# AcrylicShrimp/omok-ai

Hardware: AMD Instinct MI355X
Metric: self-play games/sec (15x15, 800 sims/move); MCTS nodes/sec (higher is better)
Workload: dtype f16x3 split MFMA, fp32 acc; fc0 corrections mixed f16/fp6; 1 GPU; 4096 concurrent 15x15 games per GPU, 800 sims/move, K=16, two trees per game; games_per_gpu=4096, board=15, sims_per_move=800, batch_k=16, warmup_step=whole episode, parallelism=games sharded x1, no hot-path collective

## Files before the change

bindings/omok_mi355x.rs:

```rust
#![allow(non_camel_case_types, dead_code)]

use std::ffi::{CStr, CString};
use std::os::raw::{c_char, c_int, c_void};
use std::ptr;

#[repr(C)]
#[derive(Clone, Copy, Debug)]
pub struct OmokConfig {
    pub board_size: i32,
    pub games: i32,
    pub max_nodes: i32,
    pub max_tables: i32,
    pub max_batch_k: i32,
    pub device: i32,
    pub net_mode: i32,
    pub max_tree_waves: i32,
    pub seed: u64,
    pub game_offset: i64,
}

#[repr(C)]
pub struct OmokEngine {
    _private: [u8; 0],
}
// ... 129 lines not shown
        pub fn omok_mirror_apply(e: *mut OmokEngine) -> c_int;
        pub fn omok_train_begin(e: *mut OmokEngine, max_batch: i32) -> c_int;
        pub fn omok_train_end(e: *mut OmokEngine) -> c_int;
        pub fn omok_train_step(e: *mut OmokEngine, records_dev: *const c_void, n_records: i64, indices: *const i64, batch: i32, losses: *mut f32) -> c_int;
        pub fn omok_train_losses(e: *mut OmokEngine, records_dev: *const c_void, n_records: i64, indices: *const i64, batch: i32, losses: *mut f32) -> c_int;
        pub fn omok_train_batch_indices(e: *mut OmokEngine, n_records: i64, batch: i32, key: u64, step: i32, out: *mut i64) -> c_int;
        pub fn omok_train_run(e: *mut OmokEngine, records_dev: *const c_void, n_records: i64, update_count: i32, batch_size: i32, key: u64, losses: *mut f32) -> c_int;
        pub fn omok_train_gradient_count(e: *const OmokEngine) -> i64;
        pub fn omok_train_backward(e: *mut OmokEngine, records_dev: *const c_void, n_records: i64, indices: *const i64, batch: i32, grad_dst_dev: *mut c_void) -> c_int;
        pub fn omok_train_apply(e: *mut OmokEngine, grads_dev: *const c_void, ranks: i32, losses: *mut f32) -> c_int;
        pub fn omok_debug_train_gradient(e: *mut OmokEngine, index: i32, out: *mut f32, count: i64) -> c_int;
        pub fn omok_net_read(e: *mut OmokEngine, index: i32, out: *mut f32, count: i64) -> c_int;
        pub fn omok_alive_count(e: *mut OmokEngine) -> c_int;
        pub fn omok_current_ply(e: *mut OmokEngine) -> c_int;
        pub fn omok_game_info(e: *mut OmokEngine, alive: *mut u8, status: *mut u8, plies: *mut i32) -> c_int;
        pub fn omok_tree_dump(e: *mut OmokEngine, game: i32, side: i32, ints: *mut i32, floats: *mut f32, cap_nodes: i32) -> c_int;
        pub fn omok_tree_root(e: *mut OmokEngine, game: i32, side: i32, root_n: *mut u32, root_w: *mut f32, n_nodes: *mut i32, n_tables: *mut i32) -> c_int;
        pub fn omok_root_stats(e: *mut OmokEngine, n: *mut u32, w: *mut f32) -> c_int;
        pub fn omok_root_children(e: *mut OmokEngine, game: i32, side: i32, actions: *mut i32, n: *mut u32, w: *mut f32, p: *mut f32, cap: i32) -> c_int;
        pub fn omok_replay_game(e: *mut OmokEngine, game: i32, boards: *mut u8, turns: *mut u8, pi: *mut f32, z: *mut f32, cap_plies: i32) -> c_int;
        pub fn omok_game_log_enable(e: *mut OmokEngine, enabled: i32) -> c_int;
        pub fn omok_game_log_read(e: *mut OmokEngine, first_game: i32, games: i32, start_boards: *mut u8, lengths: *mut i32, moves: *mut u16, root_n: *mut u32, root_w: *mut f32, child_n: *mut u32, child_w: *mut f32) -> c_int;
        pub fn omok_env_replay(e: *mut OmokEngine, start_boards: *const u8, moves: *const u16, lengths: *const i32, batch: i32, stride: i32, upto: i32, boards_out: *mut u8, status_out: *mut i32, played_out: *mut i32) -> c_int;
        pub fn omok_replay_pack_dev(e: *mut OmokEngine, dst_dev: *mut c_void, cap_records: i64) -> i64;
        pub fn omok_replay_record_bytes(e: *const OmokEngine) -> i32;
        pub fn omok_replay_augment_dev(e: *mut OmokEngine, dst_dev: *mut c_void, cap_records: i64) -> i64;
        pub fn omok_replay_augment_records_dev(e: *mut OmokEngine, records_dev: *const c_void, n_records: i64, game_offsets: *const i64, game_lengths: *const i32, games: i32, dst_dev: *mut c_void, cap_records: i64) -> i64;
        pub fn omok_replay_augmented_game(e: *mut OmokEngine, game: i32, boards: *mut u8, turns: *mut u8, pi: *mut f32, z: *mut f32, cap_records: i32) -> c_int;
        pub fn omok_operand_row_bytes(e: *const OmokEngine) -> i64;
        pub fn omok_debug_operand_rows(e: *mut OmokEngine, first_row: i32, rows: i32, out: *mut c_void) -> c_int;
        pub fn omok_debug_set_base_cache(e: *mut OmokEngine, enabled: i32) -> c_int;
        pub fn omok_debug_set_children_kernel(e: *mut OmokEngine, which: i32) -> c_int;
        pub fn omok_debug_set_window_rects(e: *mut OmokEngine, enabled: i32) -> c_int;
        pub fn omok_debug_last_plan(e: *mut OmokEngine, out: *mut i32, cap: i32) -> c_int;
        pub fn omok_get_stats(e: *mut OmokEngine, stats: *mut f64) -> c_int;
        pub fn omok_reset_stats(e: *mut OmokEngine) -> c_int;
        pub fn omok_set_profiling(e: *mut OmokEngine, enabled: i32) -> c_int;
    }
}


#[repr(u8)]
#[derive(Clone, Copy, Debug, PartialEq, Eq)]
pub enum GameStatus {
    InProgress = 0,
    Draw = 1,
    BlackWin = 2,
    WhiteWin = 3,
}

impl GameStatus {
    pub fn from_raw(v: i32) -> Option<GameStatus> {
        match v {
            0 => Some(GameStatus::InProgress),
            1 => Some(GameStatus::Draw),
            2 => Some(GameStatus::BlackWin),
            3 => Some(GameStatus::WhiteWin),
            _ => None,
        }
    }
}

#[derive(Debug)]
pub struct OmokError {
    pub code: i32,
    pub message: String,
// ... 142 lines not shown
```

include/omok_mi355x.h:

```cpp
#ifndef OMOK_MI355X_H
#define OMOK_MI355X_H
#include <stdint.h>

#ifdef __cplusplus
extern "C" {
#endif

#define OMOK_OK 0
#define OMOK_ERR_INVALID (-1)
#define OMOK_ERR_HIP (-2)
#define OMOK_ERR_STATE (-3)
#define OMOK_ERR_OVERFLOW (-4)
#define OMOK_ERR_ILLEGAL (-5)

#define OMOK_MODE_PLAYER 0
#define OMOK_MODE_OPPONENT 1

#define OMOK_NET_F16X3 0
#define OMOK_NET_F32 1
#define OMOK_NET_F16X3_ROWS 2

#define OMOK_NET_F16X3_FP6 3
#define OMOK_NET_F16X3_F16 4
#define OMOK_NET_F16X3_MIXED 5
// ... 108 lines not shown
int omok_debug_train_gradient(omok_engine* e, int32_t index, float* out, int64_t count);
int omok_net_read(omok_engine* e, int32_t index, float* out, int64_t count);

int omok_alive_count(omok_engine* e);
int omok_current_ply(omok_engine* e);
int omok_game_info(omok_engine* e, uint8_t* alive, uint8_t* status, int32_t* plies);
int omok_tree_dump(omok_engine* e, int32_t game, int32_t side, int32_t* ints, float* floats, int32_t cap_nodes);
int omok_tree_root(omok_engine* e, int32_t game, int32_t side, uint32_t* root_n, float* root_w,
                   int32_t* n_nodes, int32_t* n_tables);
int omok_root_stats(omok_engine* e, uint32_t* n, float* w);
int omok_root_children(omok_engine* e, int32_t game, int32_t side, int32_t* actions, uint32_t* n, float* w, float* p, int32_t cap);
int omok_replay_game(omok_engine* e, int32_t game, uint8_t* boards, uint8_t* turns, float* pi, float* z,
                     int32_t cap_plies);
#define OMOK_MOVE_CELL 255
#define OMOK_MOVE_EXTERNAL 256
int omok_game_log_enable(omok_engine* e, int32_t enabled);
int omok_game_log_read(omok_engine* e, int32_t first_game, int32_t games, uint8_t* start_boards, int32_t* lengths, uint16_t* moves,
                       uint32_t* root_n, float* root_w, uint32_t* child_n, float* child_w);
int omok_env_replay(omok_engine* e, const uint8_t* start_boards, const uint16_t* moves, const int32_t* lengths, int32_t batch,
                    int32_t stride, int32_t upto, uint8_t* boards_out, int32_t* status_out, int32_t* played_out);
int64_t omok_replay_pack_dev(omok_engine* e, void* dst_dev, int64_t cap_records);
int32_t omok_replay_record_bytes(const omok_engine* e);
int64_t omok_replay_augment_dev(omok_engine* e, void* dst_dev, int64_t cap_records);
int64_t omok_replay_augment_records_dev(omok_engine* e, const void* records_dev, int64_t n_records, const int64_t* game_offsets,
                                        const int32_t* game_lengths, int32_t games, void* dst_dev, int64_t cap_records);
int omok_replay_augmented_game(omok_engine* e, int32_t game, uint8_t* boards, uint8_t* turns, float* pi, float* z,
                               int32_t cap_records);

int64_t omok_operand_row_bytes(const omok_engine* e);
int omok_debug_operand_rows(omok_engine* e, int32_t first_row, int32_t rows, void* out);
int omok_debug_set_base_cache(omok_engine* e, int32_t enabled);
int omok_debug_set_children_kernel(omok_engine* e, int32_t which);
int omok_debug_set_window_rects(omok_engine* e, int32_t enabled);
#define OMOK_PLAN_INTS 16
int omok_debug_last_plan(omok_engine* e, int32_t* out, int32_t cap);

#define OMOK_STAT_SIMS 0
#define OMOK_STAT_EVALS 1
#define OMOK_STAT_PLY_GAMES 2
#define OMOK_STAT_FINISHED 3
#define OMOK_STAT_MS_TREE 4
#define OMOK_STAT_MS_TRUNK 5
#define OMOK_STAT_MS_FC0 6
#define OMOK_STAT_MS_TAIL 7
#define OMOK_STAT_MS_PLY 8
#define OMOK_STAT_FC0_LAUNCHES 9
#define OMOK_STAT_FC0_ROWS 10
#define OMOK_STAT_TREE_BYTES 11
#define OMOK_STAT_ROUND_LAUNCHES 12
#define OMOK_STAT_MS_ROUND 13
#define OMOK_STAT_PEAK_NODES 14
#define OMOK_STAT_PEAK_TABLES 15
#define OMOK_STAT_FC0_FORMAT 16
#define OMOK_STAT_PROBE_ROWS 17
#define OMOK_STAT_PROBE_DP_FP6 18
#define OMOK_STAT_PROBE_DV_FP6 19
#define OMOK_STAT_PROBE_DP_F16 20
#define OMOK_STAT_PROBE_DV_F16 21
#define OMOK_STAT_PROBE_LIMIT 22
#define OMOK_STAT_PROBE_LOGIT_MAX 23
#define OMOK_STAT_CHILDREN2_LAUNCHES 24
#define OMOK_STAT_CHILDREN1_LAUNCHES 25
#define OMOK_STAT_PROBE_DLOGIT_FP6 26
#define OMOK_STAT_PROBE_DLOGIT_F16 27
#define OMOK_STAT_PROBE_ROUND_ROWS 28
#define OMOK_STAT_PROBE_ROUND_FP6 29
// ... 25 lines not shown
```

omok-ai_amd/api.py:

```python
import ctypes as C

import os

import numpy as np

from . import binding as B
from . import weights as W

EMPTY, BLACK, WHITE = 0, 1, 2
TURN_BLACK, TURN_WHITE = 0, 1
IN_PROGRESS, DRAW, BLACK_WIN, WHITE_WIN = 0, 1, 2, 3


class Engine:

    def __init__(self, board_size=15, games=1, max_nodes=2048, max_tables=1024, max_batch_k=16, device=0,
                 net_mode=B.NET_F16X3, seed=0, game_offset=0, max_tree_waves=0):
        self.n, self.hw, self.games = board_size, board_size * board_size, games
        self.max_nodes = max_nodes
        self.max_batch_k = max_batch_k
        cfg = B.Config(board_size, games, max_nodes, max_tables, max_batch_k, device, net_mode, max_tree_waves, seed, game_offset)
        h = C.c_void_p()
        rc = B.lib().omok_create(C.byref(cfg), C.byref(h))
        if rc != 0:
# ... 185 lines not shown
        played = np.zeros(batch, dtype=np.int32)
        self._chk(B.lib().omok_env_replay(self.h, None if start is None else B.u8ptr(start), moves.ctypes.data_as(C.POINTER(C.c_uint16)),
                                          B.iptr(lengths), batch, moves.shape[1], int(upto), B.u8ptr(boards), B.iptr(status), B.iptr(played)))
        return boards, status, played

    def replay_augment_records(self, records_ptr, n_records, offsets, lengths, dst_ptr, cap_records):
        offsets = np.ascontiguousarray(offsets, dtype=np.int64).reshape(-1)
        lengths = np.ascontiguousarray(lengths, dtype=np.int32).reshape(-1)
        if len(offsets) != len(lengths):
            raise ValueError(f"{len(offsets)} offsets for {len(lengths)} lengths")
        n = B.lib().omok_replay_augment_records_dev(self.h, C.c_void_p(records_ptr), int(n_records), offsets.ctypes.data_as(C.POINTER(C.c_int64)),
                                                    B.iptr(lengths), len(lengths), C.c_void_p(dst_ptr), int(cap_records))
        if n < 0:
            raise B.OmokError(int(n), B.lib().omok_last_error(self.h).decode())
        return int(n)

    def encode_nn_input(self, boards, turns, mode=B.MODE_PLAYER):
        boards = np.ascontiguousarray(boards, dtype=np.uint8).reshape(-1, self.hw)
        turns = np.ascontiguousarray(turns, dtype=np.uint8).reshape(-1)
        out = np.zeros((boards.shape[0], 3 * self.hw), dtype=np.float32)
        self._chk(B.lib().omok_encode_nn_input(self.h, B.u8ptr(boards), B.u8ptr(turns), boards.shape[0], mode, B.fptr(out)))
        return out.reshape(-1, self.n, self.n, 3)

    def operand_rows(self, first_row, rows):
        nb = int(B.lib().omok_operand_row_bytes(self.h))
        if nb < 0:
            raise B.OmokError(nb, "no operand rows in this net mode")
        out = np.empty((rows, nb), dtype=np.uint8)
        self._chk(B.lib().omok_debug_operand_rows(self.h, first_row, rows, out.ctypes.data_as(C.c_void_p)))
        return out

    def set_base_cache(self, on=True):
        self._chk(B.lib().omok_debug_set_base_cache(self.h, int(bool(on))))

    def set_window_rects(self, on=True):
        self._chk(B.lib().omok_debug_set_window_rects(self.h, int(bool(on))))

    def set_children_kernel(self, which=2):
        self._chk(B.lib().omok_debug_set_children_kernel(self.h, int(which)))

    def last_plan(self):
        out = np.zeros(len(B.PLAN_NAMES), dtype=np.int32)
        n = self._chk(B.lib().omok_debug_last_plan(self.h, B.iptr(out), out.size))
        assert n == out.size
        d = dict(zip(B.PLAN_NAMES, (int(x) for x in out)))
        d["path"] = B.PLAN_PATHS[d["path"]]
        return d

    def set_profiling(self, on=True):
        self._chk(B.lib().omok_set_profiling(self.h, int(on)))

    def stats(self):
        s = (C.c_double * len(B.STAT_NAMES))()
        self._chk(B.lib().omok_get_stats(self.h, s))
        return dict(zip(B.STAT_NAMES, list(s)))

    def reset_stats(self):
        self._chk(B.lib().omok_reset_stats(self.h))


class Environment:

    def __init__(self, engine):
        self.eng = engine
        self._board = np.zeros((1, engine.hw), dtype=np.uint8)
        self._turn = np.zeros(1, dtype=np.uint8)
# ... 320 lines not shown
```

omok-ai_amd/binding.py:

```python
import ctypes as C
import os
import subprocess

import numpy as np

_HERE = os.path.dirname(os.path.abspath(__file__))
LIB_PATH = os.environ.get("OMOK_MI355X_LIB") or os.path.join(_HERE, "libomok_mi355x.so")

OK = 0
NET_F16X3, NET_F32, NET_F16X3_ROWS, NET_F16X3_FP6, NET_F16X3_F16, NET_F16X3_MIXED = 0, 1, 2, 3, 4, 5
FC0_FORMATS = {-1: "f32", 0: "fp6", 1: "f16", 2: "mixed"}
MODE_PLAYER, MODE_OPPONENT = 0, 1
OPP_RANDOM, OPP_NAIVE = 0, 1
PLAN_NAMES = ["path", "rows", "nsplit", "tsplit", "runs", "singles", "run_rows", "full_runs", "tiles", "t_split", "ways", "fways",
              "fc0_format", "n_cu", "nsup", "reserved"]
PLAN_PATHS = {-1: "none", 0: "plain", 1: "copy", 2: "difference", 3: "f32"}
STAT_NAMES = ["sims", "evals", "ply_games", "finished", "ms_tree", "ms_trunk", "ms_fc0", "ms_tail", "ms_ply",
              "fc0_launches", "fc0_rows", "tree_bytes", "round_launches", "ms_round", "peak_nodes", "peak_tables",
              "fc0_format", "probe_rows", "probe_dp_fp6", "probe_dv_fp6", "probe_dp_f16", "probe_dv_f16", "probe_limit", "probe_logit_max",
              "children2_launches", "children1_launches", "probe_dlogit_fp6", "probe_dlogit_f16", "probe_round_rows",
              "probe_round_dp_fp6", "probe_round_dv_fp6", "probe_round_dlogit_fp6", "probe_round_dp_mixed", "probe_round_dv_mixed", "probe_round_dlogit_mixed",
              "probe_round_dp_f16", "probe_round_dv_f16", "probe_round_dlogit_f16", "probe_logit_limit", "probe_outside",
              "work_diff_runs", "work_diff_singles", "work_diff_children", "work_copy_runs", "work_copy_singles", "work_copy_children", "work_diff_full_runs",
              "work_win_pixels", "work_win_tiles", "work_full_tiles", "ms_train_apply"]

SYMBOLS = [
    "omok_create", "omok_destroy", "omok_last_error", "omok_net_num_tensors", "omok_net_tensor_size", "omok_net_load",
    "omok_net_commit", "omok_net_load_file", "omok_net_save_file", "omok_net2_load", "omok_net2_commit", "omok_net2_load_file", "omok_net2_info", "omok_match_reset", "omok_evaluate_pv", "omok_evaluate_logits", "omok_env_play", "omok_env_place_stone", "omok_encode_nn_input", "omok_selfplay_reset", "omok_set_episode", "omok_execute", "omok_execute_shared", "omok_execute_shared_recorded",
    "omok_compute_policy", "omok_play_actions", "omok_set_actions", "omok_root_children",
    "omok_env_scripted_actions", "omok_opponent_actions", "omok_versus_run",
    "omok_env_check_positions", "omok_selfplay_reset_from", "omok_root_stats",
    "omok_match_reset_from", "omok_env_random_positions",
    "omok_sample_actions", "omok_advance", "omok_selfplay_run", "omok_selfplay_run_slots", "omok_round_generate", "omok_round_inputs",
    "omok_round_eval", "omok_round_outputs", "omok_round_logits", "omok_round_inject", "omok_round_scatter", "omok_mirror_generate",
    "omok_mirror_inputs", "omok_mirror_eval", "omok_mirror_outputs", "omok_mirror_inject", "omok_mirror_apply",
    "omok_alive_count", "omok_current_ply", "omok_game_info", "omok_tree_dump", "omok_tree_root", "omok_replay_game",
    "omok_operand_row_bytes", "omok_debug_operand_rows", "omok_debug_set_base_cache", "omok_debug_set_children_kernel", "omok_debug_set_window_rects", "omok_debug_last_plan",
    "omok_replay_pack_dev", "omok_replay_record_bytes", "omok_replay_augment_dev", "omok_replay_augmented_game", "omok_get_stats", "omok_reset_stats", "omok_set_profiling",
    "omok_train_begin", "omok_train_end", "omok_train_step", "omok_train_losses", "omok_train_batch_indices", "omok_train_run",
    "omok_train_gradient_count", "omok_train_backward", "omok_train_apply",
    "omok_debug_train_gradient", "omok_net_read",
    "omok_game_log_enable", "omok_game_log_read", "omok_env_replay",
    "omok_replay_augment_records_dev",
    "omok_selfplay_run_slots_logged", "omok_game_log_entry_bytes",
]


class Config(C.Structure):
    _fields_ = [("board_size", C.c_int32), ("games", C.c_int32), ("max_nodes", C.c_int32), ("max_tables", C.c_int32),
                ("max_batch_k", C.c_int32), ("device", C.c_int32), ("net_mode", C.c_int32), ("max_tree_waves", C.c_int32),
                ("seed", C.c_uint64), ("game_offset", C.c_int64)]


class OmokError(RuntimeError):
    def __init__(self, code, msg):
        super().__init__(f"omok error {code}: {msg}")
        self.code = code


def build():
    subprocess.check_call(["make", "-s", "-C", os.path.join(_HERE, "csrc")])


_lib = None


def lib():
    global _lib
    if _lib is not None:
        return _lib
    if not os.path.exists(LIB_PATH):
        raise OmokError(-2, f"{LIB_PATH} is missing: build it with __graft_entry__.build() (hipcc --offload-arch=gfx950); "
                            "there is no CPU fallback")
    L = C.CDLL(LIB_PATH)
    fp, ip = C.POINTER(C.c_float), C.POINTER(C.c_int32)
    u8p = C.POINTER(C.c_uint8)
    H = C.c_void_p
    L.omok_create.argtypes = [C.POINTER(Config), C.POINTER(H)]
    L.omok_destroy.argtypes = [H]
    L.omok_destroy.restype = None
    L.omok_last_error.argtypes = [H]
    L.omok_last_error.restype = C.c_char_p
    L.omok_net_tensor_size.argtypes = [H, C.c_int]
    L.omok_net_tensor_size.restype = C.c_int64
    L.omok_net_load.argtypes = [H, C.c_int, fp, C.c_int64]
    L.omok_net_commit.argtypes = [H]
    L.omok_net_load_file.argtypes = [H, C.c_char_p]
    L.omok_net_save_file.argtypes = [H, C.c_char_p]
    L.omok_net2_load.argtypes = [H, C.c_int, fp, C.c_int64]
    L.omok_net2_commit.argtypes = [H]
    L.omok_net2_load_file.argtypes = [H, C.c_char_p]
    L.omok_net2_info.argtypes = [H, ip, ip, C.POINTER(C.c_double)]
    L.omok_match_reset.argtypes = [H, C.c_int32]
    L.omok_evaluate_pv.argtypes = [H, fp, C.c_int32, fp, fp]
    L.omok_evaluate_logits.argtypes = [H, fp, C.c_int32, fp, fp]
    L.omok_env_play.argtypes = [H, ip, C.c_int32, C.c_int32, ip, u8p, u8p, C.POINTER(C.c_uint16)]
    L.omok_encode_nn_input.argtypes = [H, u8p, u8p, C.c_int32, C.c_int32, fp]
    L.omok_selfplay_reset.argtypes = [H]
    L.omok_execute_shared_recorded.argtypes = [H, C.c_int32, C.c_int32, C.c_float, C.c_float, C.c_int32, u8p, u8p, ip, fp, fp, C.c_int32, ip, ip]
    L.omok_operand_row_bytes.argtypes = [H]
    L.omok_operand_row_bytes.restype = C.c_int64
    L.omok_debug_operand_rows.argtypes = [H, C.c_int32, C.c_int32, C.c_void_p]
    L.omok_debug_set_base_cache.argtypes = [H, C.c_int32]
    L.omok_debug_set_children_kernel.argtypes = [H, C.c_int32]
    L.omok_debug_set_window_rects.argtypes = [H, C.c_int32]
    L.omok_debug_last_plan.argtypes = [H, ip, C.c_int32]
    L.omok_set_episode.argtypes = [H, C.c_uint64]
    L.omok_env_place_stone.argtypes = [H, u8p, u8p, C.POINTER(C.c_uint16), ip, C.c_int32, ip]
    L.omok_compute_policy.argtypes = [H, fp, u8p]
    L.omok_play_actions.argtypes = [H, ip]
    L.omok_set_actions.argtypes = [H, ip]
    L.omok_env_scripted_actions.argtypes = [H, C.c_int32, u8p, u8p, C.c_int32, ip]
    L.omok_opponent_actions.argtypes = [H, C.c_int32, ip]
    L.omok_versus_run.argtypes = [H, C.c_int32, C.c_int32, C.c_int32, C.c_int32, C.c_float, C.c_float, C.c_int32, ip, C.POINTER(C.c_double)]
    L.omok_env_check_positions.argtypes = [H, u8p, C.c_int32, ip, ip]
    L.omok_selfplay_reset_from.argtypes = [H, u8p]
    L.omok_match_reset_from.argtypes = [H, C.c_int32, u8p]
    L.omok_env_random_positions.argtypes = [H, C.c_uint64, C.c_int64, C.c_int32, C.c_int32, u8p, u8p]
    L.omok_root_stats.argtypes = [H, C.POINTER(C.c_uint32), fp]
    L.omok_root_children.argtypes = [H, C.c_int32, C.c_int32, ip, C.POINTER(C.c_uint32), fp, fp, C.c_int32]
    L.omok_execute.argtypes = [H, C.c_int32, C.c_int32, C.c_float, C.c_float]
    L.omok_execute_shared.argtypes = [H, C.c_int32, C.c_int32, C.c_float, C.c_float, C.c_int32]
    L.omok_sample_actions.argtypes = [H, C.c_float, C.c_int32, ip]
    L.omok_advance.argtypes = [H]
    L.omok_selfplay_run.argtypes = [H, C.c_int32, C.c_int32, C.c_float, C.c_float, C.c_float, C.c_int32, C.c_int32,
                                    C.POINTER(C.c_double)]
    L.omok_selfplay_run_slots.argtypes = [H, C.c_int32, C.c_int32, C.c_int32, C.c_float, C.c_float, C.c_float, C.c_int32, C.c_void_p, C.c_int64,
                                          C.POINTER(C.c_int64), ip, ip, C.POINTER(C.c_int64), C.POINTER(C.c_double)]
    L.omok_selfplay_run_slots_logged.argtypes = [H, C.c_int32, C.c_int32, C.c_int32, C.c_float, C.c_float, C.c_float, C.c_int32, C.c_void_p, C.c_int64,
                                                 C.c_void_p, C.POINTER(C.c_int64), ip, ip, C.POINTER(C.c_int64), C.POINTER(C.c_double)]
    L.omok_game_log_entry_bytes.argtypes = []
    L.omok_game_log_entry_bytes.restype = C.c_int32
    L.omok_round_generate.argtypes = [H, C.c_int32, C.c_int32, C.c_float, C.c_float, ip]
    L.omok_round_inputs.argtypes = [H, fp]
    L.omok_round_eval.argtypes = [H]
    L.omok_round_outputs.argtypes = [H, fp, fp]
    L.omok_round_logits.argtypes = [H, fp, fp]
    L.omok_round_inject.argtypes = [H, fp, fp]
# ... 56 lines not shown
```

omok-ai_amd/csrc/common.h:

```cpp
#pragma once
#include <hip/hip_runtime.h>
#include <stdint.h>

namespace omok {

constexpr uint16_t NONE16 = 0xFFFFu;
constexpr uint8_t NONE8 = 0xFFu;
constexpr int KMAX = 64;
constexpr float F32_EPS = 1.1920928955078125e-7f;

enum { ST_IN_PROGRESS = 0, ST_DRAW = 1, ST_BLACK_WIN = 2, ST_WHITE_WIN = 3 };
enum { RNG_EXPAND = 1, RNG_NOISE = 2, RNG_SAMPLE = 3, RNG_OPPONENT = 4, RNG_TRAIN_BATCH = 5 };

template <int N>
struct Geo {
    static constexpr int HW = N * N;
    static constexpr int ROWP = (HW + 63) / 64 * 64;
    static constexpr int NW = (HW + 63) / 64;
    static constexpr int IT = ROWP / 64;
};

struct __attribute__((aligned(16))) NodeHdr {
    uint16_t parent;
    uint16_t table;
// ... 35 lines not shown
struct Store {
    NodeHdr* hdr;
    uint64_t* board;
    float* policy;
    uint32_t* tcn;
    float* tcw;
    uint16_t* tcidx;
    uint8_t* tcorder;
    uint16_t* towner;
    TreeState* ts;
    uint16_t* req_node;
    GameState* gs;
    uint32_t* req_ref;
    uint32_t* req_aux;
    int32_t* d_count;
    uint64_t* rp_board;
    uint8_t* rp_turn;
    float* rp_pi;
    float* rp_z;
    unsigned long long* d_bytes;
    int cap_nodes, cap_tables, games;
    int stride_nodes, stride_tables;
};

struct RoundArgs {
    int side, round, K, ply;
    float epsilon, alpha;
    uint64_t seed;
    int64_t game_offset;
    const float* scatter_v;
    int32_t* req_cnt;
    int32_t* zero_ptr;
    int zero_n;
};

void launch_reset(int n, const Store& S, const float* root_policy_dev , hipStream_t st);
void launch_reset_from(int n, const Store& S, const uint8_t* boards_dev, const float* p_dev, const float* p2_dev, int split, hipStream_t st);
void launch_random_positions(int n, uint64_t key, int64_t first_game, int stones, int batch, uint8_t* boards_dev, uint8_t* ok_dev, hipStream_t st);
void launch_position_check(int n, const uint8_t* boards_dev, int batch, int32_t* verdict_dev, int32_t* stones_dev, hipStream_t st);
struct GameLog {
    uint32_t* root_n;
    float* root_w;
    uint32_t* child_n;
    float* child_w;
    uint16_t* move;
    uint8_t* start_board;
};
void launch_log_move(int n, const Store& S, int side, int start_ply, const GameLog& L, hipStream_t st);
void launch_replay(int n, const uint8_t* start_dev, const int32_t* verdict_dev, const uint16_t* moves_dev, const int32_t* lengths_dev, int batch, int stride,
                   int upto, uint8_t* boards_out, int32_t* status_out, int32_t* played_out, hipStream_t st);
void launch_root_stats(const Store& S, int side, uint32_t* n_dev, float* w_dev, hipStream_t st);
struct SlotMeta { long long offset; int32_t len; int32_t status; };
void launch_harvest(int n, const Store& S, uint8_t* mask_dev , long long* slot_off_dev , long long* out_count_dev, SlotMeta* meta_dev,
                    uint8_t* dst_dev, long long cap_records, hipStream_t st);
constexpr int LOG_ENTRY_BYTES = 20;
void launch_harvest_log(int n, const Store& S, const GameLog& L, const uint8_t* mask_dev, const long long* slot_off_dev, uint8_t* log_dst_dev,
                        long long cap_records, hipStream_t st);
void launch_refill(int n, const Store& S, const float* root_policy_dev, int32_t* next_gid_dev, int total_games, int32_t* new_gid_dev , hipStream_t st);
void launch_round(int n, const Store& S, const RoundArgs& a, hipStream_t st);
void launch_fill(const Store& S, int side, int K, hipStream_t st);
void launch_scan(int n, const Store& S, int side, int K, hipStream_t st, unsigned long long* evals_dev = nullptr, int32_t* zero_ptr = nullptr, int zero_n = 0,
                 bool fill = true);
void launch_round_shared(int n, const Store& S, const RoundArgs& a, int rounds_total, int group, int waves, uint16_t* sh_req, uint32_t* sh_cnt,
                         hipStream_t st, uint8_t* rec_order = nullptr, uint32_t* rec_pos = nullptr);
void launch_scatter_shared(int n, const Store& S, int side, const float* p_dev, const float* v_dev, int max_count, int waves, const uint16_t* sh_req,
                           const uint32_t* sh_cnt, hipStream_t st, uint8_t* rec_order = nullptr, uint32_t* rec_pos = nullptr);
constexpr int MAX_TREE_WAVES = 16;
constexpr int MAX_GAMES = 32767;
constexpr int SCAN_GAMES_PER_THREAD = 32;
void launch_scatter(int n, const Store& S, int side, const float* p_dev, const float* v_dev, int max_count, hipStream_t st, bool backups = true);
void launch_backups(int n, const Store& S, int side, const float* v_dev, hipStream_t st);
void launch_softmax_scatter(int n, const Store& S, int side, const float* logits_dev, int lrow, float* v_dev, float* vpre_dev, int max_count,
                            hipStream_t st, bool backups = true);
void launch_sample(int n, const Store& S, int side, int ply, float temperature, int threshold, uint64_t seed,
                   int64_t game_offset, int32_t* actions_dev, hipStream_t st);
void launch_mirror_scan(int n, const Store& S, int side, hipStream_t st);
void launch_advance(int n, const Store& S, int side, const float* p_dev, hipStream_t st);
void launch_encode_requests(int n, const Store& S, float* out_dev , int max_b, hipStream_t st);
void launch_env_play(int n, const int32_t* moves_dev, int batch, int len, int32_t* status_dev, uint8_t* boards_dev,
                     uint8_t* turns_dev, uint16_t* legal_dev, hipStream_t st);
void launch_encode_boards(int n, const uint8_t* boards_dev, const uint8_t* turns_dev, int batch, int mode,
                          float* out_dev, hipStream_t st);
void launch_replay_pack(int n, const Store& S, const long long* offsets_dev, uint8_t* dst_dev, long long cap_records, hipStream_t st);
void launch_replay_offsets(int n, const Store& S, int per_transition, long long* offsets_dev , hipStream_t st);
void launch_set_actions(int n, const Store& S, int side, const int32_t* actions_dev, uint32_t* d_flags , hipStream_t st);
void launch_clear_actions(const Store& S, hipStream_t st);
void launch_opponent_move(int n, const Store& S, int side, int kind, uint64_t seed, int64_t game_offset, int32_t* actions_dev, hipStream_t st);
void launch_env_scripted(int n, const uint8_t* boards_dev, int kind, int batch, int32_t* forced_dev, hipStream_t st);
void launch_policy(int n, const Store& S, int side, float* pi_dev , uint8_t* has_dev , hipStream_t st);
void launch_env_place(int n, uint8_t* boards_dev, uint8_t* turns_dev, uint16_t* legal_dev, const int32_t* actions_dev, int batch,
                      int32_t* status_dev, hipStream_t st);
int set_advance_lds_attribute(int n, size_t bytes);
void launch_replay_augment(int n, const Store& S, const long long* offsets_dev, int game_first, int game_count, long long base_sub,
                           uint8_t* dst_dev, long long cap_records, hipStream_t st);
struct AugSpan { long long src, dst; };
void launch_replay_augment_records(int n, const uint8_t* src_dev, const long long* first_dev, const AugSpan* span_dev, int m, long long transitions,
                                   uint8_t* dst_dev, long long cap_records, hipStream_t st);
size_t advance_lds_bytes(int cap_nodes, int cap_tables);

void launch_match_split(const Store& S, int tree_side, int split, uint32_t* ref2, uint32_t* aux2, int32_t* cnt, unsigned long long* evals, int max_rows,
                        hipStream_t st);
void launch_match_join(const int32_t* cnt, const float* v2, float* v1, const float* p2, float* p1, int rowp, int max_rows, hipStream_t st);
void launch_match_roots(int n, const Store& S, const float* root_policy2, int split, hipStream_t st);

struct NetBuffers;
}
```

omok-ai_amd/csrc/engine.cpp:

```cpp
#include "../../include/omok_mi355x.h"
#include "common.h"
#include "net.h"
#include "train.h"

#include <algorithm>
#include <cstdarg>
#include <cstdio>
#include <cstring>
#include <string>
#include <vector>

using namespace omok;

hipEvent_t Prof::get() {
    if (n_pool > 0) return pool[--n_pool];
    hipEvent_t e;
    hipEventCreate(&e);
    return e;
}
void Prof::begin(int cat, hipStream_t st) {
    if (!enabled || !active) return;
    if (n_items == cap_items) {
        if (cap_items >= 8192) resolve();
        else {
// ... 27 lines not shown
    }
    n_items = 0;
}
void Prof::destroy() {
    resolve();
    for (int i = 0; i < n_pool; ++i) hipEventDestroy(pool[i]);
    free(pool);
    free(items);
    pool = nullptr; items = nullptr; n_pool = cap_pool = n_items = cap_items = 0;
}

struct omok_engine {
    omok_config cfg{};
    int n = 0, hw = 0, rowp = 0, nw = 0, T = 0;
    Store S{};
    Net net{};
    Prof prof{};
    hipStream_t st = nullptr;
    std::vector<void*> allocs;
    std::string err;
    int ply = 0;
    int start_ply = 0;
    bool reset_done = false;
    bool sampled = false;
    uint64_t episode = 0;
    uint64_t key = 0;
    int round_reqs = -1;
    int round_cap = 0;
    int mirror_reqs = -1;
    float* d_root_policy = nullptr;
    int32_t* d_actions = nullptr;
    uint32_t* d_error = nullptr;
    unsigned long long* d_evals = nullptr;
    int32_t* d_req_cnt = nullptr;
    uint16_t* d_sh_req = nullptr;
    uint32_t* d_sh_cnt = nullptr;
    uint32_t* d_flags = nullptr;
    float* d_pi = nullptr;
    uint8_t* d_has = nullptr;
    long long* d_aug_offsets = nullptr;
    uint8_t* d_aug_scratch = nullptr;
    Net* net2 = nullptr;
    bool match = false;
    int split = 0;
    int match_cnt[2] = {0, 0};
    uint32_t* d_mref = nullptr;
    uint32_t* d_maux = nullptr;
    int32_t* d_mcnt = nullptr;
    unsigned long long* d_mevals = nullptr;
    float* d_root_policy2 = nullptr;
    Train* train = nullptr;
    bool log_on = false;
    bool log_started = false;
    void* log_mem = nullptr;
    GameLog log{};
    double sims = 0, evals = 0, ply_games = 0, finished = 0;
    uint32_t peak_nodes = 0, peak_tables = 0;
    size_t bytes = 0;
};

static std::string g_create_error;

static int fail(omok_engine* e, int code, const char* fmt, ...) {
    char buf[512];
    va_list ap;
    va_start(ap, fmt);
// ... 155 lines not shown
    S.stride_nodes = cfg->max_nodes | 1;
    S.stride_tables = cfg->max_tables | 1;
    S.games = cfg->games;
    const size_t T = (size_t)e->T, cn = (size_t)S.stride_nodes, ct = (size_t)S.stride_tables, rp = (size_t)e->rowp;
    const size_t G = (size_t)cfg->games, HW = (size_t)e->hw;
    if (cfg->max_tree_waves < 0 || cfg->max_tree_waves > MAX_TREE_WAVES)
        { omok_destroy(e); return fail(nullptr, OMOK_ERR_INVALID, "max_tree_waves must be in [0, %d]", MAX_TREE_WAVES); }
    const size_t max_b = std::max(G, (size_t)cfg->max_tree_waves) * (size_t)cfg->max_batch_k;
    int rc = 0;
    rc |= dalloc(e, &S.hdr, T * cn);
    rc |= dalloc(e, &S.board, T * cn * 2 * e->nw);
    rc |= dalloc(e, &S.policy, T * cn * rp);
    rc |= dalloc(e, &S.tcn, T * ct * rp);
    rc |= dalloc(e, &S.tcw, T * ct * rp);
    rc |= dalloc(e, &S.tcidx, T * ct * rp);
    rc |= dalloc(e, &S.tcorder, T * ct * rp);
    rc |= dalloc(e, &S.towner, T * ct);
    rc |= dalloc(e, &S.ts, T);
    rc |= dalloc(e, &S.req_node, T * KMAX);
    rc |= dalloc(e, &S.gs, G);
    rc |= dalloc(e, &S.req_ref, max_b);
    rc |= dalloc(e, &S.req_aux, max_b);
    rc |= dalloc(e, &S.d_count, 4);
    rc |= dalloc(e, &S.rp_board, G * HW * 2 * e->nw);
    rc |= dalloc(e, &S.rp_turn, G * HW);
    rc |= dalloc(e, &S.rp_pi, G * HW * rp);
    rc |= dalloc(e, &S.rp_z, G * HW);
    rc |= dalloc(e, &S.d_bytes, 2);
    rc |= dalloc(e, &e->d_root_policy, rp);
    rc |= dalloc(e, &e->d_actions, G);
    rc |= dalloc(e, &e->d_error, 4);
    rc |= dalloc(e, &e->d_evals, 2);
    rc |= dalloc(e, &e->d_req_cnt, G);
    rc |= dalloc(e, &e->d_sh_req, (size_t)MAX_TREE_WAVES * KMAX);
    rc |= dalloc(e, &e->d_sh_cnt, 2 * (size_t)KMAX);
    rc |= dalloc(e, &e->d_flags, 4);
    rc |= dalloc(e, &e->d_pi, G * HW);
    rc |= dalloc(e, &e->d_has, G);
    rc |= dalloc(e, &e->d_aug_offsets, G + 1);
    if (rc) {
        g_create_error = e->err;
        omok_destroy(e);
        return OMOK_ERR_HIP;
    }
    hipMemsetAsync(S.d_count, 0, 16, e->st);
    hipMemsetAsync(S.d_bytes, 0, 16, e->st);
    hipMemsetAsync(e->d_error, 0, 16, e->st);
    hipMemsetAsync(e->d_evals, 0, 16, e->st);
    hipMemsetAsync(S.gs, 0, sizeof(GameState) * G, e->st);
    hipMemsetAsync(S.ts, 0, sizeof(TreeState) * T, e->st);
    if (set_advance_lds_attribute(e->n, advance_lds_bytes(cfg->max_nodes, cfg->max_tables)) != 0) {
        g_create_error = "hipFuncSetAttribute(k_advance, max dynamic LDS) failed";
        omok_destroy(e);
        return OMOK_ERR_HIP;
    }
    configure_net(e, e->net, (int)max_b);
    if (net_alloc(e->net) == 0) {
        g_create_error = "net buffer allocation failed (hipMalloc)";
        omok_destroy(e);
        return OMOK_ERR_HIP;
    }
    if (hipStreamSynchronize(e->st) != hipSuccess) {
        g_create_error = "stream sync failed after init";
        omok_destroy(e);
        return OMOK_ERR_HIP;
    }
    *out = e;
    return OMOK_OK;
}

extern "C" int omok_net_num_tensors(void) { return NET_TENSORS; }
extern "C" int64_t omok_net_tensor_size(const omok_engine* e, int index) { return e ? net_tensor_size(e->n, index) : -1; }

static int sync_and_check(omok_engine* e, const char* what);

static int net2_alloc(omok_engine* e) {
    if (e->net2) return 0;
    const size_t mb = (size_t)e->net.max_b;
    if (!e->d_mref && dalloc(e, &e->d_mref, mb)) return OMOK_ERR_HIP;
    if (!e->d_maux && dalloc(e, &e->d_maux, mb)) return OMOK_ERR_HIP;
    if (!e->d_mcnt && dalloc(e, &e->d_mcnt, 4)) return OMOK_ERR_HIP;
// ... 141 lines not shown
        if (hipMemcpy(buf.data(), e->net.w[i], sizeof(float) * len, hipMemcpyDeviceToHost) != hipSuccess) { fclose(f); return fail(e, OMOK_ERR_HIP, "weight read-back failed"); }
        ok = wr_u64(f, len) && fwrite(buf.data(), sizeof(float), len, f) == len;
    }
    ok = (fclose(f) == 0) && ok;
    return ok ? OMOK_OK : fail(e, OMOK_ERR_INVALID, "short write to %s", path);
}

static int need_net(omok_engine* e) {
    if (!e->net.committed) return fail(e, OMOK_ERR_STATE, "net not loaded/committed (omok_net_load x31 + omok_net_commit)");
    if (e->match && !e->net2->committed) return fail(e, OMOK_ERR_STATE, "match episode: net 2 was reloaded and not committed (omok_net2_commit)");
    return 0;
}

static Net& net_at(omok_engine* e, int idx) { return idx == 0 ? e->net : *e->net2; }
static void invalidate_nets(omok_engine* e) {
    net_invalidate_sibling_cache(e->net);
    if (e->net2) net_invalidate_sibling_cache(*e->net2);
}
static bool block_live(const omok_engine* e, int b) { return b == 0 ? e->split > 0 : e->split < e->cfg.games; }
static Store block_view(const omok_engine* e, int b) {
    Store V = e->S;
    if (b == 0) V.d_count = e->d_mcnt;
    else { V.req_ref = e->d_mref; V.req_aux = e->d_maux; V.d_count = e->d_mcnt + 1; }
    return V;
}
struct Block { Net* net; Store view; int rows, off, b; };
static int eval_blocks(omok_engine* e, int tree_side, int rows, bool pending, Block out[2]) {
    if (!e->match) { out[0] = Block{&e->net, e->S, rows, 0, 0}; return 1; }
    int n = 0;
    for (int b = 0; b < 2; ++b)
        if (block_live(e, b)) out[n++] = Block{&net_at(e, tree_side ^ b), block_view(e, b), pending ? e->match_cnt[b] : rows, b ? e->match_cnt[0] : 0, b};
    return n;
}
static void block_forward(omok_engine* e, const Block& B, int max_count, int sibling_side = -1, bool skip_softmax = false) {
    Net& X = *B.net;
    if (e->match) {
        X.grp_lo = B.b ? e->split : 0;
        X.grp_hi = B.b ? e->cfg.games : e->split;
        X.grp_sub = B.b ? e->d_mcnt : nullptr;
    }
    net_forward_requests(X, B.view, max_count, e->st, &e->prof, sibling_side, skip_softmax);
    if (e->match) {
        X.grp_hi = -1;
        X.grp_sub = nullptr;
    }
}
static void match_split(omok_engine* e, int tree_side, int max_rows) {
    launch_match_split(e->S, tree_side, e->split, e->d_mref, e->d_maux, e->d_mcnt, e->d_mevals, max_rows, e->st);
}
static void match_join(omok_engine* e, int tree_side, bool p, int max_rows) {
    if (!block_live(e, 1)) return;
    Net &A = net_at(e, tree_side), &B = net_at(e, tree_side ^ 1);
    launch_match_join(e->d_mcnt, B.v, A.v, p ? B.p : nullptr, p ? A.p : nullptr, e->rowp, max_rows, e->st);
}
static int match_counts(omok_engine* e) {
    HIPCHK(e, hipMemcpyAsync(e->match_cnt, e->d_mcnt, sizeof(e->match_cnt), hipMemcpyDeviceToHost, e->st));
    return sync_and_check(e, "match counts") ? OMOK_ERR_HIP : 0;
}
static int no_match(omok_engine* e, const char* what) {
    if (e->match) return fail(e, OMOK_ERR_STATE, "%s is not available in a match episode (omok_match_reset): start self-play with omok_selfplay_reset", what);
    return 0;
}

static int check_async(omok_engine* e, const char* what) {
    hipError_t r = hipGetLastError();
    if (r != hipSuccess) return fail(e, OMOK_ERR_HIP, "%s: launch failed: %s", what, hipGetErrorString(r));
    return 0;
}

static int sync_and_check(omok_engine* e, const char* what) {
    hipError_t r = hipStreamSynchronize(e->st);
    if (r != hipSuccess) return fail(e, OMOK_ERR_HIP, "%s: %s", what, hipGetErrorString(r));
    return check_async(e, what);
}
// ... 386 lines not shown

extern "C" int omok_match_reset_from(omok_engine* e, int32_t split, const uint8_t* boards) {
    if (!e || !boards) return OMOK_ERR_INVALID;
    if (int rc = check_reset(e, true, split)) return rc;
    ENTER(e);
    return reset_from_positions(e, boards, true, split);
}

extern "C" int omok_env_random_positions(omok_engine* e, uint64_t key, int64_t first_game, int32_t stones, int32_t batch, uint8_t* boards_out,
                                         uint8_t* ok_out) {
    if (!e || !boards_out || !ok_out) return OMOK_ERR_INVALID;
    if (stones < 0 || stones >= e->hw) return fail(e, OMOK_ERR_INVALID, "stones %d outside [0, %d)", stones, e->hw);
    if (batch < 1) return fail(e, OMOK_ERR_INVALID, "batch %d < 1", batch);
    ENTER(e);
    const size_t B = (size_t)batch;
    Scratch sc;
    uint8_t* d_out = sc.get<uint8_t>(B * e->hw + B);
    if (!d_out) return fail(e, OMOK_ERR_HIP, "env_random_positions: device allocation failed");
    e->prof.begin(PC_PLY, e->st);
    launch_random_positions(e->n, key, first_game, stones, batch, d_out, d_out + B * e->hw, e->st);
    e->prof.end(e->st);
    hipMemcpyAsync(boards_out, d_out, B * e->hw, hipMemcpyDeviceToHost, e->st);
    hipMemcpyAsync(ok_out, d_out + B * e->hw, B, hipMemcpyDeviceToHost, e->st);
    return sync_and_check(e, "env_random_positions") ? OMOK_ERR_HIP : OMOK_OK;
}

static int need_reset(omok_engine* e) {
    if (!e->reset_done) return fail(e, OMOK_ERR_STATE, "omok_selfplay_reset has not been called");
    return 0;
}

static Net& backup_net(omok_engine* e, int side) { return e->match ? net_at(e, side) : e->net; }

static void forward_and_scatter(omok_engine* e, const Block& B, int side, int rows_cap, bool backups_inline) {
    Net& X = *B.net;
    const bool fused = net_logits_cover_batch(X, rows_cap);
    block_forward(e, B, rows_cap, side, fused);
    e->prof.begin(PC_TREE_OTHER, e->st);
    if (fused) {
        int lrow = 0;
        const float* lg = net_logits(X, &lrow);
        launch_softmax_scatter(e->n, B.view, side, lg, lrow, X.v, X.vpre, rows_cap, e->st, backups_inline);
    } else launch_scatter(e->n, B.view, side, X.p, X.v, rows_cap, e->st, backups_inline);
    e->prof.end(e->st);
}

static void enqueue_round(omok_engine* e, int round, int K, float eps, float alpha, bool eval_and_scatter, int alive, bool defer_backups = false,
                          bool pending_backups = false) {
    const int side = e->ply & 1;
    const int max_req = std::min(alive * K, e->net.max_b);
    const bool sib_round = !e->match && eval_and_scatter && net_round_takes_sibling_path(e->net, max_req);
    RoundArgs a{side, round, K, e->ply, eps, alpha, e->key, e->cfg.game_offset, pending_backups ? backup_net(e, side).v : nullptr,
                sib_round ? e->d_req_cnt : nullptr, sib_round ? e->net.d_gcnt : nullptr, sib_round ? NET_GCNT_INTS : 0};
    e->prof.round_begin();
    e->prof.begin(PC_ROUND, e->st);
    launch_round(e->n, e->S, a, e->st);
    e->prof.end(e->st);
    e->prof.begin(PC_TREE_OTHER, e->st);
    if (!sib_round) launch_scan(e->n, e->S, side, K, e->st, e->d_evals);
    if (e->match) match_split(e, side, max_req);
    else {
        e->net.gcnt_zeroed = e->net.fill_in_group = sib_round;
        e->net.scan_cnt = sib_round ? e->d_req_cnt : nullptr;
        e->net.scan_evals = e->d_evals;
        e->net.fill_side = side;
        e->net.fill_k = K;
    }
    e->prof.end(e->st);
    if (eval_and_scatter) {
        Block blk[2];
        const int nb = eval_blocks(e, side, alive * K, false, blk);
        for (int i = 0; i < nb; ++i) forward_and_scatter(e, blk[i], side, alive * K, !e->match && !defer_backups);
        if (e->match) {
            e->prof.begin(PC_TREE_OTHER, e->st);
            match_join(e, side, false, max_req);
            if (!defer_backups) launch_backups(e->n, e->S, side, net_at(e, side).v, e->st);
            e->prof.end(e->st);
        }
    }
    e->prof.round_end();
}

static int enqueue_execute(omok_engine* e, int count, int K, float eps, float alpha, int alive) {
    int processed = 0, round = 0;
    while (processed < count) {
        enqueue_round(e, round, K, eps, alpha, true, alive, true, round > 0);
        processed += K;
        round += 1;
    }
    if (round > 0) {
        e->prof.begin(PC_TREE_OTHER, e->st);
        launch_backups(e->n, e->S, e->ply & 1, backup_net(e, e->ply & 1).v, e->st);
        e->prof.end(e->st);
    }
    return round;
}

static int check_exec_args(omok_engine* e, int count, int K, float eps, float alpha) {
    if (count < 1) return fail(e, OMOK_ERR_INVALID, "count must be >= 1");
    if (K < 1 || K > e->cfg.max_batch_k) return fail(e, OMOK_ERR_INVALID, "batch_size %d outside [1, max_batch_k=%d]", K, e->cfg.max_batch_k);
    if (!(alpha > 0.0f && alpha <= (float)OMOK_ALPHA_MAX)) return fail(e, OMOK_ERR_INVALID, "alpha must be in (0, %d]", OMOK_ALPHA_MAX);
    if (!(eps >= 0.0f && eps <= 1.0f)) return fail(e, OMOK_ERR_INVALID, "epsilon must be in [0,1]");
    return 0;
}

static int check_temperature(omok_engine* e, float temperature) {
    if (!(temperature > 0.0f && 1.0f / temperature <= (float)OMOK_TEMPERATURE_INV_MAX))
        return fail(e, OMOK_ERR_INVALID, "temperature must be >= 1 / %d", OMOK_TEMPERATURE_INV_MAX);
    return 0;
}

static int check_search(omok_engine* e, int count, int K, float eps, float alpha, float temperature = 1.0f) {
    if (need_net(e) || need_reset(e)) return OMOK_ERR_STATE;
    if (check_exec_args(e, count, K, eps, alpha)) return OMOK_ERR_INVALID;
    return check_temperature(e, temperature);
}

extern "C" int omok_execute(omok_engine* e, int32_t count, int32_t batch_size, float epsilon, float alpha) {
    if (!e) return OMOK_ERR_INVALID;
    if (int rc = check_search(e, count, batch_size, epsilon, alpha)) return rc;
    HIPCHK(e, hipSetDevice(e->cfg.device));
    uint32_t bits = 0, alive = 0;
    if (read_status(e, &bits, &alive)) return OMOK_ERR_HIP;
    const int rounds = enqueue_execute(e, count, batch_size, epsilon, alpha, (int)alive);
    e->sims += (double)rounds * batch_size * alive;
    if (read_status(e, &bits, &alive)) return OMOK_ERR_HIP;
    return tree_error(e, bits);
}

struct SharedRecording {
    uint8_t *sim_order, *backup_order;
    int32_t* group_counts;
    float *p, *v;
    int32_t cap_requests, *n_groups, *n_requests;
};
static int execute_shared(omok_engine* e, const char* who, int count, int K, float epsilon, float alpha, int waves, const SharedRecording* rec) {
    if (int rc = check_search(e, count, K, epsilon, alpha)) return rc;
    if (no_match(e, who)) return OMOK_ERR_STATE;
    if (e->cfg.games != 1) return fail(e, OMOK_ERR_INVALID, "%s searches ONE tree: create the engine with games = 1 (got %d)", who, e->cfg.games);
    if (waves < 1 || waves > MAX_TREE_WAVES || waves * K > e->net.max_b)
        return fail(e, OMOK_ERR_INVALID, "waves must be in [1, %d] and waves * batch_size <= %d (the net batch, sized by max(games, max_tree_waves = %d) * max_batch_k)",
                    MAX_TREE_WAVES, e->net.max_b, e->cfg.max_tree_waves);
    ENTER(e);
    const size_t per = (size_t)waves * K;
    Scratch sc;
    uint8_t* d_rec = rec ? sc.get<uint8_t>(2 * per) : nullptr;
    uint32_t* d_pos = rec ? sc.get<uint32_t>(2) : nullptr;
    if (sc.failed) return fail(e, OMOK_ERR_HIP, "recorded mode: device allocation failed");
    std::vector<float> prow(rec ? per * e->rowp : 0);
    uint32_t bits = 0, alive = 0;
    if (read_status(e, &bits, &alive)) return OMOK_ERR_HIP;
    const int side = e->ply & 1;
    RoundArgs a{side, 0, 0, e->ply, epsilon, alpha, e->key, e->cfg.game_offset};
    e->prof.begin(PC_ROUND, e->st);
    launch_round(e->n, e->S, a, e->st);
    e->prof.end(e->st);
    int exec_count = count / K;
    if (exec_count * K != count) exec_count += 1;
    a.K = K;
    int group = 0, total_req = 0;
    for (; group * waves < exec_count; ++group) {
        if (rec) {
            hipMemsetAsync(d_rec, 0xFF, 2 * per, e->st);
            hipMemsetAsync(d_pos, 0, 8, e->st);
        }
        e->prof.begin(PC_ROUND, e->st);
        launch_round_shared(e->n, e->S, a, exec_count, group, waves, e->d_sh_req, e->d_sh_cnt, e->st, d_rec, d_pos);
        k_add_evals<<<1, 64, 0, e->st>>>(e->S.d_count, e->d_evals);
        e->prof.end(e->st);
        int32_t cnt = 0;
        if (rec) {
            if (hipMemcpyAsync(&cnt, e->S.d_count, 4, hipMemcpyDeviceToHost, e->st) != hipSuccess || sync_and_check(e, "execute_shared_recorded")) return OMOK_ERR_HIP;
            if (total_req + cnt > rec->cap_requests) return fail(e, OMOK_ERR_INVALID, "recorded mode: more than cap_requests = %d requests", rec->cap_requests);
        }
        if (!rec || cnt > 0) net_forward_requests(e->net, e->S, waves * K, e->st, &e->prof);
        if (cnt > 0) {
            hipMemcpyAsync(prow.data(), e->net.p, sizeof(float) * (size_t)cnt * e->rowp, hipMemcpyDeviceToHost, e->st);
            hipMemcpyAsync(rec->v + total_req, e->net.v, sizeof(float) * cnt, hipMemcpyDeviceToHost, e->st);
        }
        e->prof.begin(PC_TREE_OTHER, e->st);
        launch_scatter_shared(e->n, e->S, side, e->net.p, e->net.v, waves * K, waves, e->d_sh_req, e->d_sh_cnt, e->st, rec ? d_rec + per : nullptr, rec ? d_pos + 1 : nullptr);
        e->prof.end(e->st);
        if (!rec) continue;
        uint32_t pos[2] = {0, 0};
        hipMemcpyAsync(rec->sim_order + (size_t)group * per, d_rec, per, hipMemcpyDeviceToHost, e->st);
        hipMemcpyAsync(rec->backup_order + (size_t)group * per, d_rec + per, per, hipMemcpyDeviceToHost, e->st);
// ... 26 lines not shown
    const SharedRecording rec{sim_order, backup_order, group_counts, p, v, cap_requests, n_groups, n_requests};
    return execute_shared(e, "omok_execute_shared_recorded", count, batch_size, epsilon, alpha, waves, &rec);
}

static void enqueue_sample(omok_engine* e, float temperature, int threshold) {
    e->prof.begin(PC_PLY, e->st);
    launch_sample(e->n, e->S, e->ply & 1, e->ply, temperature, threshold, e->key, e->cfg.game_offset, e->d_actions, e->st);
    e->prof.end(e->st);
}

static void enqueue_opponent_move(omok_engine* e, int kind) {
    e->prof.begin(PC_PLY, e->st);
    launch_opponent_move(e->n, e->S, e->ply & 1, kind, e->key, e->cfg.game_offset, e->d_actions, e->st);
    e->prof.end(e->st);
}

extern "C" int omok_sample_actions(omok_engine* e, float temperature, int32_t threshold, int32_t* actions) {
    if (!e) return OMOK_ERR_INVALID;
    if (need_reset(e)) return OMOK_ERR_STATE;
    if (check_temperature(e, temperature)) return OMOK_ERR_INVALID;
    HIPCHK(e, hipSetDevice(e->cfg.device));
    enqueue_sample(e, temperature, threshold);
    if (actions) HIPCHK(e, hipMemcpyAsync(actions, e->d_actions, sizeof(int32_t) * e->cfg.games, hipMemcpyDeviceToHost, e->st));
    uint32_t bits = 0;
    if (read_status(e, &bits, nullptr)) return OMOK_ERR_HIP;
    e->sampled = true;
    return tree_error(e, bits);
}

static void enqueue_log_move(omok_engine* e, int side) {
    if (e->log_on && e->log_started) launch_log_move(e->n, e->S, side, e->start_ply, e->log, e->st);
}

static void enqueue_advance(omok_engine* e, int max_rows) {
    const int side = e->ply & 1;
    if (e->match) match_join(e, 1 - side, true, max_rows);
    enqueue_log_move(e, side);
    launch_advance(e->n, e->S, side, backup_net(e, 1 - side).p, e->st);
    invalidate_nets(e);
}

static void enqueue_mirror_and_advance(omok_engine* e, int alive) {
    const int side = e->ply & 1;
    e->prof.begin(PC_PLY, e->st);
    launch_mirror_scan(e->n, e->S, side, e->st);
    k_add_evals<<<1, 64, 0, e->st>>>(e->S.d_count, e->d_evals);
    if (e->match) match_split(e, 1 - side, alive);
    e->prof.end(e->st);
    Block blk[2];
    const int nb = eval_blocks(e, 1 - side, alive, false, blk);
    for (int i = 0; i < nb; ++i) block_forward(e, blk[i], alive);
    e->prof.begin(PC_PLY, e->st);
    enqueue_advance(e, alive);
    e->prof.end(e->st);
}

struct Search { int count, K; float epsilon, alpha, temperature; int threshold; };

static void play_ply(omok_engine* e, const Search& s, int alive, int scripted = -1) {
    if (scripted >= 0) enqueue_opponent_move(e, scripted);
    else {
        const int rounds = enqueue_execute(e, s.count, s.K, s.epsilon, s.alpha, alive);
        enqueue_sample(e, s.temperature, s.threshold);
        e->sims += (double)rounds * s.K * alive;
    }
    enqueue_mirror_and_advance(e, alive);
}

static int end_ply(omok_engine* e, uint32_t* alive, bool count_finished = true) {
    uint32_t bits = 0, after = 0;
    if (read_status(e, &bits, &after)) return OMOK_ERR_HIP;
    e->ply_games += *alive;
    if (count_finished) e->finished += (double)*alive - (double)after;
    e->ply += 1;
    e->sampled = false;
    *alive = after;
    return tree_error(e, bits);
}

extern "C" int omok_advance(omok_engine* e) {
    if (!e) return OMOK_ERR_INVALID;
    if (need_net(e) || need_reset(e)) return OMOK_ERR_STATE;
    if (!e->sampled) return fail(e, OMOK_ERR_STATE, "omok_sample_actions must precede omok_advance");
    HIPCHK(e, hipSetDevice(e->cfg.device));
    uint32_t bits = 0, alive = 0;
    if (read_status(e, &bits, &alive)) return OMOK_ERR_HIP;
    enqueue_mirror_and_advance(e, (int)alive);
    return end_ply(e, &alive);
}

extern "C" int omok_selfplay_run(omok_engine* e, int32_t count, int32_t batch_size, float epsilon, float alpha,
                                 float temperature, int32_t threshold, int32_t max_plies, double* stats) {
    if (!e) return OMOK_ERR_INVALID;
    if (int rc = check_search(e, count, batch_size, epsilon, alpha, temperature)) return rc;
    HIPCHK(e, hipSetDevice(e->cfg.device));
    const Search s{count, batch_size, epsilon, alpha, temperature, threshold};
    uint32_t bits = 0, alive = 0;
    if (read_status(e, &bits, &alive)) return OMOK_ERR_HIP;
    for (int plies = 0; alive > 0 && (max_plies <= 0 || plies < max_plies); ++plies) {
// ... 189 lines not shown
    if (e->ply != e->start_ply)
        return fail(e, OMOK_ERR_STATE, "omok_versus_run starts at a fresh reset: %d move(s) were played since (the episode is at ply %d)", e->ply - e->start_ply, e->ply);
    HIPCHK(e, hipSetDevice(e->cfg.device));
    const Search s{count, batch_size, epsilon, alpha, 1.0f, 0};
    uint32_t bits = 0, alive = 0;
    if (read_status(e, &bits, &alive)) return OMOK_ERR_HIP;
    for (int plies = 0; alive > 0 && (max_plies <= 0 || plies < max_plies); ++plies) {
        play_ply(e, s, (int)alive, (e->ply & 1) == opponent_side ? kind : -1);
        if (int rc = end_ply(e, &alive)) return rc;
    }
    e->sampled = false;
    if (results) {
        std::vector<GameState> gs((size_t)e->cfg.games);
        HIPCHK(e, hipMemcpyAsync(gs.data(), e->S.gs, sizeof(GameState) * gs.size(), hipMemcpyDeviceToHost, e->st));
        if (sync_and_check(e, "versus_run")) return OMOK_ERR_HIP;
        results[0] = results[1] = results[2] = 0;
        for (const GameState& g : gs) {
            if (g.alive) continue;
            if (g.status == ST_BLACK_WIN) results[0] += 1;
            else if (g.status == ST_WHITE_WIN) results[1] += 1;
            else if (g.status == ST_DRAW) results[2] += 1;
        }
    }
    if (stats) return omok_get_stats(e, stats);
    return OMOK_OK;
}

extern "C" int omok_root_children(omok_engine* e, int32_t game, int32_t side, int32_t* actions, uint32_t* n, float* w, float* p, int32_t cap) {
    if (!e || game < 0 || game >= e->cfg.games || (side != 0 && side != 1) || cap < 0) return OMOK_ERR_INVALID;
    ENTER(e);
    const size_t t = (size_t)side * e->cfg.games + game, rp = (size_t)e->rowp, nw2 = 2 * (size_t)e->nw;
    const size_t tn = t * (size_t)e->S.stride_nodes, tt = t * (size_t)e->S.stride_tables;
    NodeHdr h0;
    HIPCHK(e, hipMemcpyAsync(&h0, e->S.hdr + tn, sizeof(h0), hipMemcpyDeviceToHost, e->st));
    if (sync_and_check(e, "root_children")) return OMOK_ERR_HIP;
    if (h0.table == NONE16 || h0.nch == 0) return 0;
    std::vector<uint32_t> cn(rp);
    std::vector<float> cw(rp), pol(rp);
    std::vector<uint8_t> co(rp);
    std::vector<uint64_t> bb(nw2);
    const size_t row = (tt + h0.table) * rp;
    hipMemcpyAsync(cn.data(), e->S.tcn + row, 4 * rp, hipMemcpyDeviceToHost, e->st);
    hipMemcpyAsync(cw.data(), e->S.tcw + row, 4 * rp, hipMemcpyDeviceToHost, e->st);
    hipMemcpyAsync(co.data(), e->S.tcorder + row, rp, hipMemcpyDeviceToHost, e->st);
    hipMemcpyAsync(pol.data(), e->S.policy + tn * rp, 4 * rp, hipMemcpyDeviceToHost, e->st);
    hipMemcpyAsync(bb.data(), e->S.board + tn * nw2, 8 * nw2, hipMemcpyDeviceToHost, e->st);
    if (sync_and_check(e, "root_children")) return OMOK_ERR_HIP;
    for (int a = 0; a < e->hw; ++a) {
        const int rank = co[a];
        if (rank == NONE8 || rank >= cap) continue;
        if (actions) actions[rank] = a;
        if (n) n[rank] = cn[a];
        if (w) w[rank] = cw[a];
        if (p) {
            const bool occ = ((bb[a / 64] | bb[e->nw + a / 64]) >> (a % 64)) & 1ULL;
            p[rank] = h0.has_policy ? pol[a] : ((occ || h0.legal == 0) ? 0.0f : 1.0f / (float)h0.legal);
        }
    }
    return h0.nch;
}

extern "C" int omok_env_place_stone(omok_engine* e, uint8_t* boards, uint8_t* turns, uint16_t* legal, const int32_t* actions,
                                    int32_t batch, int32_t* status_out) {
    if (!e || !boards || !turns || !legal || !actions || !status_out || batch < 1) return OMOK_ERR_INVALID;
    ENTER(e);
    const size_t B = (size_t)batch;
// ... 307 lines not shown
extern "C" int omok_tree_root(omok_engine* e, int32_t game, int32_t side, uint32_t* root_n, float* root_w, int32_t* n_nodes, int32_t* n_tables) {
    if (!e || game < 0 || game >= e->cfg.games || (side != 0 && side != 1)) return OMOK_ERR_INVALID;
    ENTER(e);
    TreeState ts;
    HIPCHK(e, hipMemcpyAsync(&ts, e->S.ts + (size_t)side * e->cfg.games + game, sizeof(ts), hipMemcpyDeviceToHost, e->st));
    if (sync_and_check(e, "tree_root")) return OMOK_ERR_HIP;
    if (root_n) *root_n = ts.root_n;
    if (root_w) *root_w = ts.root_w;
    if (n_nodes) *n_nodes = (int32_t)ts.n_nodes;
    if (n_tables) *n_tables = (int32_t)ts.n_tables;
    return OMOK_OK;
}

extern "C" int omok_root_stats(omok_engine* e, uint32_t* n, float* w) {
    if (!e || !n || !w) return OMOK_ERR_INVALID;
    if (need_reset(e)) return OMOK_ERR_STATE;
    ENTER(e);
    const size_t G = (size_t)e->cfg.games;
    uint32_t* d_n = (uint32_t*)e->d_pi;
    float* d_w = e->d_pi + G;
    launch_root_stats(e->S, e->ply & 1, d_n, d_w, e->st);
    std::vector<uint32_t> host(2 * G);
    HIPCHK(e, hipMemcpyAsync(host.data(), e->d_pi, 8 * G, hipMemcpyDeviceToHost, e->st));
    if (sync_and_check(e, "root_stats")) return OMOK_ERR_HIP;
    memcpy(n, host.data(), 4 * G);
    memcpy(w, host.data() + G, 4 * G);
    return OMOK_OK;
}

extern "C" int omok_tree_dump(omok_engine* e, int32_t game, int32_t side, int32_t* ints, float* floats, int32_t cap_nodes) {
    if (!e || !ints || !floats || game < 0 || game >= e->cfg.games || (side != 0 && side != 1)) return OMOK_ERR_INVALID;
    ENTER(e);
    const size_t t = (size_t)side * e->cfg.games + game;
    TreeState ts;
    HIPCHK(e, hipMemcpyAsync(&ts, e->S.ts + t, sizeof(ts), hipMemcpyDeviceToHost, e->st));
    if (sync_and_check(e, "tree_dump")) return OMOK_ERR_HIP;
    const int nn = (int)ts.n_nodes, nt = (int)ts.n_tables;
    if (nn > cap_nodes) return -nn;
    const size_t rp = (size_t)e->rowp, nw2 = 2 * (size_t)e->nw;
    std::vector<NodeHdr> hdr((size_t)nn);
    std::vector<uint64_t> board((size_t)nn * nw2);
    std::vector<float> pol((size_t)nn * rp), cw((size_t)nt * rp);
    std::vector<uint32_t> cn((size_t)nt * rp);
    std::vector<uint8_t> co((size_t)nt * rp);
    const size_t tn = t * (size_t)e->S.stride_nodes, tt = t * (size_t)e->S.stride_tables;
    hipMemcpyAsync(hdr.data(), e->S.hdr + tn, sizeof(NodeHdr) * nn, hipMemcpyDeviceToHost, e->st);
    hipMemcpyAsync(board.data(), e->S.board + tn * nw2, 8 * nw2 * nn, hipMemcpyDeviceToHost, e->st);
    hipMemcpyAsync(pol.data(), e->S.policy + tn * rp, 4 * rp * nn, hipMemcpyDeviceToHost, e->st);
    if (nt) {
        hipMemcpyAsync(cn.data(), e->S.tcn + tt * rp, 4 * rp * nt, hipMemcpyDeviceToHost, e->st);
        hipMemcpyAsync(cw.data(), e->S.tcw + tt * rp, 4 * rp * nt, hipMemcpyDeviceToHost, e->st);
        hipMemcpyAsync(co.data(), e->S.tcorder + tt * rp, rp * nt, hipMemcpyDeviceToHost, e->st);
    }
    if (sync_and_check(e, "tree_dump")) return OMOK_ERR_HIP;
    const int hw = e->hw;
    for (int i = 0; i < nn; ++i) {
        const NodeHdr& h = hdr[i];
        int32_t* o = ints + (size_t)i * 8;
        float* f = floats + (size_t)i * (1 + hw);
        uint32_t n = ts.root_n;
        float w = ts.root_w;
        int order = -1;
        if (i != 0) {
            const size_t slot = (size_t)hdr[h.parent].table * rp + h.action;
            n = cn[slot]; w = cw[slot]; order = co[slot];
        }
// ... 117 lines not shown
    long long off[2] = {0, 0};
    launch_replay_offsets(e->n, e->S, 6, e->d_aug_offsets, e->st);
    HIPCHK(e, hipMemcpyAsync(off, e->d_aug_offsets + game, 16, hipMemcpyDeviceToHost, e->st));
    if (sync_and_check(e, "replay_augmented_game")) return OMOK_ERR_HIP;
    const int total = (int)(off[1] - off[0]);
    const int n = total < cap_records ? total : cap_records;
    if (n <= 0) return total;
    launch_replay_augment(e->n, e->S, e->d_aug_offsets, game, 1, off[0], e->d_aug_scratch, (long long)max_rec, e->st);
    std::vector<uint8_t> host((size_t)total * rec);
    HIPCHK(e, hipMemcpyAsync(host.data(), e->d_aug_scratch, host.size(), hipMemcpyDeviceToHost, e->st));
    if (sync_and_check(e, "replay_augmented_game")) return OMOK_ERR_HIP;
    for (int i = 0; i < n; ++i) {
        const uint8_t* r = host.data() + (size_t)i * rec;
        if (boards) memcpy(boards + (size_t)i * hw, r, hw);
        if (turns) turns[i] = r[hw];
        if (pi) memcpy(pi + (size_t)i * hw, r + brd, 4 * hw);
        if (z) memcpy(z + i, r + brd + 4 * hw, 4);
    }
    return total;
}

extern "C" int64_t omok_operand_row_bytes(const omok_engine* e) { return e && e->net.mode != OMOK_NET_F32 ? (int64_t)e->net.row_u4 * 16 : OMOK_ERR_INVALID; }
extern "C" int omok_debug_operand_rows(omok_engine* e, int32_t first_row, int32_t rows, void* out) {
    if (!e || !out || first_row < 0 || rows < 0 || first_row + rows > e->net.max_b || e->net.mode == OMOK_NET_F32) return OMOK_ERR_INVALID;
    ENTER(e);
    HIPCHK(e, hipMemcpyAsync(out, (const char*)e->net.a_fc0 + (size_t)first_row * e->net.row_u4 * 16, (size_t)rows * e->net.row_u4 * 16, hipMemcpyDeviceToHost, e->st));
    return sync_and_check(e, "debug_operand_rows") ? OMOK_ERR_HIP : OMOK_OK;
}

extern "C" int omok_debug_set_base_cache(omok_engine* e, int32_t enabled) {
    if (!e) return OMOK_ERR_INVALID;
    e->net.base_cache = enabled != 0;
    net_invalidate_sibling_cache(e->net);
    return OMOK_OK;
}

extern "C" int omok_debug_set_window_rects(omok_engine* e, int32_t enabled) {
    if (!e) return OMOK_ERR_INVALID;
    e->net.win_rects = enabled != 0;
    return OMOK_OK;
}

extern "C" int omok_debug_set_children_kernel(omok_engine* e, int32_t which) {
    if (!e) return OMOK_ERR_INVALID;
    if (which != 1 && which != 2) return fail(e, OMOK_ERR_INVALID, "children kernel %d (1 = k_sib_children, 2 = k_sib_children2)", which);
    if (which == 1 && e->net.mode != OMOK_NET_F32 && e->net.diff_fp6)
        return fail(e, OMOK_ERR_STATE, "omok_debug_set_children_kernel(1): the engine runs the mixed operand format, whose difference path exists in k_sib_children2 only "
                                       "(create the engine with OMOK_NET_F16X3_FP6 or _F16 to compare the two kernels)");
    e->net.sib_v2 = which == 2;
    net_invalidate_sibling_cache(e->net);
    return OMOK_OK;
}

extern "C" int omok_debug_last_plan(omok_engine* e, int32_t* out, int32_t cap) {
    if (!e || !out || cap < 0) return OMOK_ERR_INVALID;
    ENTER(e);
    const Net& net = e->net;
    int32_t plan[OMOK_PLAN_INTS] = {};
    plan[0] = net.plan_path; plan[1] = net.plan_rows; plan[2] = net.plan_nsplit; plan[3] = net.plan_tsplit;
    plan[12] = net.mode == OMOK_NET_F32 ? -1 : net.diff_fp6 ? FC0_MIXED : net.fc0_fmt;
    plan[13] = net.n_cu;
    plan[14] = 2 * net.hw;
    if (sync_and_check(e, "debug_last_plan")) return OMOK_ERR_HIP;
    if ((net.plan_path == 1 || net.plan_path == 2) && net.d_gcnt) {
        int32_t c[NET_GCNT_HEAD_INTS];
        HIPCHK(e, hipMemcpy(c, net.d_gcnt, sizeof(c), hipMemcpyDeviceToHost));
// ... 86 lines not shown
```

omok-ai_amd/csrc/net.h:

```cpp
#pragma once
#include "common.h"
#include "../../include/omok_mi355x.h"

namespace omok {

constexpr int NET_TENSORS = 31;
constexpr int NC = 128;
constexpr int NM = 32;
constexpr int NF = 512;
enum { FC0_AUTO = -1, FC0_FP6 = 0, FC0_F16 = 1, FC0_MIXED = 2 };
constexpr float NET_PROBE_LIMIT = 3e-4f;
constexpr float NET_PROBE_LOGIT_LIMIT = 5e-4f;
constexpr float NET_PROBE_CONTRACT = 1e-3f;
constexpr int NET_PROBE_ROWS = 2048;

struct Net {
    int n = 0, hw = 0, rowp = 0, mode = 0;
    int cfg_mode = 0;
    bool siblings = true;
    int device = 0;
    int max_b = 0;
    bool committed = false;
    bool loaded[NET_TENSORS] = {};
    int64_t wsize[NET_TENSORS] = {};
// ... 73 lines not shown
        case 23: return NC * hw * NF;
        case 24: return NF;
        case 25: return (int64_t)NF * NF;
        case 26: return NF;
        case 27: return NF;
        case 28: return 1;
        case 29: return NF * hw;
        case 30: return hw;
    }
    return -1;
}

bool net_logits_cover_batch(const Net& net, int max_count);
bool net_round_takes_sibling_path(const Net& net, int max_count);
enum {
    NET_GCNT_RUNS = 0,
    NET_GCNT_SINGLES = 1,
    NET_GCNT_ROWS_IN_RUNS = 2,
    NET_GCNT_FULL_ROWS = 3,
    NET_GCNT_WIN_TILES = 4,
    NET_GCNT_SPLIT_TILE0 = 5,
    NET_GCNT_WIN_WAYS = 6,
    NET_GCNT_TILE_ORDER = 7,
    NET_GCNT_BINS = 8,
    NET_GCNT_FULL_EVALS = 96,
    NET_GCNT_UNCACHEABLE = 97,
    NET_GCNT_FULL_WAYS = 98,
    NET_GCNT_FULL_STRIDE = 99,
    NET_GCNT_HEAD_INTS = 100
};
constexpr int NET_GCNT_P0 = 8 + 81 + 7 + 16;
constexpr int NET_GCNT_INTS = NET_GCNT_P0 + 225;
constexpr int NET_WORK_DIFF = 0, NET_WORK_COPY = 3, NET_WORK_DIFF_FULL = 6, NET_WORK_WIN_PIXELS = 7, NET_WORK_WIN_TILES = 8, NET_WORK_FULL_TILES = 9, NET_WORK_COUNT = 16;
void net_forward_requests(Net& net, const Store& S, int max_count, hipStream_t st, struct Prof* prof, int sibling_side = -1, bool skip_softmax = false);
void net_forward_inputs(Net& net, const Store& S, int count, hipStream_t st, struct Prof* prof);
inline void net_invalidate_sibling_cache(Net& net) { net.sib_cache_valid = false; }
int net_commit(Net& net, const Store& S, hipStream_t st);
void net_set_fc0_format(Net& net, int fmt);
const float* net_logits(const Net& net, int* row_stride);
size_t net_alloc(Net& net);
void net_free(Net& net);

enum { PC_ROUND = 0, PC_TREE_OTHER, PC_TRUNK, PC_FC0, PC_TAIL, PC_PLY, PC_TRAIN_APPLY, PC_COUNT };
constexpr int PC_COUNT_MAX = 8;
struct Prof {
    bool enabled = false;
    int every = 1;
    long long rounds_seen = 0, rounds_timed = 0;
    bool active = true;
    bool in_round = false;
    double ms_s[PC_COUNT_MAX] = {};
    long long launches_s[PC_COUNT_MAX] = {};
    void round_begin() { in_round = true; active = every <= 1 || rounds_seen % every == 0; ++rounds_seen; if (active) ++rounds_timed; }
    void round_end() { in_round = false; active = true; }
    double scale() const { return rounds_timed > 0 ? (double)rounds_seen / (double)rounds_timed : 1.0; }
    double total_ms(int cat) const { return ms[cat] + ms_s[cat] * scale(); }
    double total_launches(int cat) const { return (double)launches[cat] + (double)launches_s[cat] * scale(); }
    struct Item { int cat; bool sampled; hipEvent_t a, b; };
    Item* items = nullptr;
    int n_items = 0, cap_items = 0;
    hipEvent_t* pool = nullptr;
    int n_pool = 0, cap_pool = 0;
    double ms[PC_COUNT] = {};
    long long launches[PC_COUNT] = {};
    hipEvent_t get();
    void begin(int cat, hipStream_t st);
    void end(hipStream_t st);
// ... 6 lines not shown
```

omok-ai_amd/csrc/net_kernels.hip:

```cpp
#include "net.h"

#include <cmath>
#include <cstdlib>
#include <cstring>
#include <vector>

namespace omok {

typedef _Float16 half8 __attribute__((ext_vector_type(8)));
typedef float f32x16 __attribute__((ext_vector_type(16)));
typedef float f32x4 __attribute__((ext_vector_type(4)));

enum { EPI_SPLIT = 0, EPI_LOGITS = 1, EPI_PARTIAL = 2 };
constexpr int GT_BS = 128;

__host__ __device__ inline int kperm(int T, int s, int h, int j) { return 32 * T + 16 * s + 8 * (j >> 2) + 4 * h + (j & 3); }
__device__ inline float lrelu(float x) {
    const float y = 0.2f * x;
    float r;
    asm("v_max_f32 %0, %1, %2" : "=v"(r) : "v"(x), "v"(y));
    return r;
}

typedef _Float16 half2v __attribute__((ext_vector_type(2)));
// ... 2567 lines not shown
        asm volatile("" ::: "memory");
        const bool stage = t + NST - 1 < ksteps;
        if (stage) issue_begin();
        else if (XT != 0) tail_issue(NST - 2 - rem);
        const half8* L = (const half8*)(lds + slot * STAGE_U4);
        half8 bh[2], bl[2], ah[MTW], al[MTW];
#pragma unroll
        for (int c = 0; c < 2; ++c) {
            bh[c] = L[(WFR + (2 * ws + c) * 2 + 0) * 64 + lane];
            bl[c] = L[(WFR + (2 * ws + c) * 2 + 1) * 64 + lane];
        }
#pragma unroll
        for (int i = 0; i < MTW; ++i) {
            ah[i] = L[((wm * MTW + i) * 2 + 0) * 64 + lane];
            al[i] = L[((wm * MTW + i) * 2 + 1) * 64 + lane];
        }
#pragma unroll
        for (int term = 0; term < 3; ++term)
#pragma unroll
            for (int i = 0; i < MTW; ++i) {
#pragma unroll
                for (int c = 0; c < 2; ++c) acc[i][c] = MFMA16(term == 1 ? al[i] : ah[i], term == 2 ? bl[c] : bh[c], acc[i][c]);
                if (stage && term == 0) {
#pragma unroll
                    for (int q = i; q < LPW; q += MTW) issue_one(q, nslot);
                }
            }
        if (stage) kt += 1;
        slot = slot + 1 == NST ? 0 : slot + 1;
        nslot = nslot + 1 == NST ? 0 : nslot + 1;
    }
}

template <int MT, int EPI, int TAG, int NST>
__global__ __launch_bounds__(512) void k_gemm_t(const uint4* __restrict__ wp, const uint4* __restrict__ act, int ksteps,
                                                size_t act_row_u4, int k_full, int last_cnt, int lo_off,
                                                const float* __restrict__ bias, uint4* __restrict__ out_split,
                                                size_t out_row_u4, float* __restrict__ out_logits, const int32_t* __restrict__ d_count,
                                                int max_count) {
    constexpr int MTW = MT / 4;
    extern __shared__ __attribute__((aligned(16))) unsigned char smem[];
    uint4* lds = (uint4*)smem;
    int count = d_count[0];
    if (count > max_count) count = max_count;
    const int b0 = blockIdx.x * GT_BS;
    if (b0 >= count) return;
    const int tid = threadIdx.x, lane = tid & 63;
    const int wave = __builtin_amdgcn_readfirstlane(tid >> 6);
    const int wm = wave >> 1, ws = wave & 1;
    const int h = lane >> 5;
    const int kbeg = EPI == EPI_PARTIAL ? (int)blockIdx.y * ksteps : 0;
    f32x16 acc[MTW][2];
    gemm_t_mainloop<MT, NST, 0>(lds, wp, act, ksteps, kbeg, act_row_u4, k_full, last_cnt, lo_off, b0, wave, lane, acc, [](int) {});

#pragma unroll
    for (int c = 0; c < 2; ++c) {
        const int sample = b0 + 32 * (2 * ws + c) + (lane & 31);
        if (sample >= count) continue;
#pragma unroll
        for (int i = 0; i < MTW; ++i) {
            const int mt = wm * MTW + i;
            float y[16];
#pragma unroll
            for (int g = 0; g < 4; ++g) {
                const f32x4 bv = *(const f32x4*)(bias + 32 * mt + 8 * g + 4 * h);
#pragma unroll
                for (int q = 0; q < 4; ++q) y[4 * g + q] = acc[i][c][4 * g + q] + bv[q];
            }
            if (EPI == EPI_PARTIAL) {
#pragma unroll
                for (int g = 0; g < 4; ++g) {
                    f32x4 o;
#pragma unroll
                    for (int q = 0; q < 4; ++q) o[q] = acc[i][c][4 * g + q];
                    *(f32x4*)(out_logits + ((size_t)blockIdx.y * out_row_u4 + sample) * (MT * 32) + 32 * mt + 8 * g + 4 * h) = o;
                }
            } else if (EPI == EPI_SPLIT) {
#pragma unroll
                for (int s = 0; s < 2; ++s) {
                    float v[8];
#pragma unroll
                    for (int j = 0; j < 8; ++j) v[j] = lrelu(y[8 * s + j]);
                    half8 hi, lo;
                    split8(v, hi, lo);
                    uint4* row = out_split + (size_t)sample * out_row_u4 + (size_t)(2 * mt + s) * 4;
                    row[h] = *(const uint4*)&hi;
                    row[2 + h] = *(const uint4*)&lo;
                }
            } else {
#pragma unroll
                for (int g = 0; g < 4; ++g) {
                    f32x4 o;
#pragma unroll
                    for (int q = 0; q < 4; ++q) o[q] = y[4 * g + q];
                    *(f32x4*)(out_logits + (size_t)sample * (MT * 32) + 32 * mt + 8 * g + 4 * h) = o;
                }
            }
        }
    }
}

template <int MTH>
__global__ __launch_bounds__(512) void k_tail_fused(const uint4* __restrict__ wp_fc1, const uint4* __restrict__ act, const float* __restrict__ bias_fc1,
                                                    const uint4* __restrict__ wp_heads, const float* __restrict__ bias_heads, float* __restrict__ out_logits,
                                                    const int32_t* __restrict__ d_count, int max_count) {
    constexpr int MTW = MTH / 4;
    constexpr int WFR = MTH * 2;
    constexpr int LPW = WFR / 8;
    constexpr int FC1_STAGE_U4 = 40 * 64;
    constexpr int H0_U4 = 2 * FC1_STAGE_U4, HST_U4 = WFR * 64;
    constexpr int CHUNK_U4 = 96 * 64;
    static_assert(WFR % 8 == 0 && 2 * HST_U4 <= FC1_STAGE_U4 && H0_U4 + HST_U4 <= CHUNK_U4, "heads ring inside the freed fc1 slots");
    extern __shared__ __attribute__((aligned(16))) unsigned char smem[];
    uint4* lds = (uint4*)smem;
    int count = d_count[0];
    if (count > max_count) count = max_count;
    const int b0 = blockIdx.x * GT_BS;
    if (b0 >= count) return;
    const int tid = threadIdx.x, lane = tid & 63;
    const int wave = __builtin_amdgcn_readfirstlane(tid >> 6);
    const int wm = wave >> 1, ws = wave & 1;
    const int h = lane >> 5;

    const uint4* hsrc = wp_heads + (size_t)wave * 64 + lane;
    auto hslot = [&](int slot) { return lds + (slot == 0 ? H0_U4 : (slot - 1) * HST_U4); };
    auto hissue_one = [&](int ks, int slot, int i) { dma16(hsrc + (size_t)ks * (WFR * 64) + i * 8 * 64, hslot(slot) + (wave + 8 * i) * 64); };
    auto hissue = [&](int ks, int slot) {
#pragma unroll
        for (int i = 0; i < LPW; ++i) hissue_one(ks, slot, i);
    };

    uint4 fr[4][2][2][2];
    {
        f32x16 acc[4][2];
        gemm_t_mainloop<16, 3, LPW>(lds, wp_fc1, act, 32, 0, 128, 32, 1, 2, b0, wave, lane, acc, [&](int j) { hissue(j, j); });
#pragma unroll
        for (int i = 0; i < 4; ++i) {
            const int mt = wm * 4 + i;
// ... 58 lines not shown
            const half8* L = (const half8*)hslot(slot);
            const half8* C = (const half8*)chunk + (size_t)(kk * 8) * 64 + lane;
            half8 bh[2], bl[2], ah[MTW], al[MTW];
#pragma unroll
            for (int c = 0; c < 2; ++c) {
                bh[c] = C[((2 * ws + c) * 2 + 0) * 64];
                bl[c] = C[((2 * ws + c) * 2 + 1) * 64];
            }
#pragma unroll
            for (int i = 0; i < MTW; ++i) {
                ah[i] = L[((wm * MTW + i) * 2 + 0) * 64 + lane];
                al[i] = L[((wm * MTW + i) * 2 + 1) * 64 + lane];
            }
#pragma unroll
            for (int term = 0; term < 3; ++term)
#pragma unroll
                for (int i = 0; i < MTW; ++i) {
#pragma unroll
                    for (int c = 0; c < 2; ++c) acc[i][c] = MFMA16(term == 1 ? al[i] : ah[i], term == 2 ? bl[c] : bh[c], acc[i][c]);
                    if (stage && term == 0) {
#pragma unroll
                        for (int q = i; q < LPW; q += MTW) hissue_one(ks + 2, nslot, q);
                    }
                }
            slot = slot + 1 == 3 ? 0 : slot + 1;
            nslot = nslot + 1 == 3 ? 0 : nslot + 1;
        }
    }

#pragma unroll
    for (int c = 0; c < 2; ++c) {
        const int sample = b0 + 32 * (2 * ws + c) + (lane & 31);
        if (sample >= count) continue;
#pragma unroll
        for (int i = 0; i < MTW; ++i) {
            const int mt = wm * MTW + i;
#pragma unroll
            for (int g = 0; g < 4; ++g) {
                const f32x4 bv = *(const f32x4*)(bias_heads + 32 * mt + 8 * g + 4 * h);
                f32x4 o;
#pragma unroll
                for (int q = 0; q < 4; ++q) o[q] = acc[i][c][4 * g + q] + bv[q];
                *(f32x4*)(out_logits + (size_t)sample * (MTH * 32) + 32 * mt + 8 * g + 4 * h) = o;
            }
        }
    }
}

constexpr int GW_DA = 3, GW_NB = 3;
constexpr int gemm_w_lds(int mt) { return (8 * GW_DA * (mt / 8) * 2 + GW_NB * 16) * 1024; }
template <int MT, int EPI>
__global__ __launch_bounds__(512) void k_gemm_w(const uint4* __restrict__ wp, const uint4* __restrict__ act, int ksteps, size_t act_row_u4,
                                                const float* __restrict__ bias, uint4* __restrict__ out_split, size_t out_row_u4,
                                                float* __restrict__ out_logits, const int32_t* __restrict__ d_count, int max_count) {
    static_assert(MT % 8 == 0 && EPI != EPI_PARTIAL, "k_gemm_w: whole-K launches of at least one m-tile per wave");
    constexpr int MTW = MT / 8;
    constexpr int AF = MTW * 2;
    constexpr int B_U4 = 128 * 8;
    extern __shared__ __attribute__((aligned(16))) unsigned char smem[];
    int count = d_count[0];
    if (count > max_count) count = max_count;
    const int b0 = blockIdx.x * GT_BS;
    if (b0 >= count) return;
    const int tid = threadIdx.x, lane = tid & 63;
    const int wave = __builtin_amdgcn_readfirstlane(tid >> 6);
    const int h = lane >> 5, sl = lane & 31;
    uint4* aring = (uint4*)smem + (size_t)wave * (GW_DA * AF * 64);
    uint4* ldsB = (uint4*)smem + (size_t)8 * GW_DA * AF * 64;
    const int nchunks = ksteps >> 1;
    const uint4* asrc = wp + (size_t)(wave * AF) * 64 + lane;
    const uint4* bsrc[2];
#pragma unroll
    for (int e = 0; e < 2; ++e) {
        const int s = 16 * wave + 8 * e + (lane >> 3);
        bsrc[e] = act + (size_t)(b0 + s) * act_row_u4 + (size_t)((lane & 7) ^ ((s >> 1) & 7));
    }
    auto issueA = [&](int kt, int slot) {
        kt = kt < ksteps ? kt : ksteps - 1;
#pragma unroll
        for (int i = 0; i < AF; ++i) dma16(asrc + (size_t)kt * (MT * 2 * 64) + i * 64, aring + (slot * AF + i) * 64);
    };
    auto issueA1 = [&](int kt, int slot, int i) {
        kt = kt < ksteps ? kt : ksteps - 1;
        dma16(asrc + (size_t)kt * (MT * 2 * 64) + i * 64, aring + (slot * AF + i) * 64);
    };
    auto issueB = [&](int ch, int buf) {
        ch = ch < nchunks ? ch : nchunks - 1;
// ... 31 lines not shown
            half8 ah[MTW], al[MTW], bh[4], bl[4];
#pragma unroll
            for (int i = 0; i < MTW; ++i) {
                ah[i] = __builtin_bit_cast(half8, LA[(2 * i) * 64]);
                al[i] = __builtin_bit_cast(half8, LA[(2 * i + 1) * 64]);
            }
#pragma unroll
            for (int ct = 0; ct < 4; ++ct) {
                bh[ct] = __builtin_bit_cast(half8, LB[ct * 256 + b_rd[kk][0]]);
                bl[ct] = __builtin_bit_cast(half8, LB[ct * 256 + b_rd[kk][1]]);
            }
            asm volatile("s_waitcnt lgkmcnt(0)" ::: "memory");
#pragma unroll
            for (int term = 0; term < 3; ++term)
#pragma unroll
                for (int i = 0; i < MTW; ++i) {
#pragma unroll
                    for (int ct = 0; ct < 4; ++ct) acc[i][ct] = MFMA16(term == 1 ? al[i] : ah[i], term == 2 ? bl[ct] : bh[ct], acc[i][ct]);
                    if (term == 0) {
                        issueA1(2 * c + kk + 3, sa, 2 * i);
                        issueA1(2 * c + kk + 3, sa, 2 * i + 1);
                    }
                }
            sa = sa + 1 == GW_DA ? 0 : sa + 1;
        }
        bb = bb + 1 == GW_NB ? 0 : bb + 1;
    }
    asm volatile("s_waitcnt vmcnt(0)" ::: "memory");

#pragma unroll
    for (int ct = 0; ct < 4; ++ct) {
        const int sample = b0 + 32 * ct + sl;
        if (sample >= count) continue;
#pragma unroll
        for (int i = 0; i < MTW; ++i) {
            const int mt = wave * MTW + i;
            float y[16];
#pragma unroll
            for (int g = 0; g < 4; ++g) {
                const f32x4 bv = *(const f32x4*)(bias + 32 * mt + 8 * g + 4 * h);
#pragma unroll
                for (int q = 0; q < 4; ++q) y[4 * g + q] = acc[i][ct][4 * g + q] + bv[q];
            }
            if (EPI == EPI_SPLIT) {
#pragma unroll
                for (int s = 0; s < 2; ++s) {
                    float v[8];
#pragma unroll
                    for (int j = 0; j < 8; ++j) v[j] = lrelu(y[8 * s + j]);
                    half8 hi, lo;
                    split8(v, hi, lo);
                    uint4* row = out_split + (size_t)sample * out_row_u4 + (size_t)(2 * mt + s) * 4;
                    row[h] = *(const uint4*)&hi;
                    row[2 + h] = *(const uint4*)&lo;
                }
            } else {
#pragma unroll
                for (int g = 0; g < 4; ++g) {
                    f32x4 o;
#pragma unroll
                    for (int q = 0; q < 4; ++q) o[q] = y[4 * g + q];
                    *(f32x4*)(out_logits + (size_t)sample * (MT * 32) + 32 * mt + 8 * g + 4 * h) = o;
                }
            }
        }
    }
}

__global__ __launch_bounds__(256) void k_splitk_finish(const float* __restrict__ part, int nsplit, size_t cap_rows,
                                                       const float* __restrict__ bias, uint4* __restrict__ out_split, size_t out_row_u4,
                                                       const int32_t* __restrict__ d_count, int max_count) {
    int count = d_count[0];
    if (count > max_count) count = max_count;
    const size_t i = (size_t)blockIdx.x * blockDim.x + threadIdx.x;
    const size_t sample = i >> 6;
    if (sample >= (size_t)count) return;
    const int piece = (int)(i & 63), mt = piece >> 2, s = (piece >> 1) & 1, h = piece & 1;
    const int n0 = 32 * mt + 16 * s + 4 * h;
    float v[8];
#pragma unroll
    for (int j = 0; j < 8; ++j) v[j] = 0.0f;
    for (int sp = 0; sp < nsplit; ++sp) {
        const float* p = part + ((size_t)sp * cap_rows + sample) * NF + n0;
        const f32x4 a = *(const f32x4*)p, b = *(const f32x4*)(p + 8);
#pragma unroll
        for (int j = 0; j < 4; ++j) { v[j] += a[j]; v[4 + j] += b[j]; }
    }
    const f32x4 ba = *(const f32x4*)(bias + n0), bb = *(const f32x4*)(bias + n0 + 8);
#pragma unroll
    for (int j = 0; j < 4; ++j) { v[j] = lrelu(v[j] + ba[j]); v[4 + j] = lrelu(v[4 + j] + bb[j]); }
    half8 hi, lo;
    split8(v, hi, lo);
    uint4* row = out_split + sample * out_row_u4 + (size_t)(2 * mt + s) * 4;
    row[h] = *(const uint4*)&hi;
    row[2 + h] = *(const uint4*)&lo;
}

__global__ __launch_bounds__(256) void k_splitk_logits(const float* __restrict__ part, int nsplit, size_t cap_rows, int width, const float* __restrict__ bias,
                                                       float* __restrict__ logits, const int32_t* __restrict__ d_count, int max_count) {
    int count = d_count[0];
    if (count > max_count) count = max_count;
    const size_t per_row = (size_t)width / 4, total = (size_t)count * per_row;
    for (size_t i = (size_t)blockIdx.x * blockDim.x + threadIdx.x; i < total; i += (size_t)gridDim.x * blockDim.x) {
        const size_t row = i / per_row, col = (i % per_row) * 4;
        f32x4 a = *(const f32x4*)(part + row * width + col);
        for (int sp = 1; sp < nsplit; ++sp) {
            const f32x4 b = *(const f32x4*)(part + ((size_t)sp * cap_rows + row) * width + col);
#pragma unroll
            for (int j = 0; j < 4; ++j) a[j] += b[j];
        }
        const f32x4 bv = *(const f32x4*)(bias + col);
#pragma unroll
        for (int j = 0; j < 4; ++j) a[j] += bv[j];
        *(f32x4*)(logits + row * width + col) = a;
    }
}

__global__ __launch_bounds__(64) void k_softmax(const float* __restrict__ logits, int lrow, int hw, int rowp, float* __restrict__ p,
                                                float* __restrict__ v, float* __restrict__ vpre, const int32_t* __restrict__ d_count, int max_count) {
    int count = d_count[0];
    if (count > max_count) count = max_count;
    const int lane = threadIdx.x;
    for (int s = blockIdx.x; s < count; s += gridDim.x) {
        const float* l = logits + (size_t)s * lrow;
        float mx = -INFINITY;
        for (int a = lane; a < hw; a += 64) mx = fmaxf(mx, l[a]);
        for (int o = 32; o > 0; o >>= 1) mx = fmaxf(mx, __shfl_xor(mx, o, 64));
        float sum = 0.0f, e[4] = {0.0f, 0.0f, 0.0f, 0.0f};
#pragma unroll
        for (int i = 0; i < 4; ++i) {
            const int a = lane + 64 * i;
            if (a < hw) { e[i] = expf(l[a] - mx); sum += e[i]; }
        }
        for (int o = 32; o > 0; o >>= 1) sum += __shfl_xor(sum, o, 64);
#pragma unroll
        for (int i = 0; i < 4; ++i) {
            const int a = lane + 64 * i;
            if (a < rowp) p[(size_t)s * rowp + a] = a < hw ? e[i] / sum : 0.0f;
        }
        if (lane == 0) { v[s] = tanhf(l[hw]); vpre[s] = l[hw]; }
    }
}

static inline void split_h(float x, _Float16& hi, _Float16& lo) {
    hi = (_Float16)x;
    lo = (_Float16)(x - (float)hi);
}
// ... 340 lines not shown
    hipStreamSynchronize(st);
    return 0;
}

template <int N, bool FROM_F32, bool BASE = false, bool DELTA = false, bool F16LO = false>
static void launch_trunk(Net& net, const Store& S, int max_count, hipStream_t st, const int32_t* row_list = nullptr, const int32_t* d_nrows = nullptr,
                         const int32_t* d_out_base = nullptr, const int32_t* d_nrows2 = nullptr, bool v2 = false, const BinPrefixArgs* role = nullptr) {
    using TG = TrunkGeo<N>;
    static bool attr_done[64] = {};
    auto kern = k_trunk<N, FROM_F32, BASE, DELTA, F16LO>;
    if (!attr_done[net.device & 63]) {
        hipFuncSetAttribute((const void*)kern, hipFuncAttributeMaxDynamicSharedMemorySize, TG::LDS_BYTES);
        attr_done[net.device & 63] = true;
    }
    const int wgs = (max_count + TG::SPW - 1) / TG::SPW;
    constexpr int ROLE_WGS = (BASE && DELTA) ? 1 : 0;
    const int grid = (wgs < 256 - ROLE_WGS ? wgs : 256 - ROLE_WGS) + ROLE_WGS;
    kern<<<grid, TG::WG_THREADS, TG::LDS_BYTES, st>>>(S.req_ref, S.req_aux, S.board, S.hdr, S.d_count, S.stride_nodes, net.in_f32, (const uint4*)net.wt_trunk, net.wt_first,
                                                       (uint4*)net.a_fc0, net.row_u4, max_count, row_list, d_nrows,
                                                       (BASE && DELTA) ? (const uint2*)net.d_comp : (const uint2*)net.d_groups, net.sib_h, d_out_base, (uint4*)net.a_base,
                                                       d_nrows2, v2 ? (uint4*)net.sib_h : nullptr, role ? *role : BinPrefixArgs{});
}

template <int N, bool FROM_F32, bool BASE = false, bool DELTA = false>
static void launch_trunk_fmt(Net& net, const Store& S, int max_count, hipStream_t st, const int32_t* row_list = nullptr, const int32_t* d_nrows = nullptr,
                             const int32_t* d_out_base = nullptr, const int32_t* d_nrows2 = nullptr, bool v2 = false, const BinPrefixArgs* role = nullptr) {
    if (net.fc0_fmt == FC0_F16) launch_trunk<N, FROM_F32, BASE, DELTA, true>(net, S, max_count, st, row_list, d_nrows, d_out_base, d_nrows2, v2, role);
    else launch_trunk<N, FROM_F32, BASE, DELTA, false>(net, S, max_count, st, row_list, d_nrows, d_out_base, d_nrows2, v2, role);
}

template <int MT, int EPI, int TAG, int NST = 3>
static void launch_gemm(const void* wp, const void* act, int ksteps, size_t act_row_u4, int k_full, int last_cnt, int lo_off,
                        const float* bias, void* out_split, size_t out_row_u4, float* out_logits, const Store& S, int max_count,
                        hipStream_t st, int device, int nsplit = 1) {
    constexpr int LDS = (MT * 2 + 8) * 1024 * NST;
    static bool attr_done[64] = {};
    auto kern = k_gemm_t<MT, EPI, TAG, NST>;
    if (!attr_done[device & 63]) {
        hipFuncSetAttribute((const void*)kern, hipFuncAttributeMaxDynamicSharedMemorySize, LDS);
        attr_done[device & 63] = true;
    }
    const dim3 grid((max_count + GT_BS - 1) / GT_BS, nsplit);
    kern<<<grid, 512, LDS, st>>>((const uint4*)wp, (const uint4*)act, ksteps, act_row_u4, k_full, last_cnt, lo_off, bias, (uint4*)out_split,
                                  out_row_u4, out_logits, S.d_count, max_count);
}

template <int MTH>
static void launch_tail_fused(const void* wp_fc1, const void* act, const float* bias_fc1, const void* wp_heads, const float* bias_heads, float* out_logits, const Store& S,
                              int max_count, hipStream_t st, int device) {
    constexpr int LDS = 160 * 1024;
    static bool attr_done[64] = {};
    auto kern = k_tail_fused<MTH>;
    if (!attr_done[device & 63]) {
        hipFuncSetAttribute((const void*)kern, hipFuncAttributeMaxDynamicSharedMemorySize, LDS);
        attr_done[device & 63] = true;
    }
    kern<<<dim3((max_count + GT_BS - 1) / GT_BS), 512, LDS, st>>>((const uint4*)wp_fc1, (const uint4*)act, bias_fc1, (const uint4*)wp_heads, bias_heads, out_logits, S.d_count,
                                                                 max_count);
}

template <int MT, int EPI>
static void launch_gemm_w(const void* wp, const void* act, int ksteps, size_t act_row_u4, const float* bias, void* out_split, size_t out_row_u4, float* out_logits,
                          const Store& S, int max_count, hipStream_t st, int device) {
    constexpr int LDS = gemm_w_lds(MT);
    static_assert(LDS <= 160 * 1024, "k_gemm_w LDS");
    static bool attr_done[64] = {};
    auto kern = k_gemm_w<MT, EPI>;
    if (!attr_done[device & 63]) {
        hipFuncSetAttribute((const void*)kern, hipFuncAttributeMaxDynamicSharedMemorySize, LDS);
        attr_done[device & 63] = true;
    }
    kern<<<dim3((max_count + GT_BS - 1) / GT_BS), 512, LDS, st>>>((const uint4*)wp, (const uint4*)act, ksteps, act_row_u4, bias, (uint4*)out_split, out_row_u4, out_logits,
                                                                 S.d_count, max_count);
}

constexpr int SIB_MAX_WWAYS = 14;
constexpr int SIB_MAX_FWAYS = 64;
__global__ void k_zero_ints(int32_t* __restrict__ p, int n) {
    for (int i = threadIdx.x; i < n; i += blockDim.x) p[i] = 0;
}
typedef void (*sib_kernel_t)(const uint64_t*, const uint4*, const float*, uint4*, size_t, const uint4*, const int32_t*, const float*, const uint32_t*, const int32_t*,
                             uint4*, uint2*, unsigned long long*);
static sib_kernel_t sib_kernel(bool delta, bool x16, int n) {
    if (n == 9) return delta ? (x16 ? k_sib_children<true, true, 9> : k_sib_children<true, false, 9>)
                             : (x16 ? k_sib_children<false, true, 9> : k_sib_children<false, false, 9>);
    return delta ? (x16 ? k_sib_children<true, true, 15> : k_sib_children<true, false, 15>)
                 : (x16 ? k_sib_children<false, true, 15> : k_sib_children<false, false, 15>);
}
typedef void (*sib2_kernel_t)(const uint64_t*, const uint4*, const float*, uint4*, size_t, const uint4*, const int32_t*, const uint4*, const uint32_t*, const int32_t*,
                              uint4*, uint2*, unsigned long long*, const uint4*);
static sib2_kernel_t sib2_kernel(bool x16, int n, bool mixed = false) {
    if (mixed) return n == 9 ? k_sib_children2<true, 9, false, false> : k_sib_children2<true, 15, false, false>;
    if (n == 9) return x16 ? k_sib_children2<true, 9> : k_sib_children2<false, 9>;
    return x16 ? k_sib_children2<true, 15> : k_sib_children2<false, 15>;
}
static void launch_trunk_siblings(Net& net, const Store& S, int side, int max_count, hipStream_t st, bool delta) {
    constexpr int LDS = TR_WBYTES + 4 * SIB_CGRID_BYTES + TR_SIDE_FLOATS * 4;
    static_assert(LDS + 32 <= 160 * 1024, "k_sib_children LDS (+ the static pair-barrier flags)");
    static bool attr_done[64] = {};
    if (!attr_done[net.device & 63]) {
        for (int d = 0; d < 2; ++d)
            for (int x = 0; x < 2; ++x)
                for (int n : {9, 15}) hipFuncSetAttribute((const void*)sib_kernel(d != 0, x != 0, n), hipFuncAttributeMaxDynamicSharedMemorySize, LDS);
        for (int x = 0; x < 3; ++x)
            for (int n : {9, 15}) hipFuncSetAttribute((const void*)sib2_kernel(x != 0, n, x == 2), hipFuncAttributeMaxDynamicSharedMemorySize, V2_LDS);
        attr_done[net.device & 63] = true;
// ... 148 lines not shown
    if (!net.fill_in_group) return;
    static bool said = false;
    if (!said) {
        said = true;
        fprintf(stderr, "omok_mi355x: internal inconsistency (recovered): the round's request-list fill was handed to the sibling path, but the forward (%s) does not take it; "
                        "the list is written here instead\n", where);
    }
    if (net.scan_cnt) launch_scan(net.n, S, net.fill_side, net.fill_k, st, net.scan_evals, nullptr, 0, true);
    else launch_fill(S, net.fill_side, net.fill_k, st);
    net.fill_in_group = net.gcnt_zeroed = false;
    net.scan_cnt = nullptr;
}
static int fc0_dense_nsplit(int rows, int nsup, int n_cu, size_t part_rows) {
    const int tiles128 = (rows + GT_BS - 1) / GT_BS;
    int nsplit = 1;
    double best = 1e30;
    constexpr int dmax = 64;
    for (int d = 1; d <= dmax; ++d) {
        const int per = (nsup + d - 1) / d;
        if ((d - 1) * per >= nsup) continue;
        if (d > 1 && (size_t)d * (size_t)(tiles128 * GT_BS) > part_rows) continue;
        const double waves = (double)(((size_t)tiles128 * d + n_cu - 1) / n_cu);
        const double cost = waves * (per + 4) * (d > 1 ? 1.04 : 1.0);
        if (cost < best - 1e-9) { best = cost; nsplit = d; }
    }
    return nsplit;
}
static int tail_tsplit(int rows, int n_cu, size_t part_rows) {
    const int tiles_t = (rows + GT_BS - 1) / GT_BS;
    int tsplit = 1;
    while (tsplit < 8 && tiles_t * tsplit * 2 <= n_cu && (size_t)(tsplit * 2) * (size_t)(tiles_t * GT_BS) <= part_rows) tsplit *= 2;
    return tsplit;
}
static void forward_f16x3(Net& net, const Store& S, int max_count, bool from_f32, hipStream_t st, Prof* prof, int sib_side = -1, bool skip_softmax = false) {
    const int hw = net.hw;
    const int use_sib = sib_env();
    const bool sib = sibling_path(net, from_f32, sib_side);
    if (!sib) recover_handed_over_fill(net, S, st, "forward_f16x3 on plain rows");
    const bool delta = sib && use_sib >= 2 && max_count >= sib_delta_min_rows(net);
    if (prof) prof->begin(PC_TRUNK, st);
    if (sib) launch_trunk_siblings(net, S, sib_side, max_count, st, delta);
    else if (net.n == 9) { if (from_f32) launch_trunk_fmt<9, true>(net, S, max_count, st); else launch_trunk_fmt<9, false>(net, S, max_count, st); }
    else {
        if (from_f32) launch_trunk_fmt<15, true>(net, S, max_count, st);
        else launch_trunk_fmt<15, false>(net, S, max_count, st);
    }
    if (prof) { prof->end(st); prof->begin(PC_FC0, st); }
    const float* bias_fc0 = net.wt_first + TR_SIDE_FLOATS;
    const float* bias_fc1 = bias_fc0 + NF;
    const float* bias_heads = bias_fc1 + NF;
    uint4* h0 = (uint4*)net.h0;
    const size_t mb = ((size_t)net.max_b + GT_BS - 1) / GT_BS * GT_BS;
    uint4* h1 = h0 + mb * 128;
    net.plan_path = sib ? (delta ? 2 : 1) : 0;
    net.plan_rows = max_count;
    net.plan_nsplit = 0;
    if (delta) launch_fc0_delta(net, max_count, bias_fc0, h0, st);
    else {
        const int nsup = hw * 2, tiles128 = (max_count + GT_BS - 1) / GT_BS;
        const int nsplit = net.plan_nsplit = fc0_dense_nsplit(max_count, nsup, net.n_cu, net.part_rows);
        if (nsplit == 1) launch_fc0<EPI_SPLIT, false>(net, net.fc0_fmt, tiles128, st, net.a_fc0, nsup, net.row_u4, bias_fc0, h0, 128, nullptr, S.d_count, max_count);
        else {
            const size_t cap_rows = (size_t)tiles128 * GT_BS;
            launch_fc0<EPI_PARTIAL, false>(net, net.fc0_fmt, (tiles128 * nsplit + 7) / 8 * 8, st, net.a_fc0, (nsup + nsplit - 1) / nsplit, net.row_u4, bias_fc0, nullptr, cap_rows,
                                           net.part, S.d_count, max_count);
            k_splitk_finish<<<(unsigned)(((size_t)max_count * 64 + 255) / 256), 256, 0, st>>>(net.part, nsplit, cap_rows, bias_fc0, h0, 128, S.d_count, max_count);
        }
    }
    if (prof) { prof->end(st); prof->begin(PC_TAIL, st); }
    const int MT = heads_mt(hw);
    const int tiles_t = (max_count + GT_BS - 1) / GT_BS;
    const int tsplit = net.plan_tsplit = tail_tsplit(max_count, net.n_cu, net.part_rows);
    const size_t cap_t = (size_t)tiles_t * GT_BS;
    const size_t fin_threads = (size_t)max_count * 64;
    if (tsplit == 1) {
        const char* gw_env = getenv("OMOK_GEMM_W");
        const bool gw = gw_env && gw_env[0] == '1';
        if (!gw) {
            if (MT == 8) launch_tail_fused<8>(net.wt_fc1, h0, bias_fc1, net.wt_heads, bias_heads, net.s0, S, max_count, st, net.device);
            else launch_tail_fused<4>(net.wt_fc1, h0, bias_fc1, net.wt_heads, bias_heads, net.s0, S, max_count, st, net.device);
        } else {
            launch_gemm_w<16, EPI_SPLIT>(net.wt_fc1, h0, 32, 128, bias_fc1, h1, 128, nullptr, S, max_count, st, net.device);
            if (MT == 8) launch_gemm_w<8, EPI_LOGITS>(net.wt_heads, h1, 32, 128, bias_heads, nullptr, 0, net.s0, S, max_count, st, net.device);
            else launch_gemm<4, EPI_LOGITS, 2>(net.wt_heads, h1, 32, 128, 32, 1, 2, bias_heads, nullptr, 0, net.s0, S, max_count, st, net.device);
        }
    } else {
        launch_gemm<16, EPI_PARTIAL, 1>(net.wt_fc1, h0, 32 / tsplit, 128, 32, 1, 2, bias_fc1, nullptr, cap_t, net.part, S, max_count, st, net.device, tsplit);
        k_splitk_finish<<<(unsigned)((fin_threads + 255) / 256), 256, 0, st>>>(net.part, tsplit, cap_t, bias_fc1, h1, 128, S.d_count, max_count);
        if (MT == 8) launch_gemm<8, EPI_PARTIAL, 2>(net.wt_heads, h1, 32 / tsplit, 128, 32, 1, 2, bias_heads, nullptr, cap_t, net.part, S, max_count, st, net.device, tsplit);
        else launch_gemm<4, EPI_PARTIAL, 2>(net.wt_heads, h1, 32 / tsplit, 128, 32, 1, 2, bias_heads, nullptr, cap_t, net.part, S, max_count, st, net.device, tsplit);
        const unsigned lg = (unsigned)(((size_t)max_count * (MT * 8) + 255) / 256);
        k_splitk_logits<<<lg < 2048 ? lg : 2048, 256, 0, st>>>(net.part, tsplit, cap_t, MT * 32, bias_heads, net.s0, S.d_count, max_count);
    }
    const int sg = max_count < 32768 ? max_count : 32768;
    if (!skip_softmax) k_softmax<<<sg, 64, 0, st>>>(net.s0, MT * 32, hw, net.rowp, net.p, net.v, net.vpre, S.d_count, max_count);
    if (prof) prof->end(st);
}

__device__ inline uint32_t probe_mix(uint32_t x) { x ^= x >> 16; x *= 0x7feb352dU; x ^= x >> 15; x *= 0x846ca68bU; x ^= x >> 16; return x; }
__global__ void k_probe_inputs(float* __restrict__ in, int hw, int rows, int row0) {
    const int i = blockIdx.x * blockDim.x + threadIdx.x;
    if (i >= rows * hw) return;
    const int r = i / hw, a = i % hw, gr = row0 + r;
    const uint32_t hr = probe_mix(0x9E3779B9u * (uint32_t)(gr + 1));
    const uint32_t kind = (uint32_t)gr % 5u;
    const uint32_t dens = kind < 2 ? (hr >> 8) % 40u : kind < 4 ? (hr >> 8) % 600u : (hr >> 8) % 1024u;
    const uint32_t hc = probe_mix(hr ^ (0x85EBCA6Bu * (uint32_t)(a + 1)));
    const bool occ = (hc & 1023u) < dens, black = (hc >> 10) & 1u;
    const int turn = (int)(hr & 1u);
    const bool mine = black == (turn == 0);
    float* o = in + (size_t)r * 3 * hw;
    o[2 * a] = occ && mine ? 1.0f : 0.0f;
    o[2 * a + 1] = occ && !mine ? 1.0f : 0.0f;
    o[2 * hw + a] = turn == 0 ? 1.0f : 0.0f;
}

__global__ __launch_bounds__(64) void k_probe_store(Store S, int n, int pk) {
    const int t = blockIdx.x, lane = threadIdx.x, hw = n * n, nw = (hw + 63) / 64;
    const uint32_t hr = probe_mix(0x9E3779B9u * (uint32_t)(t + 7919));
    const uint32_t kind = (uint32_t)t % 5u;
    const uint32_t dens = kind < 2 ? (hr >> 8) % 40u : (hr >> 8) % 500u;
    const int turn = (int)(hr & 1u);
    uint64_t bw[4] = {0, 0, 0, 0}, ww[4] = {0, 0, 0, 0};
    int stones = 0;
    for (int j = 0; j < nw; ++j) {
// ... 179 lines not shown
    auto contract = [](const ProbeErr& e) { return e.dp <= NET_PROBE_CONTRACT && e.dv <= NET_PROBE_CONTRACT && e.dl <= NET_PROBE_CONTRACT; };
    const ProbeErr& cp = plain[chosen == FC0_FP6 ? 0 : 1];
    const ProbeErr& cr = rounds[chosen == FC0_FP6 ? 0 : chosen == FC0_MIXED ? 1 : 2];
    net.probe_outside = (inside(cp) && (!have_rounds || inside(cr))) ? 0 : (contract(cp) && (!have_rounds || contract(cr))) ? 1 : 2;
    if (net.probe_outside) {
        static bool said[3] = {};
        if (!said[net.probe_outside]) {
            said[net.probe_outside] = true;
            fprintf(stderr, "omok_mi355x: net_commit: the %s operand format measures |dp| %.2e |dv| %.2e |dlogit| %.2e on plain rows%s against the fp32 kernels (max |logit| %.0f): %s\n",
                    chosen == FC0_FP6 ? "fp6" : chosen == FC0_MIXED ? "mixed" : "f16", cp.dp, cp.dv, cp.dl, have_rounds ? " (+ a sibling round)" : "", lmax,
                    net.probe_outside == 1 ? "outside the probe's margin (3e-4 / 5e-4), inside the 1e-3 contract -- committed (OMOK_STAT_PROBE_OUTSIDE = 1)"
                                           : "OUTSIDE the 1e-3 contract with the most precise split-operand format -- this net is evaluated with the fp32 kernels (slow; OMOK_STAT_PROBE_OUTSIDE = 2)");
        }
    }
    net.probe[0] = (float)R;
    net.probe[1] = plain[0].dp; net.probe[2] = plain[0].dv;
    net.probe[3] = plain[1].dp; net.probe[4] = plain[1].dv;
    net.probe[5] = lmax;
    net.probe[6] = 1.0f;
    net.probe[7] = plain[0].dl; net.probe[8] = plain[1].dl;
    net.probe[9] = (float)checked;
    for (int k = 0; k < 3; ++k) { net.probe[10 + 3 * k] = rounds[k].dp; net.probe[11 + 3 * k] = rounds[k].dv; net.probe[12 + 3 * k] = rounds[k].dl; }
    static const bool verbose = getenv("OMOK_PROBE_LOG") && atoi(getenv("OMOK_PROBE_LOG"));
    if (verbose)
        fprintf(stderr, "[net probe] N=%d plain rows %d: fp6 |dp| %.2e |dv| %.2e |dlogit| %.2e, f16 %.2e %.2e %.2e (max |logit| %.1f); sibling round of %d rows (%d checked): "
                        "fp6 %.2e %.2e %.2e, mixed %.2e %.2e %.2e, f16 %.2e %.2e %.2e -> %s\n", net.n, R, plain[0].dp, plain[0].dv, plain[0].dl, plain[1].dp, plain[1].dv, plain[1].dl,
                lmax, round_rows, checked, rounds[0].dp, rounds[0].dv, rounds[0].dl, rounds[1].dp, rounds[1].dv, rounds[1].dl, rounds[2].dp, rounds[2].dv, rounds[2].dl,
                chosen == FC0_FP6 ? "fp6" : chosen == FC0_MIXED ? "mixed" : "f16");
    return 0;
}

bool net_logits_cover_batch(const Net& net, int max_count) { return net.mode != OMOK_NET_F32 && max_count <= net.max_b; }

void net_forward_requests(Net& net, const Store& S, int max_count, hipStream_t st, Prof* prof, int sibling_side, bool skip_softmax) {
    if (max_count <= 0) return;
    if (max_count > net.max_b) max_count = net.max_b;
    if (net.mode == OMOK_NET_F32) {
        recover_handed_over_fill(net, S, st, "fp32 kernels");
        launch_encode_requests(net.n, S, net.in_f32, max_count, st);
        forward_f32(net, S, max_count, st, prof);
        net.plan_path = 3; net.plan_rows = max_count; net.plan_nsplit = net.plan_tsplit = 0;
    } else {
        forward_f16x3(net, S, max_count, false, st, prof, sibling_side, skip_softmax);
    }
}

void net_forward_inputs(Net& net, const Store& S, int count, hipStream_t st, Prof* prof) {
    if (count <= 0) return;
    if (net.mode == OMOK_NET_F32) {
        forward_f32(net, S, count, st, prof);
        net.plan_path = 3; net.plan_rows = count; net.plan_nsplit = net.plan_tsplit = 0;
    } else forward_f16x3(net, S, count, true, st, prof);
}

}
```

omok-ai_amd/csrc/tree_kernels.hip:

```cpp
#include "common.h"
#include <type_traits>

namespace omok {

#define LANE ((int)(threadIdx.x & 63))

struct U4 { uint32_t x, y, z, w; };

__device__ inline U4 philox(uint64_t seed, uint32_t c0, uint32_t c1, uint32_t c2, uint32_t c3) {
    uint32_t k0 = (uint32_t)seed, k1 = (uint32_t)(seed >> 32);
#pragma unroll
    for (int r = 0; r < 10; ++r) {
        const uint32_t h0 = __umulhi(0xD2511F53u, c0), l0 = 0xD2511F53u * c0;
        const uint32_t h1 = __umulhi(0xCD9E8D57u, c2), l1 = 0xCD9E8D57u * c2;
        const uint32_t n0 = h1 ^ c1 ^ k0, n2 = h0 ^ c3 ^ k1;
        c0 = n0; c1 = l1; c2 = n2; c3 = l0;
        k0 += 0x9E3779B9u;
        k1 += 0xBB67AE85u;
    }
    return U4{c0, c1, c2, c3};
}

__device__ inline double det_log(double x) {
    const unsigned long long b = (unsigned long long)__double_as_longlong(x);
// ... 303 lines not shown
    }
    const int idx = (int)R.n_nodes++;
    if (lane == 0) {
        const size_t slot = (size_t)tab * G::ROWP + action;
        T.corder[slot] = (uint8_t)hp.nch;
        T.cidx[slot] = (uint16_t)idx;
        T.cn[slot] = 0u;
        T.cw[slot] = 0.0f;
        T.hdr[parent].nch = (uint16_t)(hp.nch + 1);
        NodeHdr c;
        c.parent = (uint16_t)parent;
        c.table = NONE16;
        c.legal = (uint16_t)(hp.legal - 1);
        c.nch = 0;
        c.action = (uint8_t)action;
        c.status = (uint8_t)status;
        c.turn = (uint8_t)turn;
        c.has_policy = (uint8_t)has_policy;
        c.pad = 0;
        T.hdr[idx] = c;
    }
    if (lane < 2 * G::NW) {
        uint64_t w = bb[0];
#pragma unroll
        for (int i = 1; i < 2 * G::NW; ++i) w = lane == i ? bb[i] : w;
        T.board[(size_t)idx * (2 * G::NW) + lane] = w;
    }
    R.bytes += 24 + 8 * 2 * G::NW;
    hp.table = (uint16_t)tab;
    hp.nch = (uint16_t)(hp.nch + 1);
    return idx;
}

template <int N>
__device__ void apply_noise(const Tree<N>& T, const RoundArgs& A, uint32_t tree_global, float* s_row) {
    using G = Geo<N>;
    const int lane = LANE;
    NodeHdr h0 = T.hdr[0];
    uint64_t bb[2 * G::NW];
#pragma unroll
    for (int i = 0; i < 2 * G::NW; ++i) bb[i] = T.board[i];
#pragma unroll
    for (int j = 0; j < G::IT; ++j) {
        const int a = j * 64 + lane;
        s_row[a] = a < G::HW ? gamma_draw(A.alpha, A.seed, (uint32_t)a, (uint32_t)A.ply, tree_global) : 0.0f;
    }
    __syncthreads();
    const float total = seq_sum(s_row, G::HW);
    __syncthreads();
    const bool ok = total > 0.0f;
    const float inv = ok ? __fdiv_rn(1.0f, total) : 0.0f;
    const float ph = h0.legal ? __fdiv_rn(1.0f, (float)h0.legal) : 0.0f;
#pragma unroll
    for (int j = 0; j < G::IT; ++j) {
        const int a = j * 64 + lane;
        float m = 0.0f;
        if (a < G::HW) {
            const float noise = ok ? s_row[a] * inv : __fdiv_rn(1.0f, (float)G::HW);
            const bool empty = !(((bb[j] | bb[G::NW + j]) >> lane) & 1ULL);
            const float p = h0.has_policy ? T.pol[a] : (empty ? ph : 0.0f);
            m = (1.0f - A.epsilon) * p + A.epsilon * noise;
        }
        s_row[a] = m;
    }
    __syncthreads();
    const float sum = seq_sum(s_row, G::HW);
    const float sum_inv = __fdiv_rn(1.0f, sum);
#pragma unroll
    for (int j = 0; j < G::IT; ++j) {
        const int a = j * 64 + lane;
        T.pol[a] = a < G::HW ? s_row[a] * sum_inv : 0.0f;
    }
    if (lane == 0 && !h0.has_policy) T.hdr[0].has_policy = 1;
    __syncthreads();
}

constexpr int PR_LEVELS = 3;
struct PathRec {
    int tab[PR_LEVELS], act[PR_LEVELS];
    uint32_t n[PR_LEVELS];
    float w[PR_LEVELS];
    int depth;
};
__device__ inline int uni(int v) { return __builtin_amdgcn_readfirstlane(v); }
__device__ inline NodeHdr uni(const NodeHdr& h) {
    uint4 q = __builtin_bit_cast(uint4, h);
    q.x = (uint32_t)uni((int)q.x); q.y = (uint32_t)uni((int)q.y); q.z = (uint32_t)uni((int)q.z); q.w = (uint32_t)uni((int)q.w);
    return __builtin_bit_cast(NodeHdr, q);
}

template <int N, bool REC>
__device__ inline void select_leaf_impl(const Tree<N>& T, NodeHdr& h, int& node, uint32_t& node_n, unsigned long long& path_bytes, PathRec& rec) {
    using G = Geo<N>;
    constexpr int ROWP = G::ROWP;
    const int lane = LANE;
    int lev = 0;
    while (h.nch == h.legal && h.nch != 0) {
        const uint32_t pn = node_n > 1u ? node_n : 1u;
        const float sq = __fsqrt_rn((float)pn);
        const size_t tb = (size_t)h.table * ROWP;
        const float ph = __fdiv_rn(1.0f, (float)h.legal);
        unsigned long long best = 0ULL;
        uint8_t ordv[G::IT];
        uint32_t nv[G::IT];
        uint16_t civ[G::IT];
        float wv[G::IT], pv[G::IT];
#pragma unroll
        for (int j = 0; j < G::IT; ++j) {
            const int a = j * 64 + lane;
            ordv[j] = T.corder[tb + a];
            nv[j] = T.cn[tb + a];
            wv[j] = T.cw[tb + a];
            pv[j] = h.has_policy ? T.pol[(size_t)node * ROWP + a] : ph;
            civ[j] = T.cidx[tb + a];
        }
#pragma unroll
        for (int j = 0; j < G::IT; ++j) {
            const int a = j * 64 + lane;
            const uint8_t ord = ordv[j];
            if (ord != NONE8) {
                const uint32_t n = nv[j];
                const float w = wv[j];
                const float p = pv[j];
                const float q = __fdiv_rn(w, (float)n + F32_EPS);
                const float bias = __fdiv_rn(sq, (float)(1u + n));
                const float score = q + (1.0f * p) * bias;
                const unsigned long long v = ((unsigned long long)total_key_biased(score) << 32) |
                                             ((unsigned long long)ord << 16) | (unsigned long long)a;
                best = v > best ? v : best;
            }
        }
        best = wave_max_u64(best);
        const int a_best = (int)(best & 0xFFFFu);
        path_bytes += 12ull * h.nch;
        {
            uint32_t n_sel = nv[0], c_sel = civ[0];
            float w_sel = wv[0];
#pragma unroll
            for (int j = 1; j < G::IT; ++j) {
                n_sel = (a_best >> 6) == j ? nv[j] : n_sel;
                c_sel = (a_best >> 6) == j ? (uint32_t)civ[j] : c_sel;
                w_sel = (a_best >> 6) == j ? wv[j] : w_sel;
            }
            node_n = (uint32_t)__shfl((int)n_sel, a_best & 63, 64);
            node = __shfl((int)c_sel, a_best & 63, 64);
            if (REC) {
                const float w_best = __shfl(w_sel, a_best & 63, 64);
#pragma unroll
                for (int l = 0; l < PR_LEVELS; ++l)
                    if (l == lev) {
                        rec.tab[l] = uni((int)h.table);
                        rec.act[l] = uni(a_best);
                        rec.n[l] = (uint32_t)uni((int)node_n);
                        rec.w[l] = __builtin_bit_cast(float, uni(__builtin_bit_cast(int, w_best)));
                    }
            }
        }
        h = T.hdr[node];
        lev += 1;
    }
    if (REC) rec.depth = lev;
}
template <int N>
__device__ inline void select_leaf(const Tree<N>& T, NodeHdr& h, int& node, uint32_t& node_n, unsigned long long& path_bytes) {
    PathRec none;
    select_leaf_impl<N, false>(T, h, node, node_n, path_bytes, none);
}

template <int N>
__device__ inline bool five_in_pair(const uint64_t* own, int a, int pr) {
    constexpr int NW = Geo<N>::NW;
    const int dx = pr == 1 ? 0 : -1, dy = pr == 0 ? 0 : (pr == 3 ? 1 : -1);
    const int x0 = a % N, y0 = a / N;
    int run_a = 0, run_b = 0;
    bool on_a = true, on_b = true;
#pragma unroll
    for (int k = 1; k <= 5; ++k) {
        const int xa = x0 + dx * k, ya = y0 + dy * k, xb = x0 - dx * k, yb = y0 - dy * k;
        const bool in_a = xa >= 0 && xa < N && ya >= 0 && ya < N, in_b = xb >= 0 && xb < N && yb >= 0 && yb < N;
        on_a = on_a && in_a && get_bit<NW>(own, in_a ? ya * N + xa : 0) != 0;
        on_b = on_b && in_b && get_bit<NW>(own, in_b ? yb * N + xb : 0) != 0;
        run_a += on_a ? 1 : 0;
        run_b += on_b ? 1 : 0;
    }
    return 1 + run_a + run_b == 5;
}
__device__ inline int nth_set_bit_lane(uint64_t w, int r) {
    uint64_t cur = w;
    int base = 0;
#pragma unroll
    for (int sh = 32; sh >= 1; sh >>= 1) {
        const uint64_t low = cur & ((1ULL << sh) - 1ULL);
        const int c = __popcll(low);
        const bool up = r >= c;
        r -= up ? c : 0;
        base += up ? sh : 0;
        cur = up ? (cur >> sh) : low;
    }
    return base;
}

template <int N>
__device__ void run_sim(const Store& S, const Tree<N>& T, Regs& R, LeafCache<N>& C, const RoundArgs& A, uint32_t sim_index,
                        uint32_t tree_global) {
    using G = Geo<N>;
    constexpr int ROWP = G::ROWP, NW = G::NW;
    const int lane = LANE;
    int node = 0;
    uint32_t node_n = R.root_n;
    unsigned long long path_bytes = 0;
    if (R.memo_node >= 0) {
        node = R.memo_node;
        node_n = R.memo_n;
        path_bytes = R.memo_bytes;
    } else C.node = -1;
    const bool cached = C.node == node;
    NodeHdr h;
    if (cached) h = C.h;
    else { fence_own_stores(R); h = T.hdr[node]; }
    if (h.nch == h.legal && h.nch != 0) { fence_own_stores(R); C.node = -1; }
    select_leaf<N>(T, h, node, node_n, path_bytes);
    R.bytes += path_bytes;
    R.memo_node = node;
    R.memo_n = node_n;
    R.memo_bytes = path_bytes;
    if (h.status != ST_IN_PROGRESS) {
        fence_own_stores(R);
        backup<N>(T, R, node, h.status >= ST_BLACK_WIN ? 1.0f : 0.0f);
        R.memo_node = -1;
        C.node = -1;
        __syncthreads();
        return;
    }
    uint64_t bb[2 * NW];
    unsigned long long cand[G::IT];
    int total = 0;
    if (C.node == node) {
#pragma unroll
        for (int i = 0; i < 2 * NW; ++i) bb[i] = C.bb[i];
#pragma unroll
        for (int j = 0; j < G::IT; ++j) { cand[j] = C.cand[j]; total += __popcll(cand[j]); }
    } else {
        fence_own_stores(R);
#pragma unroll
        for (int i = 0; i < 2 * NW; ++i) bb[i] = T.board[(size_t)node * (2 * NW) + i];
#pragma unroll
        for (int j = 0; j < G::IT; ++j) {
            const int a = j * 64 + lane;
            bool c = a < G::HW && !(((bb[j] | bb[NW + j]) >> lane) & 1ULL);
            if (c && h.table != NONE16) c = T.corder[(size_t)h.table * ROWP + a] == NONE8;
            cand[j] = __ballot(c);
            total += __popcll(cand[j]);
        }
        C.node = node;
// ... 5 lines not shown
    const U4 o = philox(A.seed, sim_index, (uint32_t)A.ply, tree_global, RNG_EXPAND);
    int r = (int)__umulhi(o.x, (uint32_t)total);
    int action = 0;
    bool found = false;
#pragma unroll
    for (int j = 0; j < G::IT; ++j) {
        const int c = __popcll(cand[j]);
        if (!found) {
            if (r < c) { action = j * 64 + nth_set_bit(cand[j], r); found = true; }
            else r -= c;
        }
    }
    const int status = place_and_status<N>(bb, h.turn, h.legal, action);
    const int child = add_child<N>(S, T, R, node, h, action, bb, status, 1 - h.turn, 0);
    if (child < 0) { C.node = -1; return; }
    R.dirty = true;
    C.h = h;
#pragma unroll
    for (int j = 0; j < G::IT; ++j) C.cand[j] = cand[j] & ~((action >> 6) == j ? (1ULL << (action & 63)) : 0ULL);
    if (status != ST_IN_PROGRESS) {
        fence_own_stores(R);
        backup<N>(T, R, child, status == ST_DRAW ? 0.0f : 1.0f);
        R.memo_node = -1;
        C.node = -1;
        __syncthreads();
    } else {
        if (lane == 0) T.req[R.n_req] = (uint16_t)child;
        R.n_req += 1u;
        R.bytes += 4 + (G::HW + 2);
    }
}

template <int N>
__device__ void run_sims(const Store& S, const Tree<N>& T, Regs& R, LeafCache<N>& C, const RoundArgs& A, uint32_t first_sim, int count, uint32_t tree_global) {
    using G = Geo<N>;
    constexpr int ROWP = G::ROWP, NW = G::NW;
    const int lane = LANE;
    int done = 0;
#ifdef KROUND_PROF
    unsigned long long (&kp)[8] = R.kp;
    unsigned long long& kp_last = R.kp_last;
#endif
    PathRec rec;
    rec.depth = -1;
    NodeHdr root_h;
    bool root_ok = false;
    while (done < count) {
        int node = 0;
        uint32_t node_n = R.root_n;
        unsigned long long path_bytes = 0;
        if (R.memo_node >= 0) {
            node = R.memo_node;
            node_n = R.memo_n;
            path_bytes = R.memo_bytes;
        } else C.node = -1;
        NodeHdr h;
        const bool from_root = R.memo_node < 0;
        if (C.node == node) h = C.h;
        else if (from_root && root_ok) h = root_h;
        else {
            fence_own_stores(R);
            h = T.hdr[node];
            if (from_root) { root_h = uni(h); root_ok = true; }
        }
        if (h.nch == h.legal && h.nch != 0) { fence_own_stores(R); C.node = -1; }
        if (from_root) select_leaf_impl<N, true>(T, h, node, node_n, path_bytes, rec);
        else {
            select_leaf<N>(T, h, node, node_n, path_bytes);
            rec.depth = -1;
        }
        KP(2);
        R.memo_node = node;
        R.memo_n = node_n;
        R.memo_bytes = path_bytes;
        if (h.status != ST_IN_PROGRESS) {
            R.bytes += path_bytes;
            if (rec.depth >= 0 && rec.depth <= PR_LEVELS) {
                float v = h.status >= ST_BLACK_WIN ? 1.0f : 0.0f;
#pragma unroll
                for (int l = PR_LEVELS - 1; l >= 0; --l)
                    if (l < rec.depth) {
                        if (lane == 0) {
                            const size_t slot = (size_t)rec.tab[l] * ROWP + rec.act[l];
                            T.cn[slot] = rec.n[l] + 1u;
                            T.cw[slot] = rec.w[l] + v;
                        }
                        v = -v;
                        R.bytes += 16;
                    }
                R.root_n += 1u;
                R.root_w += v;
                R.bytes += 16;
                R.dirty = true;
            } else {
                fence_own_stores(R);
                backup<N>(T, R, node, h.status >= ST_BLACK_WIN ? 1.0f : 0.0f);
                __syncthreads();
            }
            R.memo_node = -1;
            C.node = -1;
            done += 1;
            KP(3);
            continue;
// ... 141 lines not shown
        if (lane < n_new_req) T.req[R.n_req + lane] = (uint16_t)(idx0 + lane);
        R.n_req += (uint32_t)n_new_req;
        R.bytes += (sim_bytes + 24 + 8 * 2 * NW) * (unsigned long long)n_commit + (unsigned long long)(4 + (G::HW + 2)) * (unsigned long long)n_new_req;
        R.dirty = true;
        h.table = (uint16_t)tab;
        h.nch = (uint16_t)(h.nch + n_commit);
        if (node == 0) root_ok = false;
        if (term_status != ST_IN_PROGRESS) {
            fence_own_stores(R);
            backup<N>(T, R, idx0 + n_commit - 1, term_status == ST_DRAW ? 0.0f : 1.0f);
            R.memo_node = -1;
            C.node = -1;
            __syncthreads();
        } else {
            C.h = h;
#pragma unroll
            for (int j = 0; j < G::IT; ++j) C.cand[j] = cand[j];
        }
        KP(7);
        done += n_commit;
    }
}

#ifndef KROUND_BATCH
#define KROUND_BATCH 1
#endif
#ifndef KROUND_WPS
#define KROUND_WPS 4
#endif
template <int N>
__global__ __launch_bounds__(64, KROUND_WPS) void k_round(Store S, RoundArgs A) {
    using G = Geo<N>;
    __shared__ float s_row[G::ROWP];
    const int g = blockIdx.x;
    const int t = A.side * S.games + g;
    if (A.zero_ptr && g == 0)
        for (int i = LANE; i < A.zero_n; i += 64) A.zero_ptr[i] = 0;
    const Tree<N> T(S, t);
    const GameState gs0 = S.gs[g];
    const TreeState ts = *T.ts;
    if (!gs0.alive) {
        if (A.req_cnt && LANE == 0) A.req_cnt[g] = 0;
        return;
    }
    Regs R{ts.n_nodes, ts.n_tables, ts.root_n, 0u, ts.error, ts.root_w, 0ull};
#ifdef KROUND_PROF
    unsigned long long (&kp)[8] = R.kp;
    unsigned long long& kp_last = R.kp_last;
    kp_last = __builtin_readcyclecounter();
#endif
    if (A.scatter_v && ts.n_req > 0) {
        scatter_tree<N>(S, T, ts, R, A.scatter_v);
        R.dirty = true;
    }
    A.ply = gs0.plies;
    const uint32_t tree_global = (uint32_t)((A.game_offset + gs0.gid) * 2 + A.side);
    KP(0);
    if (A.round == 0) apply_noise<N>(T, A, tree_global, s_row);
    KP(1);
    LeafCache<N> C;
    if (KROUND_BATCH) run_sims<N>(S, T, R, C, A, (uint32_t)(A.round * A.K), A.K, tree_global);
    else for (int i = 0; i < A.K; ++i) run_sim<N>(S, T, R, C, A, (uint32_t)(A.round * A.K + i), tree_global);
    if (LANE == 0) {
        TreeState o = ts;
        o.n_nodes = R.n_nodes; o.n_tables = R.n_tables; o.root_n = R.root_n; o.root_w = R.root_w;
        o.error = R.error; o.n_req = R.n_req;
        *T.ts = o;
        if (A.req_cnt) A.req_cnt[g] = (int32_t)R.n_req;
        atomicAdd(S.d_bytes, R.bytes);
#ifdef KROUND_PROF
        const unsigned int L = (unsigned int)A.round & 63u;
        if (t < 8192)
            for (int i = 0; i < 8; ++i) g_kprof[L][t][i] = kp[i];
#endif
    }
}
#ifdef KROUND_PROF
extern "C" void omok_debug_kround_prof(unsigned long long* out ) {
    hipDeviceSynchronize();
    hipMemcpyFromSymbol(out, HIP_SYMBOL(g_kprof), sizeof(unsigned long long) * 64 * 8192 * 8);
    static unsigned long long zero[1] = {0};
    (void)zero;
}
#endif

__device__ inline void wave_fence() {
    __builtin_amdgcn_fence(__ATOMIC_SEQ_CST, "workgroup");
    __builtin_amdgcn_wave_barrier();
}
__device__ inline void tree_lock(int* lock) {
    if (LANE == 0)
        while (atomicCAS(lock, 0, 1) != 0) __builtin_amdgcn_s_sleep(2);
    wave_fence();
}
__device__ inline void tree_unlock(int* lock) {
    wave_fence();
    if (LANE == 0) atomicExch(lock, 0);
}

template <int N>
__device__ inline void backup_shared(const Tree<N>& T, int x, float v) {
    constexpr int ROWP = Geo<N>::ROWP;
// ... 358 lines not shown
                    const bool empty = a < hw && !((occ[i][jj] >> lane) & 1ULL);
                    if (a < hw) srow[i * hw + a] = empty ? p : 0.0f;
                }
            }
        }
        __syncthreads();
        if (lane < nreq) {
            float acc = 0.0f;
#pragma unroll 15
            for (int a = 0; a < hw; ++a) acc += srow[lane * hw + a];
            const bool renorm = F32_EPS <= acc;
            sinv[lane] = renorm ? __fdiv_rn(1.0f, acc) : 0.0f;
        }
        __syncthreads();
#pragma unroll
        for (int i = 0; i < SSP_BATCH; ++i) {
            if (i < nreq) {
                const float inv = sinv[i];
                const bool renorm = inv != 0.0f;
#pragma unroll
                for (int jj = 0; jj < G::IT; ++jj) {
                    const int a = jj * 64 + lane;
                    const float r = a < hw ? srow[i * hw + a] : 0.0f;
                    S.policy[tn[i] * ROWP + a] = renorm ? r * inv : r;
                }
                if (lane == 0) S.hdr[tn[i]].has_policy = 1;
            }
        }
        __syncthreads();
    }
}

template <int N>
__device__ inline void scatter_tree(const Store& S, const Tree<N>& T, const TreeState& ts, Regs& R, const float* __restrict__ V) {
    using G = Geo<N>;
    constexpr int ROWP = G::ROWP;
    const int lane = LANE, nreq = (int)ts.n_req;
    int x = 0, par = -1 - lane, act = 0;
    float val = 0.0f;
    if (lane < nreq) {
        x = (int)T.req[lane];
        const NodeHdr hx = T.hdr[x];
        par = (int)hx.parent;
        act = (int)hx.action;
        val = V[(size_t)ts.req_base + lane];
    }
    const int prev_par = __shfl_up(par, 1, 64);
    unsigned long long rem = __ballot(lane < nreq && (lane == 0 || par != prev_par));
    while (rem) {
        const int s0 = __ffsll((long long)rem) - 1;
        rem &= rem - 1ULL;
        const int s1 = rem ? __ffsll((long long)rem) - 1 : nreq;
        const int leaf = __shfl(par, s0, 64);
        int depth = 0;
        size_t my_slot = 0;
        uint32_t my_n = 0;
        float my_w = 0.0f;
        bool fits = true;
        {
            int y = leaf;
            while (y != 0) {
                const NodeHdr h = T.hdr[y];
                const size_t slot = (size_t)T.hdr[h.parent].table * ROWP + h.action;
                const uint32_t n = T.cn[slot];
                const float w = T.cw[slot];
                if (lane == depth) { my_slot = slot; my_n = n; my_w = w; }
                y = h.parent;
                depth += 1;
                if (depth >= 64) { fits = y == 0; break; }
            }
        }
        if (fits) {
            const size_t tab_leaf = (size_t)T.hdr[leaf].table * ROWP;
            if (lane >= s0 && lane < s1) {
                const size_t slot = tab_leaf + act;
                const uint32_t n = T.cn[slot] + 1u;
                const float w = T.cw[slot] + (-val);
                T.cn[slot] = n;
                T.cw[slot] = w;
            }
            float root_w = R.root_w;
            const float sgn_root = (depth & 1) ? -1.0f : 1.0f;
            for (int r = s0; r < s1; ++r) {
                const float v = __shfl(val, r, 64);
                if (lane < depth) { my_n += 1u; my_w += (lane & 1) ? -v : v; }
                root_w += sgn_root * v;
            }
            if (lane < depth) { T.cn[my_slot] = my_n; T.cw[my_slot] = my_w; }
            R.root_n += (uint32_t)(s1 - s0);
            R.root_w = root_w;
            R.bytes += (unsigned long long)(s1 - s0) * (16ull * (unsigned long long)(depth + 1) + 16ull + 8ull * G::HW + 4ull);
            if (rem) __syncthreads();
        } else {
            for (int r = s0; r < s1; ++r) {
                backup<N>(T, R, (int)T.req[r], -V[(size_t)ts.req_base + (uint32_t)r]);
                __syncthreads();
                R.bytes += 8ull * G::HW + 4;
            }
        }
    }
}

template <int N>
__global__ __launch_bounds__(64) void k_scatter(Store S, int side, const float* __restrict__ V) {
    const int g = blockIdx.x;
    if (!S.gs[g].alive) return;
    const int t = side * S.games + g;
    const Tree<N> T(S, t);
    const TreeState ts = *T.ts;
    if (ts.n_req == 0) return;
    Regs R{ts.n_nodes, ts.n_tables, ts.root_n, 0u, ts.error, ts.root_w, 0ull};
    scatter_tree<N>(S, T, ts, R, V);
    if (LANE == 0) {
        TreeState o = ts;
        o.root_n = R.root_n; o.root_w = R.root_w; o.n_req = 0;
        *T.ts = o;
        atomicAdd(S.d_bytes, R.bytes);
    }
}

template <int N>
__global__ __launch_bounds__(64) void k_reset(Store S, const float* __restrict__ root_policy) {
    using G = Geo<N>;
    const int t = blockIdx.x;
    const int lane = LANE;
    const Tree<N> T(S, t);
#pragma unroll
    for (int j = 0; j < G::IT; ++j) {
        const int a = j * 64 + lane;
        T.pol[a] = a < G::HW ? root_policy[a] : 0.0f;
    }
    if (lane < 2 * G::NW) T.board[lane] = 0ULL;
    if (lane == 0) {
        NodeHdr h;
        h.parent = NONE16; h.table = NONE16; h.legal = (uint16_t)G::HW; h.nch = 0;
        h.action = NONE8; h.status = ST_IN_PROGRESS; h.turn = 0; h.has_policy = 1; h.pad = 0;
        T.hdr[0] = h;
        TreeState s{1u, 0u, 0u, 0.0f, 0u, 0u, 0u, 0u};
        *T.ts = s;
        if (t < S.games) {
            GameState gs{};
            gs.alive = 1; gs.status = ST_IN_PROGRESS; gs.last_action = -1; gs.mirror_idx = -1; gs.gid = t;
            S.gs[t] = gs;
        }
    }
}

template <int N, bool MATCH>
__global__ __launch_bounds__(64) void k_reset_from(Store S, const uint8_t* __restrict__ boards, const float* __restrict__ P, const float* __restrict__ P2,
                                                   int split) {
// ... 693 lines not shown
    for (int k = 0; k < nt; ++k) {
        const int d = s_tmap[k];
        if (d == NONE16) continue;
        uint32_t vn[G::IT];
        float vw[G::IT];
        uint16_t vi[G::IT];
        uint8_t vo[G::IT];
#pragma unroll
        for (int j = 0; j < G::IT; ++j) {
            const size_t s = (size_t)k * ROWP + j * 64 + lane;
            vn[j] = T.cn[s]; vw[j] = T.cw[s]; vi[j] = T.cidx[s]; vo[j] = T.corder[s];
        }
        const uint16_t own = s_nmap[T.owner[k]];
        __syncthreads();
#pragma unroll
        for (int j = 0; j < G::IT; ++j) {
            const size_t s = (size_t)d * ROWP + j * 64 + lane;
            T.cn[s] = vn[j]; T.cw[s] = vw[j]; T.corder[s] = vo[j];
            T.cidx[s] = vo[j] != NONE8 ? s_nmap[vi[j]] : (uint16_t)0;
        }
        if (lane == 0) T.owner[d] = own;
        __syncthreads();
    }
    if (lane == 0) {
        TreeState o = ts;
        o.n_nodes = (uint32_t)new_nodes; o.n_tables = (uint32_t)new_tables; o.root_n = new_n; o.root_w = new_w;
        *T.ts = o;
    }
    __syncthreads();
    return 0;
}

template <int N>
__device__ void ensure_action_exists(const Store& S, const Tree<N>& T, int action, const float* __restrict__ p_row, float* s_row) {
    using G = Geo<N>;
    constexpr int ROWP = G::ROWP, NW = G::NW;
    const int lane = LANE;
    const NodeHdr h0 = T.hdr[0];
    uint64_t bb[2 * NW];
#pragma unroll
    for (int i = 0; i < 2 * NW; ++i) bb[i] = T.board[i];
    bool renorm;
    float inv;
    masked_policy_row<N>(bb, action, p_row, s_row, renorm, inv);
    const bool exists = h0.table != NONE16 && T.corder[(size_t)h0.table * ROWP + action] != NONE8;
    if (!exists) {
        const TreeState ts = *T.ts;
        Regs R{ts.n_nodes, ts.n_tables, ts.root_n, 0u, ts.error, ts.root_w, 0ull};
        if (!get_bit<NW>(bb, action) && !get_bit<NW>(bb + NW, action)) (void)place_and_status<N>(bb, h0.turn, h0.legal, action);
        NodeHdr h0m = h0;
        const int idx = add_child<N>(S, T, R, 0, h0m, action, bb, ST_IN_PROGRESS, 1 - h0.turn, 1);
        if (idx >= 0) {
#pragma unroll
            for (int j = 0; j < G::IT; ++j) {
                const int a = j * 64 + lane;
                const float x = s_row[a];
                T.pol[(size_t)idx * ROWP + a] = renorm ? x * inv : x;
            }
        }
        if (lane == 0) {
            TreeState o = ts;
            o.n_nodes = R.n_nodes; o.n_tables = R.n_tables; o.error = R.error;
            *T.ts = o;
        }
    }
    __syncthreads();
}

template <int N>
__global__ __launch_bounds__(64) void k_advance(Store S, int side, const float* __restrict__ P) {
    using G = Geo<N>;
    constexpr int ROWP = G::ROWP, NW = G::NW;
    extern __shared__ __attribute__((aligned(16))) unsigned char smem[];
    float* s_row = (float*)smem;
    uint16_t* s_nmap = (uint16_t*)(smem + ROWP * 4);
    uint16_t* s_tmap = s_nmap + S.cap_nodes;
    uint8_t* s_alive = (uint8_t*)(s_tmap + S.cap_tables);
    const int g = blockIdx.x;
    const int lane = LANE;
    const GameState gs = S.gs[g];
    if (!gs.alive || gs.last_action < 0) return;
    const int action = gs.last_action;
    const Tree<N> own(S, side * S.games + g);
    const Tree<N> opp(S, (1 - side) * S.games + g);
    if (gs.external) ensure_action_exists<N>(S, own, action, P + (size_t)gs.mirror_idx * ROWP, s_row);
    ensure_action_exists<N>(S, opp, action, P + (size_t)gs.mirror_idx * ROWP, s_row);
    int status;
    {
        const NodeHdr h0 = own.hdr[0];
        uint64_t bb[2 * NW];
#pragma unroll
        for (int i = 0; i < 2 * NW; ++i) bb[i] = own.board[i];
        status = place_and_status<N>(bb, h0.turn, h0.legal, action);
    }
    int err = 0;
    if (transition<N>(S, own, action, s_alive, s_nmap, s_tmap) != 0) err |= 16;
    if (transition<N>(S, opp, action, s_alive, s_nmap, s_tmap) != 0) err |= 32;
    if (lane == 0) {
        if (err) own.ts->error |= (uint32_t)err;
        GameState o = gs;
        if (!gs.external) {
            if (gs.rp_len < G::HW)
                S.rp_z[(size_t)g * G::HW + gs.rp_len] = (status == ST_BLACK_WIN || status == ST_WHITE_WIN) ? 1.0f : 0.0f;
            o.rp_len = gs.rp_len + 1;
        }
        o.external = 0;
        o.plies = gs.plies + 1;
        o.status = (uint8_t)status;
        o.alive = status == ST_IN_PROGRESS ? 1 : 0;
        o.last_action = -1;
        o.mirror_idx = -1;
        S.gs[g] = o;
    }
}

template <int N>
__device__ inline void load_request_board(const Store& S, uint32_t ref, uint32_t aux, uint64_t* bb, int& turn, int& mode) {
    constexpr int NW = Geo<N>::NW;
    const int t = (int)(ref >> 16), node = (int)(ref & 0xFFFFu);
// ... 379 lines not shown
                   uint8_t* boards_out, int32_t* status_out, int32_t* played_out, hipStream_t st) {
    DISPATCH_N(n, (k_replay<9><<<batch, 64, 0, st>>>(start, verdict, moves, lengths, stride, upto, boards_out, status_out, played_out)),
               (k_replay<15><<<batch, 64, 0, st>>>(start, verdict, moves, lengths, stride, upto, boards_out, status_out, played_out)));
}
void launch_root_stats(const Store& S, int side, uint32_t* n_dev, float* w_dev, hipStream_t st) {
    k_root_stats<<<(S.games + 255) / 256, 256, 0, st>>>(S, side, n_dev, w_dev);
}
void launch_round(int n, const Store& S, const RoundArgs& a, hipStream_t st) {
    DISPATCH_N(n, (k_round<9><<<S.games, 64, 0, st>>>(S, a)), (k_round<15><<<S.games, 64, 0, st>>>(S, a)));
}
void launch_round_shared(int n, const Store& S, const RoundArgs& a, int rounds_total, int group, int waves, uint16_t* sh_req, uint32_t* sh_cnt,
                         hipStream_t st, uint8_t* rec_order, uint32_t* rec_pos) {
    DISPATCH_N(n, (k_round_shared<9><<<1, waves * 64, 0, st>>>(S, a, rounds_total, group, sh_req, sh_cnt, rec_order, rec_pos)),
               (k_round_shared<15><<<1, waves * 64, 0, st>>>(S, a, rounds_total, group, sh_req, sh_cnt, rec_order, rec_pos)));
    k_scan_shared<<<1, 64, 0, st>>>(S, a.side, waves, sh_req, sh_cnt);
}
void launch_scatter_shared(int n, const Store& S, int side, const float* p, const float* v, int max_count, int waves, const uint16_t* sh_req,
                           const uint32_t* sh_cnt, hipStream_t st, uint8_t* rec_order, uint32_t* rec_pos) {
    const int grid = max_count > 0 ? max_count : 1;
    DISPATCH_N(n, (k_scatter_policy<9><<<grid, 64, 0, st>>>(S, p, max_count)), (k_scatter_policy<15><<<grid, 64, 0, st>>>(S, p, max_count)));
    DISPATCH_N(n, (k_scatter_shared<9><<<1, waves * 64, 0, st>>>(S, side, v, sh_req, sh_cnt, rec_order, rec_pos)),
               (k_scatter_shared<15><<<1, waves * 64, 0, st>>>(S, side, v, sh_req, sh_cnt, rec_order, rec_pos)));
}
void launch_fill(const Store& S, int side, int K, hipStream_t st) { k_fill<<<(S.games * K + 255) / 256, 256, 0, st>>>(S, side, K); }
void launch_scan(int n, const Store& S, int side, int K, hipStream_t st, unsigned long long* evals, int32_t* zero_ptr, int zero_n, bool fill) {
    k_scan<<<1, 1024, 0, st>>>(S, side, evals, zero_ptr, zero_ptr ? zero_n : 0);
    if (fill) launch_fill(S, side, K, st);
}
void launch_scatter(int n, const Store& S, int side, const float* p, const float* v, int max_count, hipStream_t st, bool backups) {
    const int grid = max_count < 8192 ? (max_count > 0 ? max_count : 1) : 8192;
    DISPATCH_N(n, (k_scatter_policy<9><<<grid, 64, 0, st>>>(S, p, max_count)), (k_scatter_policy<15><<<grid, 64, 0, st>>>(S, p, max_count)));
    if (backups) launch_backups(n, S, side, v, st);
}
void launch_backups(int n, const Store& S, int side, const float* v, hipStream_t st) {
    DISPATCH_N(n, (k_scatter<9><<<S.games, 64, 0, st>>>(S, side, v)), (k_scatter<15><<<S.games, 64, 0, st>>>(S, side, v)));
}
void launch_softmax_scatter(int n, const Store& S, int side, const float* logits, int lrow, float* v, float* vpre, int max_count, hipStream_t st,
                            bool backups) {
    const int nb = (max_count + SSP_BATCH - 1) / SSP_BATCH;
    const int grid = nb < 8192 ? (nb > 0 ? nb : 1) : 8192;
    DISPATCH_N(n, (k_softmax_scatter_policy<9><<<grid, 64, 0, st>>>(S, logits, lrow, v, vpre, max_count)),
               (k_softmax_scatter_policy<15><<<grid, 64, 0, st>>>(S, logits, lrow, v, vpre, max_count)));
    if (backups) launch_backups(n, S, side, v, st);
}
void launch_sample(int n, const Store& S, int side, int ply, float temperature, int threshold, uint64_t seed,
                   int64_t game_offset, int32_t* actions, hipStream_t st) {
    DISPATCH_N(n, (k_sample<9><<<S.games, 64, 0, st>>>(S, side, ply, temperature, threshold, seed, game_offset, actions)),
               (k_sample<15><<<S.games, 64, 0, st>>>(S, side, ply, temperature, threshold, seed, game_offset, actions)));
}
void launch_mirror_scan(int n, const Store& S, int side, hipStream_t st) { k_mirror_scan<<<1, 1024, 0, st>>>(S, side); }
void launch_advance(int n, const Store& S, int side, const float* p, hipStream_t st) {
    const size_t lds = advance_lds_bytes(S.cap_nodes, S.cap_tables);
    DISPATCH_N(n, (k_advance<9><<<S.games, 64, lds, st>>>(S, side, p)), (k_advance<15><<<S.games, 64, lds, st>>>(S, side, p)));
}
void launch_encode_requests(int n, const Store& S, float* out, int max_b, hipStream_t st) {
    if (max_b <= 0) return;
    DISPATCH_N(n, (k_encode_requests<9><<<max_b, 256, 0, st>>>(S, out, max_b)), (k_encode_requests<15><<<max_b, 256, 0, st>>>(S, out, max_b)));
}
void launch_env_play(int n, const int32_t* moves, int batch, int len, int32_t* status, uint8_t* boards, uint8_t* turns,
                     uint16_t* legal, hipStream_t st) {
    DISPATCH_N(n, (k_env_play<9><<<batch, 64, 0, st>>>(moves, len, status, boards, turns, legal)),
               (k_env_play<15><<<batch, 64, 0, st>>>(moves, len, status, boards, turns, legal)));
}
void launch_encode_boards(int n, const uint8_t* boards, const uint8_t* turns, int batch, int mode, float* out, hipStream_t st) {
    DISPATCH_N(n, (k_encode_boards<9><<<batch, 256, 0, st>>>(boards, turns, mode, out)),
               (k_encode_boards<15><<<batch, 256, 0, st>>>(boards, turns, mode, out)));
}
void launch_replay_offsets(int n, const Store& S, int per_transition, long long* offsets, hipStream_t st) {
    DISPATCH_N(n, (k_replay_offsets<9><<<1, 64, 0, st>>>(S, per_transition, offsets)), (k_replay_offsets<15><<<1, 64, 0, st>>>(S, per_transition, offsets)));
}
void launch_set_actions(int n, const Store& S, int side, const int32_t* actions, uint32_t* flags, hipStream_t st) {
    const int grid = (S.games + 255) / 256;
    DISPATCH_N(n, (k_set_actions<9><<<grid, 256, 0, st>>>(S, side, actions, flags)), (k_set_actions<15><<<grid, 256, 0, st>>>(S, side, actions, flags)));
}
void launch_clear_actions(const Store& S, hipStream_t st) { k_clear_actions<<<(S.games + 255) / 256, 256, 0, st>>>(S); }
void launch_opponent_move(int n, const Store& S, int side, int kind, uint64_t seed, int64_t game_offset, int32_t* actions, hipStream_t st) {
    DISPATCH_N(n, (k_opponent_move<9><<<S.games, 64, 0, st>>>(S, side, kind, seed, game_offset, actions)),
               (k_opponent_move<15><<<S.games, 64, 0, st>>>(S, side, kind, seed, game_offset, actions)));
}
void launch_env_scripted(int n, const uint8_t* boards, int kind, int batch, int32_t* forced, hipStream_t st) {
    DISPATCH_N(n, (k_env_scripted<9><<<batch, 64, 0, st>>>(boards, kind, forced)), (k_env_scripted<15><<<batch, 64, 0, st>>>(boards, kind, forced)));
}
void launch_policy(int n, const Store& S, int side, float* pi, uint8_t* has, hipStream_t st) {
    DISPATCH_N(n, (k_policy<9><<<S.games, 64, 0, st>>>(S, side, pi, has)), (k_policy<15><<<S.games, 64, 0, st>>>(S, side, pi, has)));
}
void launch_env_place(int n, uint8_t* boards, uint8_t* turns, uint16_t* legal, const int32_t* actions, int batch, int32_t* status, hipStream_t st) {
// ... 53 lines not shown
```

Baseline: 601.0 games/s.

## Defer policy softmax to node descent with raw logits written directly into tree

The policy GEMM epilogue writes raw logits straight into per-node policy rows, and value/tanh into the request buffers. Expanded nodes are marked POLICY_RAW, and the masked softmax is computed only when a node is first descended into or receives root noise. A materialise kernel normalises raw nodes before host-visible reads. This removes the separate softmax-scatter pass and the softmax work for leaves that are never revisited, at the cost of extra branching and lazy work inside the tree kernel.

```diff
diff --git a/bindings/omok_mi355x.rs b/bindings/omok_mi355x.rs
--- a/bindings/omok_mi355x.rs
+++ b/bindings/omok_mi355x.rs
@@ -185,6 +185,8 @@
         pub fn omok_debug_set_base_cache(e: *mut OmokEngine, enabled: i32) -> c_int;
         pub fn omok_debug_set_children_kernel(e: *mut OmokEngine, which: i32) -> c_int;
         pub fn omok_debug_set_window_rects(e: *mut OmokEngine, enabled: i32) -> c_int;
+        pub fn omok_debug_set_lazy_policy(e: *mut OmokEngine, enabled: i32) -> c_int;
+        pub fn omok_debug_lazy_policy_stats(e: *mut OmokEngine, out: *mut u64) -> c_int;
         pub fn omok_debug_last_plan(e: *mut OmokEngine, out: *mut i32, cap: i32) -> c_int;
         pub fn omok_get_stats(e: *mut OmokEngine, stats: *mut f64) -> c_int;
         pub fn omok_reset_stats(e: *mut OmokEngine) -> c_int;
diff --git a/include/omok_mi355x.h b/include/omok_mi355x.h
--- a/include/omok_mi355x.h
+++ b/include/omok_mi355x.h
@@ -164,6 +164,8 @@
 int omok_debug_set_base_cache(omok_engine* e, int32_t enabled);
 int omok_debug_set_children_kernel(omok_engine* e, int32_t which);
 int omok_debug_set_window_rects(omok_engine* e, int32_t enabled);
+int omok_debug_set_lazy_policy(omok_engine* e, int32_t enabled);
+int omok_debug_lazy_policy_stats(omok_engine* e, uint64_t* out);
 #define OMOK_PLAN_INTS 16
 int omok_debug_last_plan(omok_engine* e, int32_t* out, int32_t cap);
 
diff --git a/omok-ai_amd/api.py b/omok-ai_amd/api.py
--- a/omok-ai_amd/api.py
+++ b/omok-ai_amd/api.py
@@ -241,6 +241,14 @@
 
     def set_base_cache(self, on=True):
         self._chk(B.lib().omok_debug_set_base_cache(self.h, int(bool(on))))
+
+    def set_lazy_policy(self, on=True):
+        self._chk(B.lib().omok_debug_set_lazy_policy(self.h, int(bool(on))))
+
+    def lazy_policy_stats(self):
+        out = (C.c_uint64 * 2)()
+        self._chk(B.lib().omok_debug_lazy_policy_stats(self.h, out))
+        return {"noise": int(out[0]), "descent": int(out[1])}
 
     def set_window_rects(self, on=True):
         self._chk(B.lib().omok_debug_set_window_rects(self.h, int(bool(on))))
diff --git a/omok-ai_amd/binding.py b/omok-ai_amd/binding.py
--- a/omok-ai_amd/binding.py
+++ b/omok-ai_amd/binding.py
@@ -43,6 +43,7 @@
     "omok_game_log_enable", "omok_game_log_read", "omok_env_replay",
     "omok_replay_augment_records_dev",
     "omok_selfplay_run_slots_logged", "omok_game_log_entry_bytes",
+    "omok_debug_set_lazy_policy", "omok_debug_lazy_policy_stats",
 ]
 
 
@@ -104,6 +105,9 @@
     L.omok_debug_set_base_cache.argtypes = [H, C.c_int32]
     L.omok_debug_set_children_kernel.argtypes = [H, C.c_int32]
     L.omok_debug_set_window_rects.argtypes = [H, C.c_int32]
+    if hasattr(L, "omok_debug_set_lazy_policy"):
+        L.omok_debug_set_lazy_policy.argtypes = [H, C.c_int32]
+        L.omok_debug_lazy_policy_stats.argtypes = [H, C.POINTER(C.c_uint64)]
     L.omok_debug_last_plan.argtypes = [H, ip, C.c_int32]
     L.omok_set_episode.argtypes = [H, C.c_uint64]
     L.omok_env_place_stone.argtypes = [H, u8p, u8p, C.POINTER(C.c_uint16), ip, C.c_int32, ip]
diff --git a/omok-ai_amd/csrc/common.h b/omok-ai_amd/csrc/common.h
--- a/omok-ai_amd/csrc/common.h
+++ b/omok-ai_amd/csrc/common.h
@@ -91,6 +91,8 @@
     int32_t* req_cnt;
     int32_t* zero_ptr;
     int zero_n;
+    int lazy_rows;
+    uint32_t* lazy_stats;
 };
 
 void launch_reset(int n, const Store& S, const float* root_policy_dev , hipStream_t st);
@@ -128,13 +130,14 @@
 constexpr int MAX_GAMES = 32767;
 constexpr int SCAN_GAMES_PER_THREAD = 32;
 void launch_scatter(int n, const Store& S, int side, const float* p_dev, const float* v_dev, int max_count, hipStream_t st, bool backups = true);
-void launch_backups(int n, const Store& S, int side, const float* v_dev, hipStream_t st);
+void launch_backups(int n, const Store& S, int side, const float* v_dev, hipStream_t st, int raw_rows = 0);
+void launch_materialise(int n, const Store& S, int tree_first, int trees, hipStream_t st);
 void launch_softmax_scatter(int n, const Store& S, int side, const float* logits_dev, int lrow, float* v_dev, float* vpre_dev, int max_count,
                             hipStream_t st, bool backups = true);
 void launch_sample(int n, const Store& S, int side, int ply, float temperature, int threshold, uint64_t seed,
                    int64_t game_offset, int32_t* actions_dev, hipStream_t st);
 void launch_mirror_scan(int n, const Store& S, int side, hipStream_t st);
-void launch_advance(int n, const Store& S, int side, const float* p_dev, hipStream_t st);
+void launch_advance(int n, const Store& S, int side, const float* p_dev, hipStream_t st, bool raw = false);
 void launch_encode_requests(int n, const Store& S, float* out_dev , int max_b, hipStream_t st);
 void launch_env_play(int n, const int32_t* moves_dev, int batch, int len, int32_t* status_dev, uint8_t* boards_dev,
                      uint8_t* turns_dev, uint16_t* legal_dev, hipStream_t st);
diff --git a/omok-ai_amd/csrc/engine.cpp b/omok-ai_amd/csrc/engine.cpp
--- a/omok-ai_amd/csrc/engine.cpp
+++ b/omok-ai_amd/csrc/engine.cpp
@@ -83,6 +83,8 @@
     int32_t* d_actions = nullptr;
     uint32_t* d_error = nullptr;
     unsigned long long* d_evals = nullptr;
+    uint32_t* d_lazy = nullptr;
+    bool lazy_policy = true;
     int32_t* d_req_cnt = nullptr;
     uint16_t* d_sh_req = nullptr;
     uint32_t* d_sh_cnt = nullptr;
@@ -304,6 +306,7 @@
     rc |= dalloc(e, &e->d_error, 4);
     rc |= dalloc(e, &e->d_evals, 2);
     rc |= dalloc(e, &e->d_req_cnt, G);
+    rc |= dalloc(e, &e->d_lazy, 4);
     rc |= dalloc(e, &e->d_sh_req, (size_t)MAX_TREE_WAVES * KMAX);
     rc |= dalloc(e, &e->d_sh_cnt, 2 * (size_t)KMAX);
     rc |= dalloc(e, &e->d_flags, 4);
@@ -319,6 +322,7 @@
     hipMemsetAsync(S.d_bytes, 0, 16, e->st);
     hipMemsetAsync(e->d_error, 0, 16, e->st);
     hipMemsetAsync(e->d_evals, 0, 16, e->st);
+    hipMemsetAsync(e->d_lazy, 0, 16, e->st);
     hipMemsetAsync(S.gs, 0, sizeof(GameState) * G, e->st);
     hipMemsetAsync(S.ts, 0, sizeof(TreeState) * T, e->st);
     if (set_advance_lds_attribute(e->n, advance_lds_bytes(cfg->max_nodes, cfg->max_tables)) != 0) {
@@ -526,14 +530,14 @@
         if (block_live(e, b)) out[n++] = Block{&net_at(e, tree_side ^ b), block_view(e, b), pending ? e->match_cnt[b] : rows, b ? e->match_cnt[0] : 0, b};
     return n;
 }
-static void block_forward(omok_engine* e, const Block& B, int max_count, int sibling_side = -1, bool skip_softmax = false) {
+static void block_forward(omok_engine* e, const Block& B, int max_count, int sibling_side = -1, bool skip_softmax = false, bool rows_to_nodes = false) {
     Net& X = *B.net;
     if (e->match) {
         X.grp_lo = B.b ? e->split : 0;
         X.grp_hi = B.b ? e->cfg.games : e->split;
         X.grp_sub = B.b ? e->d_mcnt : nullptr;
     }
-    net_forward_requests(X, B.view, max_count, e->st, &e->prof, sibling_side, skip_softmax);
+    net_forward_requests(X, B.view, max_count, e->st, &e->prof, sibling_side, skip_softmax, rows_to_nodes);
     if (e->match) {
         X.grp_hi = -1;
         X.grp_sub = nullptr;
@@ -986,10 +990,16 @@
 
 static Net& backup_net(omok_engine* e, int side) { return e->match ? net_at(e, side) : e->net; }
 
-static void forward_and_scatter(omok_engine* e, const Block& B, int side, int rows_cap, bool backups_inline) {
+static int lazy_round_rows(const omok_engine* e, int rows_cap) {
+    if (!e->lazy_policy || e->match || !net_logits_cover_batch(e->net, rows_cap) || !net_rows_fit_policy(e->net)) return 0;
+    return rows_cap;
+}
+
+static void forward_and_scatter(omok_engine* e, const Block& B, int side, int rows_cap, bool backups_inline, bool lazy = false) {
     Net& X = *B.net;
     const bool fused = net_logits_cover_batch(X, rows_cap);
-    block_forward(e, B, rows_cap, side, fused);
+    block_forward(e, B, rows_cap, side, fused, lazy);
+    if (lazy) return;
     e->prof.begin(PC_TREE_OTHER, e->st);
     if (fused) {
         int lrow = 0;
@@ -1000,12 +1010,13 @@
 }
 
 static void enqueue_round(omok_engine* e, int round, int K, float eps, float alpha, bool eval_and_scatter, int alive, bool defer_backups = false,
-                          bool pending_backups = false) {
+                          bool pending_backups = false, bool lazy = false, int pending_raw_rows = 0) {
     const int side = e->ply & 1;
     const int max_req = std::min(alive * K, e->net.max_b);
     const bool sib_round = !e->match && eval_and_scatter && net_round_takes_sibling_path(e->net, max_req);
     RoundArgs a{side, round, K, e->ply, eps, alpha, e->key, e->cfg.game_offset, pending_backups ? backup_net(e, side).v : nullptr,
-                sib_round ? e->d_req_cnt : nullptr, sib_round ? e->net.d_gcnt : nullptr, sib_round ? NET_GCNT_INTS : 0};
+                sib_round ? e->d_req_cnt : nullptr, sib_round ? e->net.d_gcnt : nullptr, sib_round ? NET_GCNT_INTS : 0,
+                pending_backups ? pending_raw_rows : 0, e->d_lazy};
     e->prof.round_begin();
     e->prof.begin(PC_ROUND, e->st);
     launch_round(e->n, e->S, a, e->st);
@@ -1024,7 +1035,7 @@
     if (eval_and_scatter) {
         Block blk[2];
         const int nb = eval_blocks(e, side, alive * K, false, blk);
-        for (int i = 0; i < nb; ++i) forward_and_scatter(e, blk[i], side, alive * K, !e->match && !defer_backups);
+        for (int i = 0; i < nb; ++i) forward_and_scatter(e, blk[i], side, alive * K, !e->match && !defer_backups, lazy);
         if (e->match) {
             e->prof.begin(PC_TREE_OTHER, e->st);
             match_join(e, side, false, max_req);
@@ -1035,16 +1046,17 @@
     e->prof.round_end();
 }
 
-static int enqueue_execute(omok_engine* e, int count, int K, float eps, float alpha, int alive) {
+static int enqueue_execute(omok_engine* e, int count, int K, float eps, float alpha, int alive, bool run_loop = false) {
     int processed = 0, round = 0;
+    const int raw_rows = run_loop ? lazy_round_rows(e, alive * K) : 0;
     while (processed < count) {
-        enqueue_round(e, round, K, eps, alpha, true, alive, true, round > 0);
+        enqueue_round(e, round, K, eps, alpha, true, alive, true, round > 0, raw_rows > 0, raw_rows);
         processed += K;
         round += 1;
     }
     if (round > 0) {
         e->prof.begin(PC_TREE_OTHER, e->st);
-        launch_backups(e->n, e->S, e->ply & 1, backup_net(e, e->ply & 1).v, e->st);
+        launch_backups(e->n, e->S, e->ply & 1, backup_net(e, e->ply & 1).v, e->st, raw_rows);
         e->prof.end(e->st);
     }
     return round;
@@ -1106,6 +1118,7 @@
     if (read_status(e, &bits, &alive)) return OMOK_ERR_HIP;
     const int side = e->ply & 1;
     RoundArgs a{side, 0, 0, e->ply, epsilon, alpha, e->key, e->cfg.game_offset};
+    launch_materialise(e->n, e->S, side * e->cfg.games, 1, e->st);
     e->prof.begin(PC_ROUND, e->st);
     launch_round(e->n, e->S, a, e->st);
     e->prof.end(e->st);
@@ -1198,15 +1211,17 @@
     if (e->log_on && e->log_started) launch_log_move(e->n, e->S, side, e->start_ply, e->log, e->st);
 }
 
-static void enqueue_advance(omok_engine* e, int max_rows) {
+static void enqueue_advance(omok_engine* e, int max_rows, bool raw = false) {
     const int side = e->ply & 1;
     if (e->match) match_join(e, 1 - side, true, max_rows);
     enqueue_log_move(e, side);
-    launch_advance(e->n, e->S, side, backup_net(e, 1 - side).p, e->st);
+    int lrow = 0;
+    launch_advance(e->n, e->S, side, raw ? net_logits(e->net, &lrow) : backup_net(e, 1 - side).p, e->st, raw);
     invalidate_nets(e);
 }
 
-static void enqueue_mirror_and_advance(omok_engine* e, int alive) {
+static void enqueue_mirror_and_advance(omok_engine* e, int alive, bool run_loop = false) {
+    const bool raw = run_loop && lazy_round_rows(e, alive) > 0;
     const int side = e->ply & 1;
     e->prof.begin(PC_PLY, e->st);
     launch_mirror_scan(e->n, e->S, side, e->st);
@@ -1215,9 +1230,9 @@
     e->prof.end(e->st);
     Block blk[2];
     const int nb = eval_blocks(e, 1 - side, alive, false, blk);
-    for (int i = 0; i < nb; ++i) block_forward(e, blk[i], alive);
+    for (int i = 0; i < nb; ++i) block_forward(e, blk[i], alive, -1, raw);
     e->prof.begin(PC_PLY, e->st);
-    enqueue_advance(e, alive);
+    enqueue_advance(e, alive, raw);
     e->prof.end(e->st);
 }
 
@@ -1226,11 +1241,11 @@
 static void play_ply(omok_engine* e, const Search& s, int alive, int scripted = -1) {
     if (scripted >= 0) enqueue_opponent_move(e, scripted);
     else {
-        const int rounds = enqueue_execute(e, s.count, s.K, s.epsilon, s.alpha, alive);
+        const int rounds = enqueue_execute(e, s.count, s.K, s.epsilon, s.alpha, alive, true);
         enqueue_sample(e, s.temperature, s.threshold);
         e->sims += (double)rounds * s.K * alive;
     }
-    enqueue_mirror_and_advance(e, alive);
+    enqueue_mirror_and_advance(e, alive, true);
 }
 
 static int end_ply(omok_engine* e, uint32_t* alive, bool count_finished = true) {
@@ -1486,6 +1501,7 @@
     const size_t t = (size_t)side * e->cfg.games + game, rp = (size_t)e->rowp, nw2 = 2 * (size_t)e->nw;
     const size_t tn = t * (size_t)e->S.stride_nodes, tt = t * (size_t)e->S.stride_tables;
     NodeHdr h0;
+    launch_materialise(e->n, e->S, (int)t, 1, e->st);
     HIPCHK(e, hipMemcpyAsync(&h0, e->S.hdr + tn, sizeof(h0), hipMemcpyDeviceToHost, e->st));
     if (sync_and_check(e, "root_children")) return OMOK_ERR_HIP;
     if (h0.table == NONE16 || h0.nch == 0) return 0;
@@ -1859,6 +1875,7 @@
     if (!e || !ints || !floats || game < 0 || game >= e->cfg.games || (side != 0 && side != 1)) return OMOK_ERR_INVALID;
     ENTER(e);
     const size_t t = (size_t)side * e->cfg.games + game;
+    launch_materialise(e->n, e->S, (int)t, 1, e->st);
     TreeState ts;
     HIPCHK(e, hipMemcpyAsync(&ts, e->S.ts + t, sizeof(ts), hipMemcpyDeviceToHost, e->st));
     if (sync_and_check(e, "tree_dump")) return OMOK_ERR_HIP;
@@ -2042,6 +2059,22 @@
     if (!e) return OMOK_ERR_INVALID;
     e->net.base_cache = enabled != 0;
     net_invalidate_sibling_cache(e->net);
+    return OMOK_OK;
+}
+
+extern "C" int omok_debug_set_lazy_policy(omok_engine* e, int32_t enabled) {
+    if (!e) return OMOK_ERR_INVALID;
+    e->lazy_policy = enabled != 0;
+    return OMOK_OK;
+}
+extern "C" int omok_debug_lazy_policy_stats(omok_engine* e, uint64_t* out) {
+    if (!e || !out) return OMOK_ERR_INVALID;
+    ENTER(e);
+    uint32_t c[2] = {0, 0};
+    HIPCHK(e, hipMemcpyAsync(c, e->d_lazy, sizeof(c), hipMemcpyDeviceToHost, e->st));
+    if (sync_and_check(e, "lazy_policy_stats")) return OMOK_ERR_HIP;
+    out[0] = c[0];
+    out[1] = c[1];
     return OMOK_OK;
 }
 
diff --git a/omok-ai_amd/csrc/net.h b/omok-ai_amd/csrc/net.h
--- a/omok-ai_amd/csrc/net.h
+++ b/omok-ai_amd/csrc/net.h
@@ -129,7 +129,15 @@
 constexpr int NET_GCNT_P0 = 8 + 81 + 7 + 16;
 constexpr int NET_GCNT_INTS = NET_GCNT_P0 + 225;
 constexpr int NET_WORK_DIFF = 0, NET_WORK_COPY = 3, NET_WORK_DIFF_FULL = 6, NET_WORK_WIN_PIXELS = 7, NET_WORK_WIN_TILES = 8, NET_WORK_FULL_TILES = 9, NET_WORK_COUNT = 16;
-void net_forward_requests(Net& net, const Store& S, int max_count, hipStream_t st, struct Prof* prof, int sibling_side = -1, bool skip_softmax = false);
+void net_forward_requests(Net& net, const Store& S, int max_count, hipStream_t st, struct Prof* prof, int sibling_side = -1, bool skip_softmax = false,
+                          bool rows_to_nodes = false);
+bool net_rows_fit_policy(const Net& net);
+struct LogitsDst {
+    const uint32_t* req_ref;
+    float* policy;
+    float *v, *vpre;
+    int stride_nodes, hw;
+};
 void net_forward_inputs(Net& net, const Store& S, int count, hipStream_t st, struct Prof* prof);
 inline void net_invalidate_sibling_cache(Net& net) { net.sib_cache_valid = false; }
 int net_commit(Net& net, const Store& S, hipStream_t st);
diff --git a/omok-ai_amd/csrc/net_kernels.hip b/omok-ai_amd/csrc/net_kernels.hip
--- a/omok-ai_amd/csrc/net_kernels.hip
+++ b/omok-ai_amd/csrc/net_kernels.hip
@@ -2623,12 +2623,30 @@
     }
 }
 
+__device__ inline float* logits_row(const LogitsDst& D, float* out_logits, size_t sample, int width) {
+    if (!D.req_ref) return out_logits + sample * width;
+    const uint32_t ref = D.req_ref[sample];
+    return D.policy + ((size_t)(ref >> 16) * (size_t)D.stride_nodes + (size_t)(ref & 0xFFFFu)) * width;
+}
+__device__ inline void logits_value_pick(const LogitsDst& D, int col, const f32x4& o, float& x, bool& have) {
+    const int q = D.hw - col;
+    const bool mine = (unsigned)q < 4u;
+    x = mine ? (q == 0 ? o[0] : q == 1 ? o[1] : q == 2 ? o[2] : o[3]) : x;
+    have = have || mine;
+}
+__device__ inline void logits_value_store(const LogitsDst& D, size_t sample, float x, bool have) {
+    if (D.req_ref && have) {
+        D.vpre[sample] = x;
+        D.v[sample] = tanhf(x);
+    }
+}
+
 template <int MT, int EPI, int TAG, int NST>
 __global__ __launch_bounds__(512) void k_gemm_t(const uint4* __restrict__ wp, const uint4* __restrict__ act, int ksteps,
                                                 size_t act_row_u4, int k_full, int last_cnt, int lo_off,
                                                 const float* __restrict__ bias, uint4* __restrict__ out_split,
                                                 size_t out_row_u4, float* __restrict__ out_logits, const int32_t* __restrict__ d_count,
-                                                int max_count) {
+                                                int max_count, LogitsDst D) {
     constexpr int MTW = MT / 4;
     extern __shared__ __attribute__((aligned(16))) unsigned char smem[];
     uint4* lds = (uint4*)smem;
@@ -2648,6 +2666,9 @@
     for (int c = 0; c < 2; ++c) {
         const int sample = b0 + 32 * (2 * ws + c) + (lane & 31);
         if (sample >= count) continue;
+        float* lrow = EPI == EPI_LOGITS ? logits_row(D, out_logits, (size_t)sample, MT * 32) : nullptr;
+        float vx = 0.0f;
+        bool vhave = false;
 #pragma unroll
         for (int i = 0; i < MTW; ++i) {
             const int mt = wm * MTW + i;
@@ -2684,17 +2705,19 @@
                     f32x4 o;
 #pragma unroll
                     for (int q = 0; q < 4; ++q) o[q] = y[4 * g + q];
-                    *(f32x4*)(out_logits + (size_t)sample * (MT * 32) + 32 * mt + 8 * g + 4 * h) = o;
-                }
-            }
-        }
+                    *(f32x4*)(lrow + 32 * mt + 8 * g + 4 * h) = o;
+                    logits_value_pick(D, 32 * mt + 8 * g + 4 * h, o, vx, vhave);
+                }
+            }
+        }
+        if (EPI == EPI_LOGITS) logits_value_store(D, (size_t)sample, vx, vhave);
     }
 }
 
 template <int MTH>
 __global__ __launch_bounds__(512) void k_tail_fused(const uint4* __restrict__ wp_fc1, const uint4* __restrict__ act, const float* __restrict__ bias_fc1,
                                                     const uint4* __restrict__ wp_heads, const float* __restrict__ bias_heads, float* __restrict__ out_logits,
-                                                    const int32_t* __restrict__ d_count, int max_count) {
+                                                    const int32_t* __restrict__ d_count, int max_count, LogitsDst D) {
     constexpr int MTW = MTH / 4;
     constexpr int WFR = MTH * 2;
     constexpr int LPW = WFR / 8;
@@ -2819,6 +2842,9 @@
     for (int c = 0; c < 2; ++c) {
         const int sample = b0 + 32 * (2 * ws + c) + (lane & 31);
         if (sample >= count) continue;
+        float* lrow = logits_row(D, out_logits, (size_t)sample, MTH * 32);
+        float vx = 0.0f;
+        bool vhave = false;
 #pragma unroll
         for (int i = 0; i < MTW; ++i) {
             const int mt = wm * MTW + i;
@@ -2828,9 +2854,11 @@
                 f32x4 o;
 #pragma unroll
                 for (int q = 0; q < 4; ++q) o[q] = acc[i][c][4 * g + q] + bv[q];
-                *(f32x4*)(out_logits + (size_t)sample * (MTH * 32) + 32 * mt + 8 * g + 4 * h) = o;
-            }
-        }
+                *(f32x4*)(lrow + 32 * mt + 8 * g + 4 * h) = o;
+                logits_value_pick(D, 32 * mt + 8 * g + 4 * h, o, vx, vhave);
+            }
+        }
+        logits_value_store(D, (size_t)sample, vx, vhave);
     }
 }
 
@@ -2839,7 +2867,7 @@
 template <int MT, int EPI>
 __global__ __launch_bounds__(512) void k_gemm_w(const uint4* __restrict__ wp, const uint4* __restrict__ act, int ksteps, size_t act_row_u4,
                                                 const float* __restrict__ bias, uint4* __restrict__ out_split, size_t out_row_u4,
-                                                float* __restrict__ out_logits, const int32_t* __restrict__ d_count, int max_count) {
+                                                float* __restrict__ out_logits, const int32_t* __restrict__ d_count, int max_count, LogitsDst D) {
     static_assert(MT % 8 == 0 && EPI != EPI_PARTIAL, "k_gemm_w: whole-K launches of at least one m-tile per wave");
     constexpr int MTW = MT / 8;
     constexpr int AF = MTW * 2;
@@ -2937,6 +2965,9 @@
     for (int ct = 0; ct < 4; ++ct) {
         const int sample = b0 + 32 * ct + sl;
         if (sample >= count) continue;
+        float* lrow = EPI == EPI_LOGITS ? logits_row(D, out_logits, (size_t)sample, MT * 32) : nullptr;
+        float vx = 0.0f;
+        bool vhave = false;
 #pragma unroll
         for (int i = 0; i < MTW; ++i) {
             const int mt = wave * MTW + i;
@@ -2965,10 +2996,12 @@
                     f32x4 o;
 #pragma unroll
                     for (int q = 0; q < 4; ++q) o[q] = y[4 * g + q];
-                    *(f32x4*)(out_logits + (size_t)sample * (MT * 32) + 32 * mt + 8 * g + 4 * h) = o;
-                }
-            }
-        }
+                    *(f32x4*)(lrow + 32 * mt + 8 * g + 4 * h) = o;
+                    logits_value_pick(D, 32 * mt + 8 * g + 4 * h, o, vx, vhave);
+                }
+            }
+        }
+        if (EPI == EPI_LOGITS) logits_value_store(D, (size_t)sample, vx, vhave);
     }
 }
 
@@ -3002,7 +3035,7 @@
 }
 
 __global__ __launch_bounds__(256) void k_splitk_logits(const float* __restrict__ part, int nsplit, size_t cap_rows, int width, const float* __restrict__ bias,
-                                                       float* __restrict__ logits, const int32_t* __restrict__ d_count, int max_count) {
+                                                       float* __restrict__ logits, const int32_t* __restrict__ d_count, int max_count, LogitsDst D) {
     int count = d_count[0];
     if (count > max_count) count = max_count;
     const size_t per_row = (size_t)width / 4, total = (size_t)count * per_row;
@@ -3017,7 +3050,11 @@
         const f32x4 bv = *(const f32x4*)(bias + col);
 #pragma unroll
         for (int j = 0; j < 4; ++j) a[j] += bv[j];
-        *(f32x4*)(logits + row * width + col) = a;
+        *(f32x4*)(logits_row(D, logits, row, width) + col) = a;
+        float vx = 0.0f;
+        bool vhave = false;
+        logits_value_pick(D, (int)col, a, vx, vhave);
+        logits_value_store(D, row, vx, vhave);
     }
 }
 
@@ -3424,7 +3461,7 @@
 template <int MT, int EPI, int TAG, int NST = 3>
 static void launch_gemm(const void* wp, const void* act, int ksteps, size_t act_row_u4, int k_full, int last_cnt, int lo_off,
                         const float* bias, void* out_split, size_t out_row_u4, float* out_logits, const Store& S, int max_count,
-                        hipStream_t st, int device, int nsplit = 1) {
+                        hipStream_t st, int device, int nsplit = 1, const LogitsDst& D = LogitsDst{}) {
     constexpr int LDS = (MT * 2 + 8) * 1024 * NST;
     static bool attr_done[64] = {};
     auto kern = k_gemm_t<MT, EPI, TAG, NST>;
@@ -3434,12 +3471,12 @@
     }
     const dim3 grid((max_count + GT_BS - 1) / GT_BS, nsplit);
     kern<<<grid, 512, LDS, st>>>((const uint4*)wp, (const uint4*)act, ksteps, act_row_u4, k_full, last_cnt, lo_off, bias, (uint4*)out_split,
-                                  out_row_u4, out_logits, S.d_count, max_count);
+                                  out_row_u4, out_logits, S.d_count, max_count, D);
 }
 
 template <int MTH>
 static void launch_tail_fused(const void* wp_fc1, const void* act, const float* bias_fc1, const void* wp_heads, const float* bias_heads, float* out_logits, const Store& S,
-                              int max_count, hipStream_t st, int device) {
+                              int max_count, hipStream_t st, int device, const LogitsDst& D) {
     constexpr int LDS = 160 * 1024;
     static bool attr_done[64] = {};
     auto kern = k_tail_fused<MTH>;
@@ -3448,12 +3485,12 @@
         attr_done[device & 63] = true;
     }
     kern<<<dim3((max_count + GT_BS - 1) / GT_BS), 512, LDS, st>>>((const uint4*)wp_fc1, (const uint4*)act, bias_fc1, (const uint4*)wp_heads, bias_heads, out_logits, S.d_count,
-                                                                 max_count);
+                                                                 max_count, D);
 }
 
 template <int MT, int EPI>
 static void launch_gemm_w(const void* wp, const void* act, int ksteps, size_t act_row_u4, const float* bias, void* out_split, size_t out_row_u4, float* out_logits,
-                          const Store& S, int max_count, hipStream_t st, int device) {
+                          const Store& S, int max_count, hipStream_t st, int device, const LogitsDst& D = LogitsDst{}) {
     constexpr int LDS = gemm_w_lds(MT);
     static_assert(LDS <= 160 * 1024, "k_gemm_w LDS");
     static bool attr_done[64] = {};
@@ -3463,7 +3500,7 @@
         attr_done[device & 63] = true;
     }
     kern<<<dim3((max_count + GT_BS - 1) / GT_BS), 512, LDS, st>>>((const uint4*)wp, (const uint4*)act, ksteps, act_row_u4, bias, (uint4*)out_split, out_row_u4, out_logits,
-                                                                 S.d_count, max_count);
+                                                                 S.d_count, max_count, D);
 }
 
 constexpr int SIB_MAX_WWAYS = 14;
@@ -3678,7 +3715,8 @@
     while (tsplit < 8 && tiles_t * tsplit * 2 <= n_cu && (size_t)(tsplit * 2) * (size_t)(tiles_t * GT_BS) <= part_rows) tsplit *= 2;
     return tsplit;
 }
-static void forward_f16x3(Net& net, const Store& S, int max_count, bool from_f32, hipStream_t st, Prof* prof, int sib_side = -1, bool skip_softmax = false) {
+static void forward_f16x3(Net& net, const Store& S, int max_count, bool from_f32, hipStream_t st, Prof* prof, int sib_side = -1, bool skip_softmax = false,
+                          bool rows_to_nodes = false) {
     const int hw = net.hw;
     const int use_sib = sib_env();
     const bool sib = sibling_path(net, from_f32, sib_side);
@@ -3715,6 +3753,8 @@
     }
     if (prof) { prof->end(st); prof->begin(PC_TAIL, st); }
     const int MT = heads_mt(hw);
+    LogitsDst D{};
+    if (rows_to_nodes && skip_softmax && MT * 32 == net.rowp) D = LogitsDst{S.req_ref, S.policy, net.v, net.vpre, S.stride_nodes, hw};
     const int tiles_t = (max_count + GT_BS - 1) / GT_BS;
     const int tsplit = net.plan_tsplit = tail_tsplit(max_count, net.n_cu, net.part_rows);
     const size_t cap_t = (size_t)tiles_t * GT_BS;
@@ -3723,12 +3763,12 @@
         const char* gw_env = getenv("OMOK_GEMM_W");
         const bool gw = gw_env && gw_env[0] == '1';
         if (!gw) {
-            if (MT == 8) launch_tail_fused<8>(net.wt_fc1, h0, bias_fc1, net.wt_heads, bias_heads, net.s0, S, max_count, st, net.device);
-            else launch_tail_fused<4>(net.wt_fc1, h0, bias_fc1, net.wt_heads, bias_heads, net.s0, S, max_count, st, net.device);
+            if (MT == 8) launch_tail_fused<8>(net.wt_fc1, h0, bias_fc1, net.wt_heads, bias_heads, net.s0, S, max_count, st, net.device, D);
+            else launch_tail_fused<4>(net.wt_fc1, h0, bias_fc1, net.wt_heads, bias_heads, net.s0, S, max_count, st, net.device, D);
         } else {
             launch_gemm_w<16, EPI_SPLIT>(net.wt_fc1, h0, 32, 128, bias_fc1, h1, 128, nullptr, S, max_count, st, net.device);
-            if (MT == 8) launch_gemm_w<8, EPI_LOGITS>(net.wt_heads, h1, 32, 128, bias_heads, nullptr, 0, net.s0, S, max_count, st, net.device);
-            else launch_gemm<4, EPI_LOGITS, 2>(net.wt_heads, h1, 32, 128, 32, 1, 2, bias_heads, nullptr, 0, net.s0, S, max_count, st, net.device);
+            if (MT == 8) launch_gemm_w<8, EPI_LOGITS>(net.wt_heads, h1, 32, 128, bias_heads, nullptr, 0, net.s0, S, max_count, st, net.device, D);
+            else launch_gemm<4, EPI_LOGITS, 2>(net.wt_heads, h1, 32, 128, 32, 1, 2, bias_heads, nullptr, 0, net.s0, S, max_count, st, net.device, 1, D);
         }
     } else {
         launch_gemm<16, EPI_PARTIAL, 1>(net.wt_fc1, h0, 32 / tsplit, 128, 32, 1, 2, bias_fc1, nullptr, cap_t, net.part, S, max_count, st, net.device, tsplit);
@@ -3736,7 +3776,7 @@
         if (MT == 8) launch_gemm<8, EPI_PARTIAL, 2>(net.wt_heads, h1, 32 / tsplit, 128, 32, 1, 2, bias_heads, nullptr, cap_t, net.part, S, max_count, st, net.device, tsplit);
         else launch_gemm<4, EPI_PARTIAL, 2>(net.wt_heads, h1, 32 / tsplit, 128, 32, 1, 2, bias_heads, nullptr, cap_t, net.part, S, max_count, st, net.device, tsplit);
         const unsigned lg = (unsigned)(((size_t)max_count * (MT * 8) + 255) / 256);
-        k_splitk_logits<<<lg < 2048 ? lg : 2048, 256, 0, st>>>(net.part, tsplit, cap_t, MT * 32, bias_heads, net.s0, S.d_count, max_count);
+        k_splitk_logits<<<lg < 2048 ? lg : 2048, 256, 0, st>>>(net.part, tsplit, cap_t, MT * 32, bias_heads, net.s0, S.d_count, max_count, D);
     }
     const int sg = max_count < 32768 ? max_count : 32768;
     if (!skip_softmax) k_softmax<<<sg, 64, 0, st>>>(net.s0, MT * 32, hw, net.rowp, net.p, net.v, net.vpre, S.d_count, max_count);
@@ -3982,7 +4022,9 @@
 
 bool net_logits_cover_batch(const Net& net, int max_count) { return net.mode != OMOK_NET_F32 && max_count <= net.max_b; }
 
-void net_forward_requests(Net& net, const Store& S, int max_count, hipStream_t st, Prof* prof, int sibling_side, bool skip_softmax) {
+bool net_rows_fit_policy(const Net& net) { return net.mode != OMOK_NET_F32 && heads_mt(net.hw) * 32 == net.rowp; }
+
+void net_forward_requests(Net& net, const Store& S, int max_count, hipStream_t st, Prof* prof, int sibling_side, bool skip_softmax, bool rows_to_nodes) {
     if (max_count <= 0) return;
     if (max_count > net.max_b) max_count = net.max_b;
     if (net.mode == OMOK_NET_F32) {
@@ -3991,7 +4033,7 @@
         forward_f32(net, S, max_count, st, prof);
         net.plan_path = 3; net.plan_rows = max_count; net.plan_nsplit = net.plan_tsplit = 0;
     } else {
-        forward_f16x3(net, S, max_count, false, st, prof, sibling_side, skip_softmax);
+        forward_f16x3(net, S, max_count, false, st, prof, sibling_side, skip_softmax, rows_to_nodes);
     }
 }
 
diff --git a/omok-ai_amd/csrc/tree_kernels.hip b/omok-ai_amd/csrc/tree_kernels.hip
--- a/omok-ai_amd/csrc/tree_kernels.hip
+++ b/omok-ai_amd/csrc/tree_kernels.hip
@@ -359,11 +359,64 @@
     return idx;
 }
 
-template <int N>
-__device__ void apply_noise(const Tree<N>& T, const RoundArgs& A, uint32_t tree_global, float* s_row) {
+constexpr uint8_t POLICY_RAW = 2;
+#ifndef LAZY_INLINE
+#define LAZY_INLINE inline
+#endif
+template <int N>
+__device__ LAZY_INLINE void policy_materialise_at(float* __restrict__ prow, const uint64_t* __restrict__ bnode, NodeHdr* hnode, float* s_row) {
+    using G = Geo<N>;
+    constexpr int NW = G::NW, hw = G::HW;
+    const int lane = LANE;
+    float lv[G::IT];
+#pragma unroll
+    for (int jj = 0; jj < G::IT; ++jj) lv[jj] = lane + 64 * jj < hw ? prow[lane + 64 * jj] : -INFINITY;
+    uint64_t occ[NW];
+#pragma unroll
+    for (int w = 0; w < NW; ++w) occ[w] = bnode[w] | bnode[NW + w];
+    float mx = -INFINITY;
+#pragma unroll
+    for (int jj = 0; jj < G::IT; ++jj) mx = fmaxf(mx, lv[jj]);
+    for (int o = 32; o > 0; o >>= 1) mx = fmaxf(mx, __shfl_xor(mx, o, 64));
+    float sum = 0.0f, row[G::IT];
+#pragma unroll
+    for (int jj = 0; jj < G::IT; ++jj) {
+        const int a = lane + 64 * jj;
+        row[jj] = 0.0f;
+        if (a < hw) { row[jj] = expf(lv[jj] - mx); sum += row[jj]; }
+    }
+    for (int o = 32; o > 0; o >>= 1) sum += __shfl_xor(sum, o, 64);
+    __syncthreads();
+#pragma unroll
+    for (int jj = 0; jj < G::IT; ++jj) {
+        const int a = jj * 64 + lane;
+        const float p = a < hw ? row[jj] / sum : 0.0f;
+        const bool empty = a < hw && !((occ[jj] >> lane) & 1ULL);
+        row[jj] = empty ? p : 0.0f;
+        s_row[a] = row[jj];
+    }
+    __syncthreads();
+    const float acc = seq_sum(s_row, hw);
+    const bool renorm = F32_EPS <= acc;
+    const float inv = renorm ? __fdiv_rn(1.0f, acc) : 1.0f;
+#pragma unroll
+    for (int jj = 0; jj < G::IT; ++jj) prow[jj * 64 + lane] = renorm ? row[jj] * inv : row[jj];
+    if (lane == 0) hnode->has_policy = 1;
+    __syncthreads();
+}
+template <int N>
+__device__ inline void policy_materialise(const Tree<N>& T, int node, float* s_row, uint32_t* s_cnt = nullptr, int site = 0) {
+    policy_materialise_at<N>(T.pol + (size_t)node * Geo<N>::ROWP, T.board + (size_t)node * (2 * Geo<N>::NW), T.hdr + node, s_row);
+    if (s_cnt && LANE == 0) s_cnt[site] += 1u;
+}
+struct Lazy { float* s_row; uint32_t* s_cnt; };
+
+template <int N>
+__device__ void apply_noise(const Tree<N>& T, const RoundArgs& A, uint32_t tree_global, float* s_row, uint32_t* s_cnt = nullptr) {
     using G = Geo<N>;
     const int lane = LANE;
     NodeHdr h0 = T.hdr[0];
+    if (h0.has_policy == POLICY_RAW) policy_materialise<N>(T, 0, s_row, s_cnt, 0);
     uint64_t bb[2 * G::NW];
 #pragma unroll
     for (int i = 0; i < 2 * G::NW; ++i) bb[i] = T.board[i];
@@ -417,12 +470,11 @@
 }
 
 template <int N, bool REC>
-__device__ inline void select_leaf_impl(const Tree<N>& T, NodeHdr& h, int& node, uint32_t& node_n, unsigned long long& path_bytes, PathRec& rec) {
+__device__ inline void select_leaf_impl(const Tree<N>& T, NodeHdr& h, int& node, uint32_t& node_n, unsigned long long& path_bytes, PathRec& rec, int& lev) {
     using G = Geo<N>;
     constexpr int ROWP = G::ROWP;
     const int lane = LANE;
-    int lev = 0;
-    while (h.nch == h.legal && h.nch != 0) {
+    while (h.nch == h.legal && h.nch != 0 && h.has_policy != POLICY_RAW) {
         const uint32_t pn = node_n > 1u ? node_n : 1u;
         const float sq = __fsqrt_rn((float)pn);
         const size_t tb = (size_t)h.table * ROWP;
@@ -489,9 +541,24 @@
     if (REC) rec.depth = lev;
 }
 template <int N>
-__device__ inline void select_leaf(const Tree<N>& T, NodeHdr& h, int& node, uint32_t& node_n, unsigned long long& path_bytes) {
+__device__ inline bool select_leaf_lazy(const Tree<N>& T, NodeHdr& h, int& node, uint32_t& node_n, unsigned long long& path_bytes, PathRec& rec, bool rec_on,
+                                        const Lazy& L) {
+    int lev = 0;
+    bool root_done = false;
+    for (;;) {
+        if (rec_on) select_leaf_impl<N, true>(T, h, node, node_n, path_bytes, rec, lev);
+        else select_leaf_impl<N, false>(T, h, node, node_n, path_bytes, rec, lev);
+        if (!(h.nch == h.legal && h.nch != 0)) break;
+        root_done = root_done || node == 0;
+        policy_materialise<N>(T, uni(node), L.s_row, L.s_cnt, 1);
+        h.has_policy = 1;
+    }
+    return root_done;
+}
+template <int N>
+__device__ inline void select_leaf(const Tree<N>& T, NodeHdr& h, int& node, uint32_t& node_n, unsigned long long& path_bytes, const Lazy& L) {
     PathRec none;
-    select_leaf_impl<N, false>(T, h, node, node_n, path_bytes, none);
+    select_leaf_lazy<N>(T, h, node, node_n, path_bytes, none, false, L);
 }
 
 template <int N>
@@ -529,7 +596,7 @@
 
 template <int N>
 __device__ void run_sim(const Store& S, const Tree<N>& T, Regs& R, LeafCache<N>& C, const RoundArgs& A, uint32_t sim_index,
-                        uint32_t tree_global) {
+                        uint32_t tree_global, const Lazy& L) {
     using G = Geo<N>;
     constexpr int ROWP = G::ROWP, NW = G::NW;
     const int lane = LANE;
@@ -546,7 +613,7 @@
     if (cached) h = C.h;
     else { fence_own_stores(R); h = T.hdr[node]; }
     if (h.nch == h.legal && h.nch != 0) { fence_own_stores(R); C.node = -1; }
-    select_leaf<N>(T, h, node, node_n, path_bytes);
+    select_leaf<N>(T, h, node, node_n, path_bytes, L);
     R.bytes += path_bytes;
     R.memo_node = node;
     R.memo_n = node_n;
@@ -618,7 +685,8 @@
 }
 
 template <int N>
-__device__ void run_sims(const Store& S, const Tree<N>& T, Regs& R, LeafCache<N>& C, const RoundArgs& A, uint32_t first_sim, int count, uint32_t tree_global) {
+__device__ void run_sims(const Store& S, const Tree<N>& T, Regs& R, LeafCache<N>& C, const RoundArgs& A, uint32_t first_sim, int count, uint32_t tree_global,
+                         const Lazy& L) {
     using G = Geo<N>;
     constexpr int ROWP = G::ROWP, NW = G::NW;
     const int lane = LANE;
@@ -650,11 +718,8 @@
             if (from_root) { root_h = uni(h); root_ok = true; }
         }
         if (h.nch == h.legal && h.nch != 0) { fence_own_stores(R); C.node = -1; }
-        if (from_root) select_leaf_impl<N, true>(T, h, node, node_n, path_bytes, rec);
-        else {
-            select_leaf<N>(T, h, node, node_n, path_bytes);
-            rec.depth = -1;
-        }
+        if (select_leaf_lazy<N>(T, h, node, node_n, path_bytes, rec, from_root, L)) root_h.has_policy = 1;
+        if (!from_root) rec.depth = -1;
         KP(2);
         R.memo_node = node;
         R.memo_n = node_n;
@@ -862,6 +927,8 @@
 __global__ __launch_bounds__(64, KROUND_WPS) void k_round(Store S, RoundArgs A) {
     using G = Geo<N>;
     __shared__ float s_row[G::ROWP];
+    __shared__ uint32_t s_cnt[2];
+    if (LANE < 2) s_cnt[LANE] = 0u;
     const int g = blockIdx.x;
     const int t = A.side * S.games + g;
     if (A.zero_ptr && g == 0)
@@ -880,17 +947,18 @@
     kp_last = __builtin_readcyclecounter();
 #endif
     if (A.scatter_v && ts.n_req > 0) {
-        scatter_tree<N>(S, T, ts, R, A.scatter_v);
+        scatter_tree<N>(S, T, ts, R, A.scatter_v, A.lazy_rows);
         R.dirty = true;
     }
     A.ply = gs0.plies;
     const uint32_t tree_global = (uint32_t)((A.game_offset + gs0.gid) * 2 + A.side);
     KP(0);
-    if (A.round == 0) apply_noise<N>(T, A, tree_global, s_row);
+    if (A.round == 0) apply_noise<N>(T, A, tree_global, s_row, s_cnt);
     KP(1);
     LeafCache<N> C;
-    if (KROUND_BATCH) run_sims<N>(S, T, R, C, A, (uint32_t)(A.round * A.K), A.K, tree_global);
-    else for (int i = 0; i < A.K; ++i) run_sim<N>(S, T, R, C, A, (uint32_t)(A.round * A.K + i), tree_global);
+    const Lazy L{s_row, s_cnt};
+    if (KROUND_BATCH) run_sims<N>(S, T, R, C, A, (uint32_t)(A.round * A.K), A.K, tree_global, L);
+    else for (int i = 0; i < A.K; ++i) run_sim<N>(S, T, R, C, A, (uint32_t)(A.round * A.K + i), tree_global, L);
     if (LANE == 0) {
         TreeState o = ts;
         o.n_nodes = R.n_nodes; o.n_tables = R.n_tables; o.root_n = R.root_n; o.root_w = R.root_w;
@@ -898,6 +966,10 @@
         *T.ts = o;
         if (A.req_cnt) A.req_cnt[g] = (int32_t)R.n_req;
         atomicAdd(S.d_bytes, R.bytes);
+        if (A.lazy_stats) {
+            if (s_cnt[0]) atomicAdd(A.lazy_stats, s_cnt[0]);
+            if (s_cnt[1]) atomicAdd(A.lazy_stats + 1, s_cnt[1]);
+        }
 #ifdef KROUND_PROF
         const unsigned int L = (unsigned int)A.round & 63u;
         if (t < 8192)
@@ -1322,7 +1394,7 @@
 }
 
 template <int N>
-__device__ inline void scatter_tree(const Store& S, const Tree<N>& T, const TreeState& ts, Regs& R, const float* __restrict__ V) {
+__device__ inline void scatter_tree(const Store& S, const Tree<N>& T, const TreeState& ts, Regs& R, const float* __restrict__ V, int raw_rows) {
     using G = Geo<N>;
     constexpr int ROWP = G::ROWP;
     const int lane = LANE, nreq = (int)ts.n_req;
@@ -1334,6 +1406,7 @@
         par = (int)hx.parent;
         act = (int)hx.action;
         val = V[(size_t)ts.req_base + lane];
+        if (ts.req_base + (uint32_t)lane < (uint32_t)raw_rows) T.hdr[x].has_policy = POLICY_RAW;
     }
     const int prev_par = __shfl_up(par, 1, 64);
     unsigned long long rem = __ballot(lane < nreq && (lane == 0 || par != prev_par));
@@ -1392,7 +1465,7 @@
 }
 
 template <int N>
-__global__ __launch_bounds__(64) void k_scatter(Store S, int side, const float* __restrict__ V) {
+__global__ __launch_bounds__(64) void k_scatter(Store S, int side, const float* __restrict__ V, int raw_rows) {
     const int g = blockIdx.x;
     if (!S.gs[g].alive) return;
     const int t = side * S.games + g;
@@ -1400,12 +1473,26 @@
     const TreeState ts = *T.ts;
     if (ts.n_req == 0) return;
     Regs R{ts.n_nodes, ts.n_tables, ts.root_n, 0u, ts.error, ts.root_w, 0ull};
-    scatter_tree<N>(S, T, ts, R, V);
+    scatter_tree<N>(S, T, ts, R, V, raw_rows);
     if (LANE == 0) {
         TreeState o = ts;
         o.root_n = R.root_n; o.root_w = R.root_w; o.n_req = 0;
         *T.ts = o;
         atomicAdd(S.d_bytes, R.bytes);
+    }
+}
+
+template <int N>
+__global__ __launch_bounds__(64) void k_materialise(Store S, int tree_first) {
+    __shared__ float s_row[Geo<N>::ROWP];
+    const Tree<N> T(S, tree_first + (int)blockIdx.y);
+    const int i = (int)blockIdx.x * 64 + LANE;
+    const uint32_t nn = T.ts->n_nodes < (uint32_t)S.cap_nodes ? T.ts->n_nodes : (uint32_t)S.cap_nodes;
+    unsigned long long m = __ballot((uint32_t)i < nn && T.hdr[(uint32_t)i < nn ? i : 0].has_policy == POLICY_RAW);
+    while (m) {
+        const int l = __ffsll((long long)m) - 1;
+        m &= m - 1;
+        policy_materialise<N>(T, (int)blockIdx.x * 64 + l, s_row);
     }
 }
 
@@ -2165,7 +2252,7 @@
 }
 
 template <int N>
-__device__ void ensure_action_exists(const Store& S, const Tree<N>& T, int action, const float* __restrict__ p_row, float* s_row) {
+__device__ void ensure_action_exists(const Store& S, const Tree<N>& T, int action, const float* __restrict__ p_row, float* s_row, bool raw) {
     using G = Geo<N>;
     constexpr int ROWP = G::ROWP, NW = G::NW;
     const int lane = LANE;
@@ -2173,21 +2260,21 @@
     uint64_t bb[2 * NW];
 #pragma unroll
     for (int i = 0; i < 2 * NW; ++i) bb[i] = T.board[i];
-    bool renorm;
-    float inv;
-    masked_policy_row<N>(bb, action, p_row, s_row, renorm, inv);
+    bool renorm = false;
+    float inv = 1.0f;
+    if (!raw) masked_policy_row<N>(bb, action, p_row, s_row, renorm, inv);
     const bool exists = h0.table != NONE16 && T.corder[(size_t)h0.table * ROWP + action] != NONE8;
     if (!exists) {
         const TreeState ts = *T.ts;
         Regs R{ts.n_nodes, ts.n_tables, ts.root_n, 0u, ts.error, ts.root_w, 0ull};
         if (!get_bit<NW>(bb, action) && !get_bit<NW>(bb + NW, action)) (void)place_and_status<N>(bb, h0.turn, h0.legal, action);
         NodeHdr h0m = h0;
-        const int idx = add_child<N>(S, T, R, 0, h0m, action, bb, ST_IN_PROGRESS, 1 - h0.turn, 1);
+        const int idx = add_child<N>(S, T, R, 0, h0m, action, bb, ST_IN_PROGRESS, 1 - h0.turn, raw ? POLICY_RAW : 1);
         if (idx >= 0) {
 #pragma unroll
             for (int j = 0; j < G::IT; ++j) {
                 const int a = j * 64 + lane;
-                const float x = s_row[a];
+                const float x = raw ? p_row[a] : s_row[a];
                 T.pol[(size_t)idx * ROWP + a] = renorm ? x * inv : x;
             }
         }
@@ -2201,7 +2288,7 @@
 }
 
 template <int N>
-__global__ __launch_bounds__(64) void k_advance(Store S, int side, const float* __restrict__ P) {
+__global__ __launch_bounds__(64) void k_advance(Store S, int side, const float* __restrict__ P, int raw) {
     using G = Geo<N>;
     constexpr int ROWP = G::ROWP, NW = G::NW;
     extern __shared__ __attribute__((aligned(16))) unsigned char smem[];
@@ -2216,8 +2303,8 @@
     const int action = gs.last_action;
     const Tree<N> own(S, side * S.games + g);
     const Tree<N> opp(S, (1 - side) * S.games + g);
-    if (gs.external) ensure_action_exists<N>(S, own, action, P + (size_t)gs.mirror_idx * ROWP, s_row);
-    ensure_action_exists<N>(S, opp, action, P + (size_t)gs.mirror_idx * ROWP, s_row);
+    if (gs.external) ensure_action_exists<N>(S, own, action, P + (size_t)gs.mirror_idx * ROWP, s_row, raw != 0);
+    ensure_action_exists<N>(S, opp, action, P + (size_t)gs.mirror_idx * ROWP, s_row, raw != 0);
     int status;
     {
         const NodeHdr h0 = own.hdr[0];
@@ -2663,8 +2750,12 @@
     DISPATCH_N(n, (k_scatter_policy<9><<<grid, 64, 0, st>>>(S, p, max_count)), (k_scatter_policy<15><<<grid, 64, 0, st>>>(S, p, max_count)));
     if (backups) launch_backups(n, S, side, v, st);
 }
-void launch_backups(int n, const Store& S, int side, const float* v, hipStream_t st) {
-    DISPATCH_N(n, (k_scatter<9><<<S.games, 64, 0, st>>>(S, side, v)), (k_scatter<15><<<S.games, 64, 0, st>>>(S, side, v)));
+void launch_backups(int n, const Store& S, int side, const float* v, hipStream_t st, int raw_rows) {
+    DISPATCH_N(n, (k_scatter<9><<<S.games, 64, 0, st>>>(S, side, v, raw_rows)), (k_scatter<15><<<S.games, 64, 0, st>>>(S, side, v, raw_rows)));
+}
+void launch_materialise(int n, const Store& S, int tree_first, int trees, hipStream_t st) {
+    const dim3 grid((unsigned)((S.cap_nodes + 63) / 64), (unsigned)trees);
+    DISPATCH_N(n, (k_materialise<9><<<grid, 64, 0, st>>>(S, tree_first)), (k_materialise<15><<<grid, 64, 0, st>>>(S, tree_first)));
 }
 void launch_softmax_scatter(int n, const Store& S, int side, const float* logits, int lrow, float* v, float* vpre, int max_count, hipStream_t st,
                             bool backups) {
@@ -2680,9 +2771,9 @@
                (k_sample<15><<<S.games, 64, 0, st>>>(S, side, ply, temperature, threshold, seed, game_offset, actions)));
 }
 void launch_mirror_scan(int n, const Store& S, int side, hipStream_t st) { k_mirror_scan<<<1, 1024, 0, st>>>(S, side); }
-void launch_advance(int n, const Store& S, int side, const float* p, hipStream_t st) {
+void launch_advance(int n, const Store& S, int side, const float* p, hipStream_t st, bool raw) {
     const size_t lds = advance_lds_bytes(S.cap_nodes, S.cap_tables);
-    DISPATCH_N(n, (k_advance<9><<<S.games, 64, lds, st>>>(S, side, p)), (k_advance<15><<<S.games, 64, lds, st>>>(S, side, p)));
+    DISPATCH_N(n, (k_advance<9><<<S.games, 64, lds, st>>>(S, side, p, raw ? 1 : 0)), (k_advance<15><<<S.games, 64, lds, st>>>(S, side, p, raw ? 1 : 0)));
 }
 void launch_encode_requests(int n, const Store& S, float* out, int max_b, hipStream_t st) {
     if (max_b <= 0) return;
```

Result: faster. 613.8 games/s, median of 6 (+2.1%).
